# vghuy17ck1/svt-av1-psyex

Measured on AMD Instinct MI355X. Metric: ME+RD-cost Mpixels/s (2160p10 preset-6), higher is better.
Workload: dtype u8 SAD / i32 transforms; 1 GPU; 3840x2160 10-bit synthetic pan sequence, preset 6 (M6) search controls at qp 35; step = 16 pictures (4 current pictures x ref distance 1,2,4,8; R=2): open-loop ME of all 2040 b64 + full-pel pred + RD chain (64x64,32x32,16x16 DCT_DCT, 10-bit, b quantizer; qcoeff + recon + scalars written); 3 picture sets alternate from step to step

## Files before the change

### include/svt_hip_me.h

```cpp
#ifndef SVT_HIP_ME_H
#define SVT_HIP_ME_H

#include <stdint.h>
#include <stddef.h>

#ifdef __cplusplus
extern "C" {
#endif

#define SVT_HIP_OK 0
#define SVT_HIP_ERR_NO_DEVICE 1
#define SVT_HIP_ERR_BAD_PARAM 2
#define SVT_HIP_ERR_NO_MEMORY 3
#define SVT_HIP_ERR_LAUNCH 4

#define SVT_HIP_MAX_LISTS 2
#define SVT_HIP_MAX_REFS 4
#define SVT_HIP_SQUARE_PU_COUNT 85
#define SVT_HIP_MAX_SAD_VALUE (128 * 128 * 255)

typedef struct SvtHipSearchArea {
    uint16_t width, height;
} SvtHipSearchArea;

typedef struct SvtHipSearchAreaMinMax {
    SvtHipSearchArea sa_min, sa_max;
} SvtHipSearchAreaMinMax;

typedef struct SvtHipMeConfig {
    uint8_t hme_search_method, me_search_method;
    uint8_t enable_hme_flag, enable_hme_level0_flag, enable_hme_level1_flag, enable_hme_level2_flag;
    uint16_t num_hme_sa_w, num_hme_sa_h;
    SvtHipSearchAreaMinMax hme_l0_sa;
    SvtHipSearchArea       hme_l1_sa, hme_l2_sa;
    SvtHipSearchAreaMinMax me_sa;
    uint8_t                prehme_enable, prehme_skip_search_line, prehme_l1_early_exit;
    uint8_t                me_type;
    SvtHipSearchAreaMinMax prehme_sa_cfg[2];
    uint8_t  enable_me_hme_ref_pruning;
    uint16_t prune_ref_if_hme_sad_dev_bigger_than_th, prune_ref_if_me_sad_dev_bigger_than_th;
    uint32_t zz_sad_th;
    uint16_t zz_sad_pct;
    uint32_t phme_sad_th;
    uint16_t phme_sad_pct;
    uint8_t  enable_me_sr_adjustment;
    uint16_t reduce_me_sr_based_on_mv_length_th, stationary_hme_sad_abs_th, stationary_me_sr_divisor;
    uint16_t reduce_me_sr_based_on_hme_sad_abs_th, me_sr_divisor_for_low_hme_sad;
    uint8_t  distance_based_hme_resizing;
    uint8_t  me_8x8_var_enabled;
    uint32_t me_sr_div4_th, me_sr_div2_th, me_sr_mult2_th;
    uint8_t  mv_sa_adj_enabled, mv_sa_adj_nearest_ref_only;
    uint16_t mv_sa_adj_mv_size_th, mv_sa_adj_sa_multiplier;
    int32_t  prune_me_candidates_th;
    uint8_t  use_best_unipred_cand_only;
    uint8_t  reduce_hme_l0_sr_th_min, reduce_hme_l0_sr_th_max;
    uint32_t me_early_exit_th, me_safe_limit_zz_th, prev_me_stage_based_exit_th;
} SvtHipMeConfig;

typedef struct SvtHipMePresetDesc {
    int8_t   enc_mode;
    uint8_t  input_resolution;
    uint8_t  sc_class1;
    uint8_t  rtc_tune;
    uint8_t  temporal_layer_index;
    uint8_t  hierarchical_levels;
    uint32_t qp;
    uint32_t frame_rate_q16;
    uint8_t  safe_limit_nref;
    uint32_t safe_limit_zz_th;
} SvtHipMePresetDesc;

typedef struct SvtHipPlaneDesc {
    const uint8_t *buffer_y;
    uint32_t       stride_y;
    uint16_t       org_x, org_y;
    uint16_t       width, height;
} SvtHipPlaneDesc;

typedef struct SvtHipContext   SvtHipContext;
typedef struct SvtHipPaPicture SvtHipPaPicture;

typedef struct SvtHipMePictureDesc {
    uint64_t picture_number;
    uint16_t aligned_width, aligned_height;
    uint8_t  num_of_list_to_search;
    uint8_t  num_of_ref_pic_to_search[SVT_HIP_MAX_LISTS];
    uint8_t  temporal_layer_index, hierarchical_levels, is_ref, similar_brightness_refs;
    uint8_t  enable_me_8x8, enable_me_16x16;
    uint8_t  max_number_of_pus_per_sb;
    uint8_t  max_cand, max_refs, max_l0;
    uint8_t  input_resolution;
    uint8_t  only_l_bwd;
    uint8_t  gm_enabled, gm_use_distance_based_active_th;
    uint16_t b64_row_start, b64_row_count;
    uint32_t tf_me_exit_th;
    uint64_t ref_picture_number[SVT_HIP_MAX_LISTS][SVT_HIP_MAX_REFS];
} SvtHipMePictureDesc;

typedef struct SvtHipMeResults {
    uint8_t  *total_me_candidate_index;
    uint32_t *me_mv_array;
    uint8_t  *me_candidate_array;
    uint32_t *me_64x64_distortion, *me_32x32_distortion, *me_16x16_distortion, *me_8x8_distortion;
    uint32_t *rc_me_distortion, *me_8x8_cost_variance;
    uint8_t  *stationary_block_present_sb, *rc_me_allow_gm;
    uint32_t *sb_best_sad, *sb_best_mv;
    int16_t  *hme_sc;
    uint32_t *hme_sad;
    uint8_t  *do_ref;
} SvtHipMeResults;

static inline uint32_t svt_hip_me_n_pu(uint8_t enable_me_16x16, uint8_t enable_me_8x8) {
    return enable_me_16x16 ? (enable_me_8x8 ? 85u : 21u) : 5u;
}

int  svt_hip_context_create(SvtHipContext **ctx, int device);
void svt_hip_context_destroy(SvtHipContext *ctx);
const char *svt_hip_last_error(const SvtHipContext *ctx);
void *svt_hip_context_stream(SvtHipContext *ctx);
int   svt_hip_context_sync(SvtHipContext *ctx);
int   svt_hip_context_set_me_waves_per_cu(SvtHipContext *ctx, uint32_t waves);
int   svt_hip_context_set_me_dense(SvtHipContext *ctx, int on);
int   svt_hip_context_set_me_staged(SvtHipContext *ctx, int on);
#define SVT_HIP_ME_CHAIN_KERNELS 7
int   svt_hip_context_set_me_timing(SvtHipContext *ctx, int on);
int   svt_hip_me_launch_times(SvtHipContext *ctx, float ms[SVT_HIP_ME_CHAIN_KERNELS]);
const char *svt_hip_me_chain_kernel_name(int i);
int   svt_hip_context_set_me_counting(SvtHipContext *ctx, int on);
int   svt_hip_me_dense_counters(SvtHipContext *ctx, unsigned long long out[2]);

int     svt_hip_me_config_from_preset(const SvtHipMePresetDesc *p, SvtHipMeConfig *cfg);
uint8_t svt_hip_input_resolution(uint32_t width, uint32_t height);
uint8_t svt_hip_enable_me_8x8(int8_t enc_mode, uint8_t rtc_tune, uint8_t input_resolution);

int  svt_hip_pa_picture_create(SvtHipContext *ctx, const SvtHipPlaneDesc *full, const SvtHipPlaneDesc *quarter,
                               const SvtHipPlaneDesc *sixteenth, SvtHipPaPicture **pic);
int  svt_hip_pa_picture_create_dev(SvtHipContext *ctx, const SvtHipPlaneDesc *full_dev, SvtHipPaPicture **pic);
int  svt_hip_pa_picture_update(SvtHipContext *ctx, SvtHipPaPicture *pic, const SvtHipPlaneDesc *full, int full_on_device);
int  svt_hip_pa_picture_update_ahead(SvtHipContext *ctx, SvtHipPaPicture *pic, const SvtHipPlaneDesc *full, int full_on_device);
void *svt_hip_context_transfer_stream(SvtHipContext *ctx);
void svt_hip_pa_picture_destroy(SvtHipContext *ctx, SvtHipPaPicture *pic);
int  svt_hip_pa_picture_download(SvtHipContext *ctx, const SvtHipPaPicture *pic, int level, uint8_t *dst,
                                 uint32_t dst_stride);
int  svt_hip_pa_picture_geometry(const SvtHipPaPicture *pic, int level, SvtHipPlaneDesc *out);

int svt_hip_me_picture(SvtHipContext *ctx, const SvtHipMeConfig *cfg, const SvtHipMePictureDesc *desc,
                       const SvtHipPaPicture *cur, const SvtHipPaPicture *const refs[SVT_HIP_MAX_LISTS][SVT_HIP_MAX_REFS],
                       SvtHipMeResults *res);
int svt_hip_me_picture_async(SvtHipContext *ctx, const SvtHipMeConfig *cfg, const SvtHipMePictureDesc *desc,
                             const SvtHipPaPicture *cur,
                             const SvtHipPaPicture *const refs[SVT_HIP_MAX_LISTS][SVT_HIP_MAX_REFS],
                             const SvtHipMeResults *res_dev);

typedef struct SvtHipMeJob {
    const SvtHipMeConfig      *cfg;
    const SvtHipMePictureDesc *desc;
    const SvtHipPaPicture     *cur;
    const SvtHipPaPicture     *refs[SVT_HIP_MAX_LISTS][SVT_HIP_MAX_REFS];
    const SvtHipMeResults     *results;
} SvtHipMeJob;
int svt_hip_me_pictures_async(SvtHipContext *ctx, uint32_t n_pictures, const SvtHipMeJob *jobs);

typedef struct SvtHipDgMetrics {
    uint64_t tot_dist;
    uint32_t tot_cplx;
    uint32_t tot_active;
    int32_t  sum_in_vectors;
    uint32_t reserved;
} SvtHipDgMetrics;

int svt_hip_dg_detector_hme_level0(SvtHipContext *ctx, const SvtHipPaPicture *src, const SvtHipPaPicture *ref,
                                   uint16_t aligned_width, uint16_t aligned_height, uint8_t input_resolution,
                                   SvtHipDgMetrics *metrics, uint32_t *b64_sad, int16_t *b64_mv);
int svt_hip_dg_detector_hme_level0_async(SvtHipContext *ctx, const SvtHipPaPicture *src, const SvtHipPaPicture *ref,
                                         uint16_t aligned_width, uint16_t aligned_height, uint8_t input_resolution,
                                         SvtHipDgMetrics *metrics_dev, uint32_t *b64_sad_dev, int16_t *b64_mv_dev);

#ifdef __cplusplus
}
#endif
#endif
```

### svt-av1-psyex_amd/api.py

```python
import ctypes as C
import os

import numpy as np

from . import abi

_HERE = os.path.dirname(os.path.abspath(__file__))
LIB_PATH = os.environ.get("SVT_HIP_LIBRARY") or os.path.join(_HERE, "libsvthip.so")
_lib = None

ERRORS = {1: "no usable gfx950 device", 2: "bad parameter", 3: "out of device memory", 4: "launch/stream error"}


class SvtHipError(RuntimeError):
    pass


def lib():
    global _lib
    if _lib is None:
        if not os.path.exists(LIB_PATH):
            raise SvtHipError(f"{LIB_PATH} is missing: build it with `make -C svt-av1-psyex_amd/csrc` "
                              "(or __graft_entry__.build()); there is no CPU fallback")
        try:
            import torch
        except Exception:
            pass
        L = C.CDLL(LIB_PATH)
        L.svt_hip_last_error.restype = C.c_char_p
        L.svt_hip_last_error.argtypes = [C.c_void_p]
        L.svt_hip_context_stream.restype = C.c_void_p
        L.svt_hip_context_stream.argtypes = [C.c_void_p]
        L.svt_hip_sizeof.restype = C.c_size_t
        L.svt_hip_input_resolution.restype = C.c_uint8
        L.svt_hip_enable_me_8x8.restype = C.c_uint8
        for name in ("svt_hip_context_destroy", "svt_hip_context_sync"):
            getattr(L, name).argtypes = [C.c_void_p]
        L.svt_hip_pa_picture_destroy.argtypes = [C.c_void_p, C.c_void_p]
        L.svt_hip_block_stats_jobs_per_wave.restype = C.c_uint32
        L.svt_hip_block_stats_jobs_per_wave.argtypes = [C.c_void_p, C.c_void_p]
        _lib = L
    return _lib


def config_from_preset(enc_mode, width, height, qp=35, temporal_layer_index=1, hierarchical_levels=4, sc_class1=0,
                       rtc_tune=0, fps=30):
    L = lib()
    pd = abi.MePresetDesc(enc_mode=enc_mode, input_resolution=L.svt_hip_input_resolution(width, height), sc_class1=sc_class1,
                          rtc_tune=rtc_tune, temporal_layer_index=temporal_layer_index, hierarchical_levels=hierarchical_levels,
                          qp=qp, frame_rate_q16=fps << 16)
    cfg = abi.MeConfig()
    rc = L.svt_hip_me_config_from_preset(C.byref(pd), C.byref(cfg))
    if rc:
        raise SvtHipError(f"svt_hip_me_config_from_preset: {ERRORS.get(rc, rc)}")
    return cfg


def picture_desc(width, height, picture_number, refs, enc_mode=6, temporal_layer_index=1, hierarchical_levels=4, is_ref=1,
                 gm_enabled=0, rtc_tune=0):
    L = lib()
    res = L.svt_hip_input_resolution(width, height)
    r0 = sum(1 for (li, _) in refs if li == 0)
    r1 = sum(1 for (li, _) in refs if li == 1)
    d = abi.MePictureDesc(picture_number=picture_number, aligned_width=width, aligned_height=height,
                          num_of_list_to_search=2 if r1 else 1, temporal_layer_index=temporal_layer_index,
                          hierarchical_levels=hierarchical_levels, is_ref=is_ref, similar_brightness_refs=0,
                          enable_me_8x8=L.svt_hip_enable_me_8x8(enc_mode, rtc_tune, res), enable_me_16x16=1,
                          max_number_of_pus_per_sb=85, input_resolution=res, gm_enabled=gm_enabled)
    d.num_of_ref_pic_to_search[0] = r0
    d.num_of_ref_pic_to_search[1] = r1
    d.max_refs = r0 + r1
    d.max_cand = r0 + r1 + r0 * r1 + (r0 - 1) + (1 if r1 == 3 else 0)
    d.max_l0 = r0
    for (li, ri), num in refs.items():
        d.ref_picture_number[li][ri] = num
    return d


class Context:

    def __init__(self, device=-1):
        self._h = C.c_void_p()
        rc = lib().svt_hip_context_create(C.byref(self._h), device)
        if rc:
            raise SvtHipError(f"svt_hip_context_create failed: {ERRORS.get(rc, rc)} -- the HIP path cannot run here")

    def check(self, rc, what):
        if rc:
            raise SvtHipError(f"{what}: {ERRORS.get(rc, rc)}: {lib().svt_hip_last_error(self._h).decode()}")

    @property
    def stream(self):
        return lib().svt_hip_context_stream(self._h)

    def sync(self):
        self.check(lib().svt_hip_context_sync(self._h), "sync")

    def close(self):
        if self._h:
            lib().svt_hip_context_destroy(self._h)
            self._h = C.c_void_p()

    def set_me_dense(self, on):
        self.check(lib().svt_hip_context_set_me_dense(self._h, 1 if on else 0), "svt_hip_context_set_me_dense")

    def set_me_staged(self, on):
        self.check(lib().svt_hip_context_set_me_staged(self._h, int(on)), "svt_hip_context_set_me_staged")

    def set_me_timing(self, on):
        self.check(lib().svt_hip_context_set_me_timing(self._h, 1 if on else 0), "svt_hip_context_set_me_timing")

    def me_launch_times(self):
        L = lib()
        ms = (C.c_float * 7)()
        self.check(L.svt_hip_me_launch_times(self._h, ms), "svt_hip_me_launch_times")
        L.svt_hip_me_chain_kernel_name.restype = C.c_char_p
        return {L.svt_hip_me_chain_kernel_name(i).decode(): float(ms[i]) for i in range(7) if ms[i] > 0}

    def set_me_counting(self, on):
        self.check(lib().svt_hip_context_set_me_counting(self._h, 1 if on else 0), "svt_hip_context_set_me_counting")

    def me_dense_counters(self):
        v = (C.c_ulonglong * 2)()
        self.check(lib().svt_hip_me_dense_counters(self._h, v), "svt_hip_me_dense_counters")
        return int(v[0]), int(v[1])

    def upload(self, host_pyramid, device_pyramid=True):
        pic = C.c_void_p()
        full = host_pyramid.desc(2)
        if device_pyramid:
            rc = lib().svt_hip_pa_picture_create(self._h, C.byref(full), None, None, C.byref(pic))
        else:
            q, s = host_pyramid.desc(1), host_pyramid.desc(0)
            rc = lib().svt_hip_pa_picture_create(self._h, C.byref(full), C.byref(q), C.byref(s), C.byref(pic))
        self.check(rc, "svt_hip_pa_picture_create")
        return DevicePicture(self, pic, host_pyramid.picture_number)

    def upload_dev(self, dev_ptr, stride, width, height, pad, picture_number=0):
        pic = C.c_void_p()
        full = abi.PlaneDesc(dev_ptr, stride, pad, pad, width, height)
        self.check(lib().svt_hip_pa_picture_create_dev(self._h, C.byref(full), C.byref(pic)), "svt_hip_pa_picture_create_dev")
        return DevicePicture(self, pic, picture_number)

    def _ref_array(self, refs):
        arr = ((C.c_void_p * abi.MAX_REFS) * abi.MAX_LISTS)()
        for (li, ri), pic in refs.items():
            arr[li][ri] = pic._h
        return arr

    def me_picture(self, cfg, desc, cur, refs, search_level=True):
        n = abi.n_pu(desc.enable_me_16x16, desc.enable_me_8x8)
        nb = ((desc.aligned_width + 63) // 64) * ((desc.aligned_height + 63) // 64)
        res, arrs = abi.MeResults(), {}
        for name, dt, cnt in abi.RESULT_FIELDS:
            if not search_level and name in ("sb_best_sad", "sb_best_mv", "hme_sc", "hme_sad", "do_ref"):
                continue
            arrs[name] = np.zeros((nb, cnt(n, desc.max_refs, desc.max_cand)), dtype=dt)
            setattr(res, name, arrs[name].ctypes.data)
        rc = lib().svt_hip_me_picture(self._h, C.byref(cfg), C.byref(desc), cur._h, self._ref_array(refs), C.byref(res))
        self.check(rc, "svt_hip_me_picture")
        return arrs

    def me_picture_async(self, cfg, desc, cur, refs, res_dev):
        rc = lib().svt_hip_me_picture_async(self._h, C.byref(cfg), C.byref(desc), cur._h, self._ref_array(refs), C.byref(res_dev))
        self.check(rc, "svt_hip_me_picture_async")


    def me_pictures_async(self, jobs):
        arr = (abi.MeJob * len(jobs))()
        for j, (cfg, desc, cur, refs, res) in zip(arr, jobs):
            j.cfg, j.desc, j.results = C.addressof(cfg), C.addressof(desc), C.addressof(res)
            j.cur = cur._h if isinstance(cur._h, int) else cur._h.value
            for (li, ri), pic in refs.items():
                j.refs[li][ri] = pic._h if isinstance(pic._h, int) else pic._h.value
        self.check(lib().svt_hip_me_pictures_async(self._h, len(jobs), arr), "svt_hip_me_pictures_async")


    def dg_detector_hme_level0(self, src, ref, aligned_width, aligned_height, input_resolution, per_block=True):
        n = ((aligned_width + 63) // 64) * ((aligned_height + 63) // 64)
        m = abi.DgMetrics()
        sad = np.zeros(n, np.uint32) if per_block else None
        mv = np.zeros((n, 2), np.int16) if per_block else None
        rc = lib().svt_hip_dg_detector_hme_level0(self._h, src._h, ref._h, aligned_width, aligned_height, input_resolution, C.byref(m),
                                                  sad.ctypes.data_as(C.c_void_p) if per_block else None,
                                                  mv.ctypes.data_as(C.c_void_p) if per_block else None)
        self.check(rc, "svt_hip_dg_detector_hme_level0")
        out = m.as_dict()
        if per_block:
            out["b64_sad"], out["b64_mv"] = sad, mv
        return out


    def dg_detector_hme_level0_async(self, src, ref, aligned_width, aligned_height, input_resolution, metrics_ptr, sad_ptr=None, mv_ptr=None):
        rc = lib().svt_hip_dg_detector_hme_level0_async(self._h, src._h, ref._h, aligned_width, aligned_height, input_resolution,
                                                        C.c_void_p(metrics_ptr), C.c_void_p(sad_ptr), C.c_void_p(mv_ptr))
        self.check(rc, "svt_hip_dg_detector_hme_level0_async")


class DevicePicture:
    def __init__(self, ctx, handle, picture_number):
        self.ctx, self._h, self.picture_number = ctx, handle, picture_number

    def geometry(self, level):
        d = abi.PlaneDesc()
        self.ctx.check(lib().svt_hip_pa_picture_geometry(self._h, level, C.byref(d)), "geometry")
        return d

    def download(self, level):
        g = self.geometry(level)
        out = np.zeros((g.height + 2 * g.org_y, g.width + 2 * g.org_x), np.uint8)
        self.ctx.check(lib().svt_hip_pa_picture_download(self.ctx._h, self._h, level, out.ctypes.data_as(C.c_void_p), out.shape[1]), "download")
        return out

    def free(self):
        if self._h:
            lib().svt_hip_pa_picture_destroy(self.ctx._h, self._h)
            self._h = C.c_void_p()
```

### svt-av1-psyex_amd/csrc/me_kernel.hip

```cpp
#include <hip/hip_runtime.h>
#include <stdint.h>
#include <string.h>
#include "me_kernel.h"
#include "wave_ops.h"
#include "lds_dma.h"

#ifdef SVT_HIP_ME_PROFILE
struct Prof { uint32_t *acc; unsigned long long last; int step; };
#define SVT_HIP_ME_PROFILE_LDS (48 * 4)
#define PROF_DECL Prof prof_; prof_.acc = reinterpret_cast<uint32_t *>(g_lds + lay.total); if (threadIdx.x < 48) prof_.acc[threadIdx.x] = 0; prof_.last = __builtin_readcyclecounter(); prof_.step = 0; Prof *prof = &prof_
#define PROF_STEP(s) (prof->step = (s))
#define PROFS(i) PROF((i) + prof->step)
#define PROF(i) do { const unsigned long long t_ = __builtin_readcyclecounter(); if (threadIdx.x == 0) atomicAdd(&prof->acc[i], (uint32_t)(t_ - prof->last)); prof->last = t_; } while (0)
#define PROF_FLUSH(ptr) do { __builtin_amdgcn_fence(__ATOMIC_RELEASE, "wavefront"); if (threadIdx.x < 48) atomicAdd((unsigned long long *)(ptr) + threadIdx.x, (unsigned long long)prof->acc[threadIdx.x]); } while (0)
#define PROF_PARAM , Prof *prof
#define PROF_ARG , prof
#else
#define PROF_DECL do { } while (0)
#define PROF(i) do { } while (0)
#define PROFS(i) do { } while (0)
#define PROF_STEP(s) do { } while (0)
#define PROF_FLUSH(ptr) do { } while (0)
#define SVT_HIP_ME_PROFILE_LDS 0
#define PROF_PARAM
#define PROF_ARG
#endif

namespace {

constexpr int kThreads  = 64;
constexpr int kMaxReq   = 32;
constexpr int kWinBytes = SVT_HIP_ME_WIN_BYTES;
constexpr int kSrc64Pitch = 80, kSrc32Pitch = 48, kSrc16Pitch = 16;
constexpr int kNarrowMaxPos = 32;

__device__ const uint8_t c_z_to_raster[85] = {
    0,  1,  2,  3,  4,  5,  6,  9,  10, 7,  8,  11, 12, 13, 14, 17, 18, 15, 16, 19, 20, 21, 22, 29, 30, 23, 24, 31, 32,
    37, 38, 45, 46, 39, 40, 47, 48, 25, 26, 33, 34, 27, 28, 35, 36, 41, 42, 49, 50, 43, 44, 51, 52, 53, 54, 61, 62, 55,
    56, 63, 64, 69, 70, 77, 78, 71, 72, 79, 80, 57, 58, 65, 66, 59, 60, 67, 68, 73, 74, 81, 82, 75, 76, 83, 84};
__device__ const uint8_t c_8x8_to_16x16[64] = {5,  5,  6,  6,  7,  7,  8,  8,  5,  5,  6,  6,  7,  7,  8,  8,  9,  9,  10, 10, 11, 11,
                                               12, 12, 9,  9,  10, 10, 11, 11, 12, 12, 13, 13, 14, 14, 15, 15, 16, 16, 13, 13, 14, 14,
                                               15, 15, 16, 16, 17, 17, 18, 18, 19, 19, 20, 20, 17, 17, 18, 18, 19, 19, 20, 20};
__device__ const uint8_t c_16x16_to_32x32[16] = {1, 1, 2, 2, 1, 1, 2, 2, 3, 3, 4, 4, 3, 3, 4, 4};

typedef unsigned long long u64;

#define SVT_CONST_AS __attribute__((address_space(4)))
typedef const SVT_CONST_AS MeKernelParams CParams;
typedef const SVT_CONST_AS DevPlane       CPlane;

struct Req {
    const uint8_t *win;
    uint32_t       stride;
    int16_t        sa_w, sa_h;
    uint8_t        bw, bh, rs, level;
    uint8_t        skip_even, done;
    int16_t        pad1;
};

struct SearchGeo { int ox, oy, sa_w, sa_h; };

constexpr int kMaxTiles = 40;
struct __attribute__((aligned(16))) TileEnt {
    const uint8_t *g0;
    uint32_t stride;
    int16_t  x0, y0;
    int16_t  w, h;
    uint16_t pitch, nvec;
    uint8_t  req, flags;
    uint8_t  bw, bh;
    uint8_t  rs, kd, km, pad;
};
static_assert(sizeof(TileEnt) == 32, "TileEnt is read as two 16-byte words");

struct MeReq {
    const uint8_t *pix0;
    uint32_t       stride;
    int16_t        ox, oy, sa_w, sa_h;
    uint8_t        li, ri, probe, pad;
    int16_t        min_x, max_x, min_y, max_y;
};

struct PreHme {
    uint16_t sa_w, sa_h;
    int16_t  col, row;
    uint32_t sad;
    uint8_t  valid, pad[3];
};

struct St {
    uint32_t org_x, org_y, b64_w, b64_h, b64_index;
    uint32_t zz_sad[2][4];
    uint32_t sr_divisor[2][4];
    uint32_t hme_sad_final[2][4];
    u64      hme_sad64[2][4];
    int16_t  hme_sc_x[2][4], hme_sc_y[2][4];
    uint8_t  do_ref[2][4];
    PreHme   prehme[2][4][2];
    uint8_t  performed_phme[2][4][2];
    int16_t  hx[3][2][4][2][2], hy[3][2][4][2][2];
    uint32_t hs[3][2][4][2][2];
    SvtHipSearchAreaMinMax hme_l0_sa;
    int16_t  me_cx[2][4], me_cy[2][4];
    uint8_t  ph_req[2][4][2];
    uint8_t  l0_req[2][4];
    uint8_t  lvl_req[2][4][2][2];
    uint8_t  c00_req[2][4];
    int      nreq;
    union {
        Req      req[kMaxReq];
        struct { MeReq me[8], me_probe[8]; };
    };
    u64      req_key[kMaxReq];
    TileEnt  tile[kMaxTiles];
    uint32_t sadbuf[kNarrowMaxPos];
    int      nme, nprobe;
    uint32_t me_dist[85];
    uint8_t  cand0[88];
    uint32_t red[8];
    int      job, tf_exit;
};

struct LdsLayout { uint32_t src16, src32, src64, bsad, bmv, dense, win, total; };
constexpr int kMeFull = 0, kMeMid1 = 1, kMeS1 = 2, kMeMid2 = 4, kMeS2 = 5, kMeTail = 7;
#ifndef SVT_HIP_ME_LIST_WAVES_PER_CU
#define SVT_HIP_ME_LIST_WAVES_PER_CU 2
#endif
constexpr uint32_t kListWavesPerCu = SVT_HIP_ME_LIST_WAVES_PER_CU;
constexpr uint32_t kStagedMinJobs = 2048;
__host__ __device__ constexpr bool me_is_search(int m) { return m == kMeS1 || m == kMeS2; }
constexpr int kDirectWinBytes = 5120;
__host__ __device__ constexpr LdsLayout lds_layout(int n_slot, int cshift, int dense = 1, int mode = 0) {
    const bool v16 = mode == kMeFull, v32 = mode == kMeFull || mode == kMeS1, v64 = mode == kMeFull || mode == kMeS2 || mode == kMeTail;
    const bool best = mode == kMeFull || mode == kMeTail, slots = dense && (mode == kMeFull || mode == kMeMid1);
    const uint32_t arena = (mode == kMeMid1 || mode == kMeMid2) ? 0u : (mode == kMeS1 || mode == kMeS2) ? (uint32_t)kDirectWinBytes : (uint32_t)kWinBytes;
    LdsLayout l = {};
    l.src16 = (uint32_t)((sizeof(St) + 15) & ~(size_t)15);
    l.src32 = l.src16 + (v16 ? (uint32_t)((16 >> cshift) * kSrc16Pitch) : 0u);
    l.src64 = l.src32 + (v32 ? (uint32_t)((32 >> cshift) * kSrc32Pitch) : 0u);
    l.bsad  = l.src64 + (v64 ? (uint32_t)((64 >> cshift) * kSrc64Pitch) : 0u);
    l.bmv   = l.bsad + (best ? (uint32_t)n_slot * 85 * 4 : 0u);
    l.dense = (l.bmv + (best ? (uint32_t)n_slot * 85 * 4 : 0u) + 15) & ~15u;
    l.win   = l.dense + (slots ? (uint32_t)n_slot * SVT_HIP_ME_DENSE_KINDS * 16u : 0u);
    l.total = l.win + arena;
    return l;
}
extern __shared__ __attribute__((aligned(16))) uint8_t g_lds[];
struct Shared {
    St       &st;
    uint32_t  src64, src32, src16, win;
    int       cshift;
};
#define LDS(off) (g_lds + (off))

__host__ __device__ __forceinline__ int iabs(int v) { return v < 0 ? -v : v; }
__host__ __device__ __forceinline__ int imax(int a, int b) { return a > b ? a : b; }
__host__ __device__ __forceinline__ int imin(int a, int b) { return a < b ? a : b; }
__device__ __forceinline__ uint32_t umin32(uint32_t a, uint32_t b) { return a < b ? a : b; }
__device__ __forceinline__ uint32_t umin(uint32_t a, uint32_t b) { return a < b ? a : b; }

__host__ __device__ __forceinline__ uint32_t scaled_distance(uint32_t dist) { return (dist * 5) / 8 + ((dist % 8) ? 1 : 0); }

template <class P> __host__ __device__ __forceinline__ uint32_t ref_distance(P &p, int li, int ri) {
    long long d = (long long)p.desc.picture_number - (long long)p.desc.ref_picture_number[li][ri];
    return (uint16_t)(int16_t)(d < 0 ? -d : d);
}

__device__ __forceinline__ void clip_axis(int org, int &origin, int &size, int pad, int dim) {
    if (org + origin < -pad) origin = -pad - org;
    if (org + origin > dim - 1) origin -= (org + origin) - (dim - 1);
    if (org + origin + size > dim) size = imax(1, size - ((org + origin + size) - dim));
}

__device__ __forceinline__ const uint8_t *plane_at(CPlane &pl, int x, int y) {
    return pl.base + (long long)(pl.org_y + y) * pl.stride + (pl.org_x + x);
}


__device__ __forceinline__ float rcp_of(uint32_t d) { return __builtin_amdgcn_rcpf((float)d); }
__device__ __forceinline__ uint32_t div_by_rcp(uint32_t k, float r) { return (uint32_t)(((float)k + 0.5f) * r); }

__device__ __forceinline__ uint32_t row_pitch(int w, int bw) {
    uint32_t p = (uint32_t)(((w + 7) & ~7) + bw + 4 + 15) & ~15u;
    return (p & 16u) ? p : p + 16u;
}

__device__ __forceinline__ uint32_t tile_bytes(const Req &r, int w, int h) {
    return row_pitch(w, r.bw) * (uint32_t)(h - 1 + (r.bh - 1) * r.rs + 1);
}




__device__ __forceinline__ const uint8_t *src_view(const Shared &sh, int level) {
    return LDS(level == 2 ? sh.src64 : (level == 1 ? sh.src32 : sh.src16));
}

template <int NDW>
__device__ __forceinline__ void quad_sad_rows(const uint8_t *src, int src_pitch, int srs, const uint8_t *wrow0, int pitch, int rs, int r0, int r1,
                                              uint32_t out[4]) {
    uint32_t a0 = 0, a1 = 0, a2 = 0, a3 = 0;
    constexpr int kRowsPerFlush = 64 / NDW;
    for (int rb = r0; rb < r1; rb += kRowsPerFlush) {
        const int re = rb + kRowsPerFlush < r1 ? rb + kRowsPerFlush : r1;
        u64       acc = 0;
        for (int r = rb; r < re; r++) {
            const uint32_t *s = reinterpret_cast<const uint32_t *>(src + r * srs * src_pitch);
            const uint32_t *w = reinterpret_cast<const uint32_t *>(wrow0 + r * rs * pitch);
            uint32_t sv[NDW], wv[NDW + 1];
            if constexpr (NDW % 4 == 0) {
#pragma unroll
                for (int j = 0; j < NDW; j += 4) {
                    const uint4 q = *reinterpret_cast<const uint4 *>(s + j);
                    sv[j] = q.x; sv[j + 1] = q.y; sv[j + 2] = q.z; sv[j + 3] = q.w;
                }
            } else {
#pragma unroll
                for (int j = 0; j < NDW; j++) sv[j] = s[j];
            }
#pragma unroll
            for (int j = 0; j <= NDW; j++) wv[j] = w[j];
#pragma unroll
            for (int j = 0; j < NDW; j++) acc = __builtin_amdgcn_qsad_pk_u16_u8(((u64)wv[j + 1] << 32) | wv[j], sv[j], acc);
        }
        a0 += (uint32_t)(acc & 0xFFFF); a1 += (uint32_t)((acc >> 16) & 0xFFFF);
        a2 += (uint32_t)((acc >> 32) & 0xFFFF); a3 += (uint32_t)(acc >> 48);
    }
    out[0] = a0; out[1] = a1; out[2] = a2; out[3] = a3;
}

__device__ __attribute__((noinline)) uint4 quad_sad_generic(const uint8_t *src, int src_pitch, int srs, const uint8_t *wrow0, int pitch, int rs, int bw, int r0, int r1) {
    uint32_t a0 = 0, a1 = 0, a2 = 0, a3 = 0;
    if ((bw & 3) == 0) {
        const int nd = bw >> 2;
        for (int r = r0; r < r1; r++) {
            const uint32_t *s = reinterpret_cast<const uint32_t *>(src + r * srs * src_pitch);
            const uint32_t *w = reinterpret_cast<const uint32_t *>(wrow0 + r * rs * pitch);
            u64      acc = 0;
            uint32_t lo  = w[0];
            for (int j = 0; j < nd; j++) {
                const uint32_t hi = w[j + 1];
                acc = __builtin_amdgcn_qsad_pk_u16_u8(((u64)hi << 32) | lo, s[j], acc);
                lo  = hi;
            }
            a0 += (uint32_t)(acc & 0xFFFF); a1 += (uint32_t)((acc >> 16) & 0xFFFF);
            a2 += (uint32_t)((acc >> 32) & 0xFFFF); a3 += (uint32_t)(acc >> 48);
        }
    } else {
        for (int r = r0; r < r1; r++) {
            const uint8_t *s = src + r * srs * src_pitch;
            const uint8_t *w = wrow0 + r * rs * pitch;
            for (int c = 0; c < bw; c++) {
                const int sv = s[c];
                a0 += (uint32_t)iabs(sv - (int)w[c]);     a1 += (uint32_t)iabs(sv - (int)w[c + 1]);
                a2 += (uint32_t)iabs(sv - (int)w[c + 2]); a3 += (uint32_t)iabs(sv - (int)w[c + 3]);
            }
        }
    }
    return make_uint4(a0, a1, a2, a3);
}

__device__ __forceinline__ void quad_sad(const uint8_t *src, int src_pitch, int srs, const uint8_t *wrow0, int pitch, int rs, int bw, int r0,
                                         int r1, uint32_t out[4]) {
    switch (bw) {
    case 16: quad_sad_rows<4>(src, src_pitch, srs, wrow0, pitch, rs, r0, r1, out); return;
    case 32: quad_sad_rows<8>(src, src_pitch, srs, wrow0, pitch, rs, r0, r1, out); return;
    case 64: quad_sad_rows<16>(src, src_pitch, srs, wrow0, pitch, rs, r0, r1, out); return;
    case 8: quad_sad_rows<2>(src, src_pitch, srs, wrow0, pitch, rs, r0, r1, out); return;
    case 4: quad_sad_rows<1>(src, src_pitch, srs, wrow0, pitch, rs, r0, r1, out); return;
    default: break;
    }
    const uint4 v = quad_sad_generic(src, src_pitch, srs, wrow0, pitch, rs, bw, r0, r1);
    out[0] = v.x; out[1] = v.y; out[2] = v.z; out[3] = v.w;
}

template <int NDW>
__device__ __forceinline__ void oct_sad_rows(const uint8_t *src, int src_pitch, int srs, const uint8_t *wrow0, int pitch, int rs, int r0, int r1, uint32_t out[8]) {
    uint32_t a[8] = {0, 0, 0, 0, 0, 0, 0, 0};
    constexpr int kRowsPerFlush = 64 / NDW;
    constexpr int CH = NDW > 8 ? 8 : NDW;
    for (int rb = r0; rb < r1; rb += kRowsPerFlush) {
        const int re = rb + kRowsPerFlush < r1 ? rb + kRowsPerFlush : r1;
        u64       acc0 = 0, acc1 = 0;
        for (int r = rb; r < re; r++) {
            const uint32_t *s = reinterpret_cast<const uint32_t *>(src + r * srs * src_pitch);
            const uint32_t *w = reinterpret_cast<const uint32_t *>(wrow0 + r * rs * pitch);
#pragma unroll
            for (int c0 = 0; c0 < NDW; c0 += CH) {
                uint32_t sv[CH], wv[CH + 2];
                if constexpr (CH % 4 == 0) {
#pragma unroll
                    for (int j = 0; j < CH; j += 4) {
                        const uint4 q = *reinterpret_cast<const uint4 *>(s + c0 + j);
                        sv[j] = q.x; sv[j + 1] = q.y; sv[j + 2] = q.z; sv[j + 3] = q.w;
                    }
                } else {
#pragma unroll
                    for (int j = 0; j < CH; j++) sv[j] = s[c0 + j];
                }
                if constexpr (CH % 2 == 0) {
#pragma unroll
                    for (int j = 0; j < CH + 2; j += 2) {
                        const uint2 q = *reinterpret_cast<const uint2 *>(w + c0 + j);
                        wv[j] = q.x; wv[j + 1] = q.y;
                    }
                } else {
#pragma unroll
                    for (int j = 0; j < CH + 2; j++) wv[j] = w[c0 + j];
                }
#pragma unroll
                for (int j = 0; j < CH; j++) {
                    acc0 = __builtin_amdgcn_qsad_pk_u16_u8(((u64)wv[j + 1] << 32) | wv[j], sv[j], acc0);
                    acc1 = __builtin_amdgcn_qsad_pk_u16_u8(((u64)wv[j + 2] << 32) | wv[j + 1], sv[j], acc1);
                }
            }
        }
#pragma unroll
        for (int i = 0; i < 4; i++) { a[i] += (uint32_t)((acc0 >> (16 * i)) & 0xFFFF); a[4 + i] += (uint32_t)((acc1 >> (16 * i)) & 0xFFFF); }
    }
#pragma unroll
    for (int i = 0; i < 8; i++) out[i] = a[i];
}

__device__ __forceinline__ void oct_sad(const uint8_t *src, int src_pitch, int srs, const uint8_t *wrow0, int pitch, int rs, int bw, int r0, int r1, uint32_t out[8]) {
    switch (bw) {
    case 16: oct_sad_rows<4>(src, src_pitch, srs, wrow0, pitch, rs, r0, r1, out); return;
    case 32: oct_sad_rows<8>(src, src_pitch, srs, wrow0, pitch, rs, r0, r1, out); return;
    case 64: oct_sad_rows<16>(src, src_pitch, srs, wrow0, pitch, rs, r0, r1, out); return;
    case 8: oct_sad_rows<2>(src, src_pitch, srs, wrow0, pitch, rs, r0, r1, out); return;
    case 4: oct_sad_rows<1>(src, src_pitch, srs, wrow0, pitch, rs, r0, r1, out); return;
    default: break;
    }
    quad_sad(src, src_pitch, srs, wrow0, pitch, rs, bw, r0, r1, out);
    quad_sad(src, src_pitch, srs, wrow0 + 4, pitch, rs, bw, r0, r1, out + 4);
}

typedef uint32_t V4 __attribute__((ext_vector_type(4)));
typedef const __attribute__((address_space(1))) V4 GV4;
constexpr int kVecPerLane = (kWinBytes / 16 + 63) / 64;

__device__ __forceinline__ uint32_t uni(uint32_t v) { return (uint32_t)__builtin_amdgcn_readfirstlane((int)v); }
__device__ __forceinline__ const uint8_t *uni_ptr(const uint8_t *p) {
    const uintptr_t a = reinterpret_cast<uintptr_t>(p);
    return reinterpret_cast<const uint8_t *>(((uintptr_t)uni((uint32_t)(a >> 32)) << 32) | uni((uint32_t)a));
}

__device__ __forceinline__ u64 wave_min_key(uint32_t sad, uint32_t pos) {
    const uint32_t smin = wave_min_dpp(sad);
    const uint32_t pmin = wave_min_dpp(sad == smin ? pos : 0xFFFFFFFFu);
    return ((u64)smin << 32) | pmin;
}

struct TileGeo {
    const uint8_t *g0;
    uint32_t stride;
    int      req;
    int      x0, y0, w, h;
    int      pitch, nvec;
    int      last;
    int      bw, bh, rs, level, skip_even, narrow;
    int      kd, km;
};

__device__ __forceinline__ int scan32(int v) {
#define SVT_SCAN_DPP(ctrl, rmask, bc) v += __builtin_amdgcn_update_dpp(0, v, ctrl, rmask, 0xF, bc);
    SVT_SCAN_DPP(0x111, 0xF, true)
    SVT_SCAN_DPP(0x112, 0xF, true)
    SVT_SCAN_DPP(0x114, 0xF, true)
    SVT_SCAN_DPP(0x118, 0xF, true)
    SVT_SCAN_DPP(0x142, 0xA, false)
#undef SVT_SCAN_DPP
    return v;
}

__device__ __forceinline__ int plan_tiles(St &st, int nreq, int t0) {
    const int lane = threadIdx.x;
    int cnt = 0, tw = 8, th = 1, ntx = 1;
    Req r = {};
    if (lane < nreq) {
        r = st.req[lane];
        if (r.done) {
        } else if (r.sa_w > 0 && r.sa_h > 0) {
            tw = r.sa_w; th = r.sa_h;
            while (th > 1 && tile_bytes(r, tw, th) > (uint32_t)kWinBytes) th = (th + 1) >> 1;
            while (tw > 8 && tile_bytes(r, tw, th) > (uint32_t)kWinBytes) tw = ((tw >> 1) + 7) & ~7;
            ntx = (int)div_by_rcp((uint32_t)(r.sa_w + tw - 1), rcp_of((uint32_t)tw));
            cnt = ntx * (int)div_by_rcp((uint32_t)(r.sa_h + th - 1), rcp_of((uint32_t)th));
        } else if (t0 == 0)
            st.req_key[lane] = (0xffffffull << 32) | 0xffffffffull;
    }
    const int incl = scan32(cnt), base = incl - cnt - t0;
    const int total = __builtin_amdgcn_readlane(incl, 31);
    const float ntx_rcp = rcp_of((uint32_t)ntx);
    const int narrow = (r.sa_w * r.sa_h <= kNarrowMaxPos) ? 1 : 0;
    for (int k = imax(0, -base); k < cnt && base + k < kMaxTiles; k++) {
        const int ty = (int)div_by_rcp((uint32_t)k, ntx_rcp), tx = k - ty * ntx;
        const int x0 = tx * tw, y0 = ty * th, w = imin(tw, r.sa_w - x0), h = imin(th, r.sa_h - y0);
        const int pitch = (int)row_pitch(w, r.bw), vpr = pitch >> 4;
        const int kd = (int)div_by_rcp(64u, rcp_of((uint32_t)vpr));
        TileEnt e;
        e.g0 = r.win + x0 + (long long)y0 * r.stride; e.stride = r.stride;
        e.x0 = (int16_t)x0; e.y0 = (int16_t)y0; e.w = (int16_t)w; e.h = (int16_t)h;
        e.pitch = (uint16_t)pitch; e.nvec = (uint16_t)(vpr * (h - 1 + (r.bh - 1) * r.rs + 1));
        e.req = (uint8_t)lane; e.flags = (uint8_t)(r.level | (r.skip_even << 2) | (narrow << 3) | ((k == cnt - 1) << 4));
        e.bw = r.bw; e.bh = r.bh; e.rs = r.rs; e.kd = (uint8_t)kd; e.km = (uint8_t)(64 - kd * vpr); e.pad = 0;
        st.tile[base + k] = e;
    }
    return total;
}

__device__ __forceinline__ TileGeo read_tile(const St &st, int i) {
    const uint4 a = *reinterpret_cast<const uint4 *>(&st.tile[i]);
    const uint4 b = *(reinterpret_cast<const uint4 *>(&st.tile[i]) + 1);
    const uint32_t a0 = uni(a.x), a1 = uni(a.y), a2 = uni(a.z), a3 = uni(a.w), b0 = uni(b.x), b1 = uni(b.y), b2 = uni(b.z), b3 = uni(b.w);
    TileGeo t;
    t.g0 = reinterpret_cast<const uint8_t *>(((uintptr_t)a1 << 32) | a0); t.stride = a2;
    t.x0 = (int16_t)(a3 & 0xFFFF); t.y0 = (int16_t)(a3 >> 16); t.w = (int16_t)(b0 & 0xFFFF); t.h = (int16_t)(b0 >> 16);
    t.pitch = (int)(b1 & 0xFFFF); t.nvec = (int)(b1 >> 16);
    t.req = (int)(b2 & 0xFF);
    const int f = (int)((b2 >> 8) & 0xFF);
    t.level = f & 3; t.skip_even = (f >> 2) & 1; t.narrow = (f >> 3) & 1; t.last = (f >> 4) & 1;
    t.bw = (int)((b2 >> 16) & 0xFF); t.bh = (int)(b2 >> 24);
    t.rs = (int)(b3 & 0xFF); t.kd = (int)((b3 >> 8) & 0xFF); t.km = (int)((b3 >> 16) & 0xFF);
    return t;
}

typedef uint32_t V4U __attribute__((ext_vector_type(4), aligned(1)));
typedef const __attribute__((address_space(1))) V4U GV4U;
constexpr int kSmallVec = 128;
template <int S0, int NS>
__device__ __forceinline__ void tile_load(const TileGeo &t, V4 (&v)[kVecPerLane]) {
    const int      lane = threadIdx.x, vpr = t.pitch >> 4, nrows = (int)div_by_rcp((uint32_t)t.nvec, rcp_of((uint32_t)vpr));
    const int      row0 = (int)div_by_rcp((uint32_t)lane, rcp_of((uint32_t)vpr));
    int            c    = lane - row0 * vpr;
    uint32_t       off  = (uint32_t)__mul24(row0, (int)t.stride) + (uint32_t)c * 16u;
    const uint32_t last = (uint32_t)__mul24(nrows - 1, (int)t.stride) + (uint32_t)(vpr - 1) * 16u;
    const uint32_t step = (uint32_t)__mul24(t.kd, (int)t.stride) + (uint32_t)t.km * 16u, wrap = t.stride - (uint32_t)vpr * 16u;
    const uintptr_t base = reinterpret_cast<uintptr_t>(t.g0);
#pragma unroll
    for (int j = 0; j < NS; j++)
        if (j * 64 < t.nvec) {
            v[S0 + j] = __builtin_bit_cast(V4, *reinterpret_cast<GV4U *>(base + (uint64_t)umin(off, last)));
            off += step; c += t.km;
            if (c >= vpr) { c -= vpr; off += wrap; }
        }
}
template <int S0, int NS>
__device__ __forceinline__ void tile_store(const Shared &sh, int nvec, int lds_vec, const V4 (&v)[kVecPerLane]) {
    const int lane = threadIdx.x;
#pragma unroll
    for (int j = 0; j < NS; j++)
        if (j * 64 < nvec && lane + j * 64 < nvec) *reinterpret_cast<V4 *>(&LDS(sh.win)[(lds_vec + lane + j * 64) * 16]) = v[S0 + j];
}

__device__ __forceinline__ u64 tile_eval(const Shared &sh, const TileGeo &t, int lds_off PROF_PARAM) {
    St            &st   = sh.st;
    const int      lane = threadIdx.x;
    const uint8_t *src  = src_view(sh, t.level);
    const uint8_t *win  = LDS(sh.win) + lds_off;
    const int      sp   = (t.level == 2) ? kSrc64Pitch : (t.level == 1 ? kSrc32Pitch : kSrc16Pitch);
    const int      srs  = t.rs >> sh.cshift;
    uint32_t bsad_ = 0xFFFFFFFFu, bpos_ = 0xFFFFFFFFu;
    if (!t.narrow) {
        const int   ng = (t.w + 7) >> 3, nitems = ng * t.h;
        const float ng_rcp = rcp_of((uint32_t)ng);
        uint32_t best = 0xFFFFFFFFu;
        int      seq  = 0;
        for (int it = lane; it < nitems; it += kThreads, seq += 8) {
            const int y = (int)div_by_rcp((uint32_t)it, ng_rcp), g = it - y * ng;
            if (t.skip_even && !((t.y0 + y) & 1)) continue;
            uint32_t s8[8];
            oct_sad(src, sp, srs, win + y * t.pitch + 8 * g, t.pitch, t.rs, t.bw, 0, t.bh, s8);
            uint32_t k[8];
#pragma unroll
            for (int i = 0; i < 8; i++) k[i] = (s8[i] << 12) + (uint32_t)i;
            if (t.w & 7) {
#pragma unroll
// ... 143 lines not shown
    for (int dpt = 0; dpt < DEPTH; dpt++) {
#pragma unroll
        for (int k = 0; k < NV; k++) v[dpt][k] = V4U{0, 0, 0, 0};
        request(v[dpt], dpt);
    }
    u64 acc0 = 0, acc1 = 0;
    auto step = [&](V4U (&r)[NV], int t) {
#pragma unroll
        for (int k = 0; k < NV; k++) *reinterpret_cast<V4U *>(arena + 16 * (lane + 64 * k)) = r[k];
        wave_sync();
        request(r, t + DEPTH);
        if (t < rows) {
            const uint32_t *s = reinterpret_cast<const uint32_t *>(src + (e0 + t) * srs * sp);
            uint32_t sv[NDW], wv[4 * NV];
#pragma unroll
            for (int j = 0; j < NDW; j += 4) {
                const uint4 q = *reinterpret_cast<const uint4 *>(s + j);
                sv[j] = q.x; sv[j + 1] = q.y; sv[j + 2] = q.z; sv[j + 3] = q.w;
            }
#pragma unroll
            for (int k = 0; k < NV; k++) {
                const uint4 q = *reinterpret_cast<const uint4 *>(arena + 16 * (lane * NV + k));
                wv[4 * k] = q.x; wv[4 * k + 1] = q.y; wv[4 * k + 2] = q.z; wv[4 * k + 3] = q.w;
            }
#pragma unroll
            for (int j = 0; j < NDW; j++) {
                acc0 = __builtin_amdgcn_qsad_pk_u16_u8(((u64)wv[j + 1] << 32) | wv[j], sv[j], acc0);
                acc1 = __builtin_amdgcn_qsad_pk_u16_u8(((u64)wv[j + 2] << 32) | wv[j + 1], sv[j], acc1);
            }
        }
        if ((t + 1) % kRowsPerFlush == 0 || t + 1 == rows_max) {
#pragma unroll
            for (int i = 0; i < 4; i++) { a[i] += (uint32_t)((acc0 >> (16 * i)) & 0xFFFF); a[4 + i] += (uint32_t)((acc1 >> (16 * i)) & 0xFFFF); }
            acc0 = acc1 = 0;
        }
        wave_sync();
    };
    for (int t = 0; t < rows_max; t += DEPTH) {
        step(v[0], t);
        if (DEPTH >= 2 && t + 1 < rows_max) step(v[DEPTH >= 2 ? 1 : 0], t + 1);
        if (DEPTH >= 3 && t + 2 < rows_max) step(v[DEPTH >= 3 ? 2 : 0], t + 2);
    }
#pragma unroll
    for (int i = 0; i < 8; i++) out[i] = a[i];
}

__device__ __forceinline__ bool small_direct_ok(const St &st, int *q_total = nullptr) {
    const int lane = threadIdx.x, nreq = (int)uni((uint32_t)st.nreq);
    const Req &r0 = st.req[0];
    const int  bw = (int)uni(r0.bw), bh = (int)uni(r0.bh), rs = (int)uni(r0.rs), level = (int)uni(r0.level), stride = (int)uni((uint32_t)r0.stride);
    bool ok = true;
    int  per = 0;
    if (lane < nreq) {
        const Req &r = st.req[lane];
        const int  w = r.sa_w, h = r.sa_h;
        ok  = w > 0 && h > 0 && w * h <= kNarrowMaxPos && r.bw == bw && r.bh == bh && r.rs == rs && r.level == level && (int)r.stride == stride && !r.skip_even && !r.done;
        per = ((w + 7) >> 3) * h;
    }
    if (!__all(ok) || (bw != 32 && bw != 64) || nreq > kMaxReq || nreq <= 0) return false;
    const int q = (int)wave_sum_dpp((uint32_t)per);
    if (q_total) *q_total = q;
    return q <= kThreads;
}
template <int NDW, int DEPTH>
__device__ __forceinline__ void ring_rows(uint8_t *arena, const uint8_t *src, int sp, int srs, const St &st, int nreq, int lg, int S, int rows_per, int bh, int rs, int sa_h,
                                          long long stride, uint32_t (&a)[3][8]) {
    constexpr int NV = (NDW + 2 + 3) / 4, kRowsPerFlush = 64 / NDW;
    static_assert(NV & 1, "owners read their pieces back without bank conflicts");
    static_assert(DEPTH >= 1 && DEPTH <= 3, "steps in flight");
    const int lane = threadIdx.x, gmask = (1 << lg) - 1;
    const int steps_max = rs * (rows_per - 1) + sa_h;
    const uint8_t *pp[NV];
    int            pn[NV];
#pragma unroll
    for (int k = 0; k < NV; k++) {
        const int  n = lane + 64 * k, owner = n / NV, part = n - owner * NV, orq = owner >> lg, osl = owner & gmask;
        const bool act = orq < nreq && osl < S;
        const int  oe0 = osl * rows_per, orows = imin(oe0 + rows_per, bh) - oe0;
        pn[k] = act ? rs * (orows - 1) + sa_h : 0;
        pp[k] = st.req[act ? orq : 0].win + (long long)(oe0 * rs) * stride + 16 * part;
    }
    const int  req = lane >> lg, slice = lane & gmask, e0 = slice * rows_per;
    const int  rows = (req < nreq && slice < S) ? imin(e0 + rows_per, bh) - e0 : 0;
    V4U v[DEPTH][NV];
    auto request = [&](V4U (&r)[NV], int step) {
#pragma unroll
        for (int k = 0; k < NV; k++) {
            if (step < pn[k]) r[k] = *reinterpret_cast<GV4U *>(reinterpret_cast<uintptr_t>(pp[k]));
            pp[k] += stride;
        }
    };
#pragma unroll
    for (int dpt = 0; dpt < DEPTH; dpt++) {
#pragma unroll
        for (int k = 0; k < NV; k++) v[dpt][k] = V4U{0, 0, 0, 0};
        request(v[dpt], dpt);
    }
#pragma unroll
    for (int y = 0; y < 3; y++)
#pragma unroll
        for (int i = 0; i < 8; i++) a[y][i] = 0;
    u64 acc[3][2] = {{0, 0}, {0, 0}, {0, 0}};
    auto step = [&](V4U (&r)[NV], int j) {
#pragma unroll
        for (int k = 0; k < NV; k++) *reinterpret_cast<V4U *>(arena + 16 * (lane + 64 * k)) = r[k];
        wave_sync();
        request(r, j + DEPTH);
        uint32_t wv[4 * NV];
#pragma unroll
        for (int k = 0; k < NV; k++) {
            const uint4 q = *reinterpret_cast<const uint4 *>(arena + 16 * (lane * NV + k));
            wv[4 * k] = q.x; wv[4 * k + 1] = q.y; wv[4 * k + 2] = q.z; wv[4 * k + 3] = q.w;
        }
#pragma unroll
        for (int y = 0; y < 3; y++) {
            const int dd = j - y, t = rs == 2 ? dd >> 1 : dd;
            if (y < sa_h && dd >= 0 && (rs == 1 || !(dd & 1)) && t < rows_per) {
                if (t < rows) {
                    const uint32_t *s = reinterpret_cast<const uint32_t *>(src + (e0 + t) * srs * sp);
                    uint32_t sv[NDW];
#pragma unroll
                    for (int c = 0; c < NDW; c += 4) {
                        const uint4 q = *reinterpret_cast<const uint4 *>(s + c);
                        sv[c] = q.x; sv[c + 1] = q.y; sv[c + 2] = q.z; sv[c + 3] = q.w;
                    }
#pragma unroll
                    for (int c = 0; c < NDW; c++) {
                        acc[y][0] = __builtin_amdgcn_qsad_pk_u16_u8(((u64)wv[c + 1] << 32) | wv[c], sv[c], acc[y][0]);
                        acc[y][1] = __builtin_amdgcn_qsad_pk_u16_u8(((u64)wv[c + 2] << 32) | wv[c + 1], sv[c], acc[y][1]);
                    }
                }
                if ((t + 1) % kRowsPerFlush == 0 || t + 1 == rows_per) {
#pragma unroll
                    for (int i = 0; i < 4; i++) { a[y][i] += (uint32_t)((acc[y][0] >> (16 * i)) & 0xFFFF); a[y][4 + i] += (uint32_t)((acc[y][1] >> (16 * i)) & 0xFFFF); }
                    acc[y][0] = acc[y][1] = 0;
                }
            }
        }
        wave_sync();
    };
    for (int j = 0; j < steps_max; j += DEPTH) {
        step(v[0], j);
        if (DEPTH >= 2 && j + 1 < steps_max) step(v[DEPTH >= 2 ? 1 : 0], j + 1);
        if (DEPTH >= 3 && j + 2 < steps_max) step(v[DEPTH >= 3 ? 2 : 0], j + 2);
    }
}

template <int DEPTH> __device__ __forceinline__ void run_ring_searches(Shared &sh, int nreq, int bw, int bh, int rs, int level, int sa_h PROF_PARAM) {
    St       &st   = sh.st;
    const int lane = threadIdx.x;
    int lg = 0;
    while ((2 << lg) * nreq <= kThreads) lg++;
    const int S0 = imin(bh, 1 << lg), rows_per = (int)uni(div_by_rcp((uint32_t)(bh + S0 - 1), rcp_of((uint32_t)S0)));
    const int S  = (int)uni(div_by_rcp((uint32_t)(bh + rows_per - 1), rcp_of((uint32_t)rows_per)));
    const uint8_t *src = src_view(sh, level);
    const int      sp  = (level == 2) ? kSrc64Pitch : (level == 1 ? kSrc32Pitch : kSrc16Pitch), srs = rs >> sh.cshift;
    const long long stride = (long long)(int)uni((uint32_t)st.req[0].stride);
    uint32_t a[3][8];
    PROF(26);
    if (bw == 64) ring_rows<16, DEPTH>(LDS(sh.win), src, sp, srs, st, nreq, lg, S, rows_per, bh, rs, sa_h, stride, a);
    else ring_rows<8, DEPTH>(LDS(sh.win), src, sp, srs, st, nreq, lg, S, rows_per, bh, rs, sa_h, stride, a);
    PROF(27);
#define SVT_RING_SUM(cond, expr)                                                  \
    if (cond) {                                                                   \
        _Pragma("unroll") for (int y = 0; y < 3; y++)                             \
            _Pragma("unroll") for (int i = 0; i < 8; i++) { const uint32_t v = a[y][i]; a[y][i] = v + (uint32_t)(expr); } \
    }
    SVT_RING_SUM(lg >= 1, __builtin_amdgcn_mov_dpp((int)v, 0xB1 , 0xF, 0xF, true))
    SVT_RING_SUM(lg >= 2, __builtin_amdgcn_mov_dpp((int)v, 0x4E , 0xF, 0xF, true))
    SVT_RING_SUM(lg >= 3, __builtin_amdgcn_mov_dpp((int)v, 0x141 , 0xF, 0xF, true))
    SVT_RING_SUM(lg >= 4, __builtin_amdgcn_mov_dpp((int)v, 0x140 , 0xF, 0xF, true))
    SVT_RING_SUM(lg >= 5, __shfl_xor((int)v, 16, 64))
    SVT_RING_SUM(lg >= 6, __shfl_xor((int)v, 32, 64))
#undef SVT_RING_SUM
    PROF(23);
    const int req = lane >> lg;
    if (req < nreq && (lane & ((1 << lg) - 1)) == 0) {
        const int w = st.req[req].sa_w;
        uint32_t  best = 0xFFFFFFFFu;
#pragma unroll
        for (int y = 0; y < 3; y++)
#pragma unroll
            for (int i = 0; i < 8; i++)
                if (y < sa_h && i < w) best = umin(best, (a[y][i] << 6) | (uint32_t)(y * w + i));
        const int wl = (int)(best & 63u), wy = (int)div_by_rcp((uint32_t)wl, rcp_of((uint32_t)w)), wx = wl - wy * w;
        st.req_key[req] = ((u64)(best >> 6) << 32) | ((uint32_t)wy << 16) | (uint32_t)wx;
    }
    wave_sync();
}

#ifndef SVT_HIP_ME_DIRECT_RING
#define SVT_HIP_ME_DIRECT_RING 1
#endif
#ifndef SVT_HIP_ME_DIRECT_RING_FULL
#define SVT_HIP_ME_DIRECT_RING_FULL 0
#endif
#ifndef SVT_HIP_ME_DIRECT_TRUST
#define SVT_HIP_ME_DIRECT_TRUST 1
#endif
template <int DEPTH = 1, bool QUALIFIED = false, bool RING = true> __device__ __forceinline__ bool run_small_searches_direct(Shared &sh PROF_PARAM) {
    St       &st   = sh.st;
    const int lane = threadIdx.x, nreq = (int)uni((uint32_t)st.nreq);
    if constexpr (!(QUALIFIED && SVT_HIP_ME_DIRECT_TRUST)) {
        if (!small_direct_ok(st)) return false;
    }
    const Req &r0 = st.req[0];
    const int  bw = (int)uni(r0.bw), bh = (int)uni(r0.bh), rs = (int)uni(r0.rs), level = (int)uni(r0.level);
    int per = 0;
    if constexpr (RING && SVT_HIP_ME_DIRECT_RING) {
        const int h0 = (int)uni((uint32_t)r0.sa_h);
        bool alike = true;
        if (lane < nreq) {
            const int w = st.req[lane].sa_w, h = st.req[lane].sa_h;
            alike = w <= 8 && h == h0;
            per   = ((w + 7) >> 3) * h;
        }
        if (h0 <= 3 && rs <= 2 && __all(alike)) {
            run_ring_searches<DEPTH>(sh, nreq, bw, bh, rs, level, h0 PROF_ARG);
            return true;
        }
    } else if (lane < nreq)
        per = ((st.req[lane].sa_w + 7) >> 3) * st.req[lane].sa_h;
    const int Q = (int)wave_sum_dpp((uint32_t)per);
    {
        int incl = per;
#pragma unroll
        for (int o = 1; o < 32; o <<= 1) { const int t = __shfl_up(incl, o, 64); if ((lane & 31) >= o) incl += t; }
        if (lane < nreq) st.req_key[lane] = (u64)(uint32_t)(incl - per);
    }
    wave_sync();
    int       S        = imin(bh, (int)uni(div_by_rcp((uint32_t)kThreads, rcp_of((uint32_t)Q))));
    const int rows_per = (int)uni(div_by_rcp((uint32_t)(bh + S - 1), rcp_of((uint32_t)S)));
    S                  = (int)uni(div_by_rcp((uint32_t)(bh + rows_per - 1), rcp_of((uint32_t)rows_per)));
    uint32_t *sad = reinterpret_cast<uint32_t *>(LDS(sh.win));
    const uint8_t *src = src_view(sh, level);
    const int      sp  = (level == 2) ? kSrc64Pitch : (level == 1 ? kSrc32Pitch : kSrc16Pitch), srs = rs >> sh.cshift;
    const long long wstep = (long long)rs * (long long)(int)uni((uint32_t)r0.stride);
    const bool mine = lane < Q * S;
    int req = 0, y = 0, g = 0, e0 = 0, rows = 0, w = 1;
    const uint8_t *wp = nullptr;
    if (mine) {
        const int slice = (int)div_by_rcp((uint32_t)lane, rcp_of((uint32_t)Q)), q = lane - slice * Q;
        for (int r = 1; r < nreq; r++) req += q >= (int)(uint32_t)st.req_key[r] ? 1 : 0;
        const Req &r = st.req[req];
        w = r.sa_w;
        const int ng = (w + 7) >> 3, ql = q - (int)(uint32_t)st.req_key[req];
        y = (int)div_by_rcp((uint32_t)ql, rcp_of((uint32_t)ng)); g = ql - y * ng;
        e0   = slice * rows_per;
        rows = imin(e0 + rows_per, bh) - e0;
        wp   = r.win + (long long)y * r.stride + (long long)e0 * wstep + 8 * g;
    }
    uint32_t s8[8];
    PROF(26);
    if (bw == 64) direct_rows<16, DEPTH>(LDS(sh.win), src, sp, srs, wp, wstep, e0, rows, rows_per, s8);
    else direct_rows<8, DEPTH>(LDS(sh.win), src, sp, srs, wp, wstep, e0, rows, rows_per, s8);
    PROF(27);
    for (int p = lane; p < nreq * kNarrowMaxPos; p += kThreads) sad[p] = 0;
    wave_sync();
    if (mine) {
#pragma unroll
        for (int i = 0; i < 8; i++)
            if (8 * g + i < w) atomicAdd(&sad[req * kNarrowMaxPos + y * w + 8 * g + i], s8[i]);
    }
    wave_sync();
    PROF(23);
    for (int rq = 0; rq < nreq; rq++) {
        const int      wr = (int16_t)uni((uint32_t)st.req[rq].sa_w), hr = (int16_t)uni((uint32_t)st.req[rq].sa_h);
        const uint32_t k32 = wave_min_dpp(lane < wr * hr ? (sad[rq * kNarrowMaxPos + lane] << 6) | (uint32_t)lane : 0xFFFFFFFFu);
        const int      wl = (int)(k32 & 63u), wy = (int)uni(div_by_rcp((uint32_t)wl, rcp_of((uint32_t)wr))), wx = wl - wy * wr;
        if (lane == 0) st.req_key[rq] = ((u64)(k32 >> 6) << 32) | ((uint32_t)wy << 16) | (uint32_t)wx;
    }
    wave_sync();
    return true;
}

constexpr int kDenseKinds = SVT_HIP_ME_DENSE_KINDS;
__device__ __forceinline__ uint32_t dense_pack(int a, int b) { return (uint32_t)(uint16_t)a | ((uint32_t)(uint16_t)b << 16); }
__device__ __forceinline__ void dense_take(St &st, const MeDenseSlot *dl, int idx, int req, const SearchGeo &g, uint32_t &n_hit, uint32_t &n_miss) {
    if (!dl) return;
    const MeDenseSlot s = dl[idx];
    if (s.org == dense_pack(g.ox, g.oy) && s.size == dense_pack(g.sa_w, g.sa_h)) {
        st.req[req].done = 1;
        st.req_key[req]  = s.key == ~0ull ? ((0xffffffull << 32) | 0xffffffffull) : s.key;
        n_hit++;
    } else
        n_miss++;
}

__device__ __forceinline__ void push_req(St &st, const uint8_t *win, uint32_t stride, int sa_w, int sa_h, int bw, int bh, int rs,
                                         int level, int skip, int slot = -1) {
    Req &r      = st.req[slot >= 0 ? slot : st.nreq++];
    r.win       = win;
    r.stride    = stride;
    r.sa_w      = (int16_t)sa_w;
    r.sa_h      = (int16_t)sa_h;
    r.bw        = (uint8_t)bw;
    r.bh        = (uint8_t)bh;
    r.rs        = (uint8_t)rs;
    r.level     = (uint8_t)level;
    r.skip_even = (uint8_t)(skip && bw == 16 && bh <= 16);
    r.done      = 0;
}

__device__ __forceinline__ void push_hme_req(St &st, CParams &p, int level, CPlane &rp, int org_x, int org_y,
                                             int bw, int bh, int ox, int oy, int sa_w, int sa_h, int skip, int slot = -1) {
    const int full = (p.cfg.hme_search_method == 1);
    push_req(st, plane_at(rp, org_x + ox, org_y + oy), rp.stride, sa_w, sa_h, bw, full ? bh : (bh >> 1), full ? 1 : 2, level, skip, slot);
}


__device__ __forceinline__ void upd(u64 &best, uint32_t sad, uint32_t ord) {
    const u64 k = ((u64)sad << 32) | ord;
    best        = k < best ? k : best;
}

__device__ __attribute__((noinline)) void stage_clamped(uint8_t *win, const uint8_t *pix0, uint32_t stride, int min_x, int max_x, int min_y, int max_y, int wx0, int wy0,
                                                        int pitch, int rows) {
    for (int i = threadIdx.x; i < pitch * rows; i += kThreads) {
        const int row = i / pitch, cb = i - row * pitch;
        const int x = imin(imax(wx0 + cb, min_x), max_x), y = imin(imax(wy0 + row, min_y), max_y);
        win[row * pitch + cb] = pix0[x + (long long)y * stride];
    }
}

constexpr int kMeOrdBits = 12;
__device__ __forceinline__ void run_me_searches(Shared &sh, CParams &p, const MeReq *list, int count, uint32_t *bsad, uint32_t *bmv, int r0n PROF_PARAM) {
    const int lane = threadIdx.x;
    const int sub  = (p.cfg.me_search_method == 0);
    const int nrow = sub ? 4 : 8, rstep = sub ? 2 : 1;
    const int g = lane >> 4, pu = lane & 15;
    const int bx = (pu & 1) | ((pu >> 1) & 2), by = ((pu >> 1) & 1) | ((pu >> 2) & 2);
    const uint8_t *srow = &LDS(sh.src64)[bx * 16];
    for (int mi = 0; mi < count; mi++) {
        MeReq m;
        {
            const MeReq &mm = list[mi];
            m.pix0 = uni_ptr(mm.pix0); m.stride = uni(mm.stride);
            m.ox = (int16_t)uni((uint32_t)mm.ox); m.oy = (int16_t)uni((uint32_t)mm.oy); m.sa_w = (int16_t)uni((uint32_t)mm.sa_w); m.sa_h = (int16_t)uni((uint32_t)mm.sa_h);
            m.li = (uint8_t)uni(mm.li); m.ri = (uint8_t)uni(mm.ri); m.probe = 0; m.pad = 0;
            m.min_x = (int16_t)uni((uint32_t)mm.min_x); m.max_x = (int16_t)uni((uint32_t)mm.max_x); m.min_y = (int16_t)uni((uint32_t)mm.min_y); m.max_y = (int16_t)uni((uint32_t)mm.max_y);
        }
        u64 b8[4] = {~0ull, ~0ull, ~0ull, ~0ull}, b16 = ~0ull, b32 = ~0ull, b64 = ~0ull;
        const int W = m.sa_w, H = m.sa_h;
        int       tw = W, th = H;
        auto me_pitch = [](int shift, int ww) { return ((shift + ww - 1 + 64 + 15) & ~15) + 16; };
        auto wbytes = [&](int ww, int hh) { return (uint32_t)me_pitch(0, ww) * (uint32_t)(hh - 1 + 64); };
        while (th > 1 && (wbytes(tw, th) > (uint32_t)kWinBytes || tw * th > (1 << kMeOrdBits))) th = (th + 1) >> 1;
        while (tw > 8 && (wbytes(tw, th) > (uint32_t)kWinBytes || tw * th > (1 << kMeOrdBits))) tw = ((tw >> 1) + 7) & ~7;
        for (int y0 = 0; y0 < H; y0 += th)
            for (int x0 = 0; x0 < W; x0 += tw) {
                const int w = imin(tw, W - x0), h = imin(th, H - y0);
                const uint8_t *gwin  = m.pix0 + (m.ox + x0) + (long long)(m.oy + y0) * m.stride;
                const int pitch = me_pitch(0, w);
                const int rows        = h - 1 + 64;
                const int vec_per_row = pitch >> 4;
                lds_dma_after_stores();
                const int wx0 = m.ox + x0, wy0 = m.oy + y0;
                if (m.ox + x0 >= m.min_x && m.ox + x0 + w - 1 + 63 <= m.max_x && wy0 >= m.min_y && wy0 + rows - 1 <= m.max_y) {
                    lds_dma_window(gwin, m.stride, vec_per_row, rows, g_lds, sh.win);
                    lds_dma_wait();
                } else {
                    stage_clamped(LDS(sh.win), m.pix0, m.stride, m.min_x, m.max_x, m.min_y, m.max_y, wx0, wy0, pitch, rows);
                }
                wave_sync();
                PROF(46);
                const int ng = (w + 3) >> 2;
                uint32_t k8[4] = {~0u, ~0u, ~0u, ~0u}, k16 = ~0u, k32 = ~0u, k64 = ~0u;
                const int kshift = kMeOrdBits + sub;
                for (int y = 0; y < h; y += 4) {
                    const bool live = y + g < h;
                    const int  yy   = live ? y + g : h - 1;
                    const uint8_t *wrow = &LDS(sh.win)[(yy + by * 16) * pitch + bx * 16];
                    const uint32_t ord0 = (uint32_t)(yy * w);
                    for (int gq = 0; gq < ng; gq++) {
                        const uint8_t *wp = wrow + 4 * gq;
                        u64 acc[4] = {0, 0, 0, 0};
#pragma unroll
                        for (int half = 0; half < 2; half++)
#pragma unroll
                            for (int k = 0; k < 8; k++) {
                                if (k < nrow) {
                                    const int r = 8 * half + k * rstep;
                                    const uint32_t *wr = reinterpret_cast<const uint32_t *>(wp + r * pitch);
                                    const uint32_t d0 = wr[0], d1 = wr[1], d2 = wr[2], d3 = wr[3], d4 = wr[4];
                                    const uint4 sv = *reinterpret_cast<const uint4 *>(srow + ((by * 16 + r) >> sh.cshift) * kSrc64Pitch);
                                    acc[2 * half] = __builtin_amdgcn_qsad_pk_u16_u8(((u64)d1 << 32) | d0, sv.x, acc[2 * half]);
                                    acc[2 * half] = __builtin_amdgcn_qsad_pk_u16_u8(((u64)d2 << 32) | d1, sv.y, acc[2 * half]);
                                    acc[2 * half + 1] = __builtin_amdgcn_qsad_pk_u16_u8(((u64)d3 << 32) | d2, sv.z, acc[2 * half + 1]);
                                    acc[2 * half + 1] = __builtin_amdgcn_qsad_pk_u16_u8(((u64)d4 << 32) | d3, sv.w, acc[2 * half + 1]);
                                }
                            }
#pragma unroll
                        for (int i = 0; i < 4; i++) {
                            const int x = 4 * gq + i;
                            uint32_t v8[4];
#pragma unroll
                            for (int j = 0; j < 4; j++) v8[j] = (uint32_t)((acc[j] >> (16 * i)) & 0xFFFF);
                            const uint32_t v16 = (v8[0] + v8[1]) + (v8[2] + v8[3]);
                            const uint32_t v32 = quad_sum(v16);
                            const uint32_t v64 = row16_sum_of_quads(v32);
                            if (x < w && live) {
                                const uint32_t ord = ord0 + (uint32_t)x;
#pragma unroll
                                for (int j = 0; j < 4; j++) k8[j] = umin32(k8[j], (v8[j] << kshift) | ord);
                                k16 = umin32(k16, (v16 << kshift) | ord);
                                k32 = umin32(k32, (v32 << kshift) | ord);
                                k64 = umin32(k64, (v64 << kshift) | ord);
                            }
                        }
                    }
                }
                PROF(47);
                const float w_rcp = rcp_of((uint32_t)w);
                auto fold = [&](u64 &best, uint32_t k) {
                    k = umin32(k, (uint32_t)__shfl_xor((int)k, 16, 64));
                    k = umin32(k, (uint32_t)__shfl_xor((int)k, 32, 64));
                    if (k != ~0u) {
                        const uint32_t ordl = k & ((1u << kMeOrdBits) - 1u), ty = div_by_rcp(ordl, w_rcp), tx = ordl - ty * (uint32_t)w;
                        upd(best, k >> kMeOrdBits, (uint32_t)((y0 + (int)ty) * W + (x0 + (int)tx)));
                    }
                };
#pragma unroll
                for (int j = 0; j < 4; j++) fold(b8[j], k8[j]);
                fold(b16, k16); fold(b32, k32); fold(b64, k64);
            }
        uint32_t *rs_ = bsad + ((m.li ? r0n : 0) + m.ri) * 85, *rm_ = bmv + ((m.li ? r0n : 0) + m.ri) * 85;
        auto merge = [&](int n, u64 k) {
            const uint32_t sad = (uint32_t)(k >> 32);
            if (k != ~0ull && sad < rs_[n]) {
                const uint32_t ord = (uint32_t)k;
                const int      yy = (int)(ord / (uint32_t)W), xx = (int)(ord - (uint32_t)yy * (uint32_t)W);
                rs_[n] = sad;
                rm_[n] = ((uint32_t)(m.oy + yy) << 16) | (uint16_t)(m.ox + xx);
            }
        };
        if (g == 0) {
#pragma unroll
            for (int j = 0; j < 4; j++) merge(21 + 4 * pu + j, b8[j]);
            merge(5 + pu, b16);
            if ((pu & 3) == 0) merge(1 + (pu >> 2), b32);
            if (pu == 0) merge(0, b64);
        }
        wave_sync();
    }
}


constexpr int kC00Round = 8;
__device__ __forceinline__ void c00_sads(Shared &sh) {
    St &st = sh.st;
    const int lane = threadIdx.x;
    const int nreq = (int)uni((uint32_t)st.nreq), bw = (int)uni(st.b64_w), bh = (int)uni(st.b64_h);
    for (int q0 = 0; q0 < nreq; q0 += kC00Round) {
        V4 w[kC00Round][2];
#pragma unroll
        for (int j = 0; j < kC00Round; j++)
            if (q0 + j < nreq) {
                const uint8_t *win = uni_ptr(st.req[q0 + j].win);
                const uint32_t stride = uni(st.req[q0 + j].stride);
#pragma unroll
                for (int h = 0; h < 2; h++) {
                    const int i = lane + 64 * h, y = (i >> 2) * 2, x = (i & 3) * 16;
                    w[j][h] = V4{0, 0, 0, 0};
                    if (y < bh && x < bw) w[j][h] = __builtin_bit_cast(V4, *reinterpret_cast<GV4U *>(reinterpret_cast<uintptr_t>(win + (long long)y * stride + x)));
                }
            }
#pragma unroll
        for (int j = 0; j < kC00Round; j++)
            if (q0 + j < nreq) {
                uint32_t a = 0;
#pragma unroll
                for (int h = 0; h < 2; h++) {
                    const int i = lane + 64 * h, y = (i >> 2) * 2, x = (i & 3) * 16;
                    if (y < bh && x < bw) {
                        const V4 v = *reinterpret_cast<const V4 *>(&LDS(sh.src64)[(y >> sh.cshift) * kSrc64Pitch + x]);
                        a = __builtin_amdgcn_sad_u8(v.x, w[j][h].x, a);
                        a = __builtin_amdgcn_sad_u8(v.y, w[j][h].y, a);
                        if (x + 8 < bw) { a = __builtin_amdgcn_sad_u8(v.z, w[j][h].z, a); a = __builtin_amdgcn_sad_u8(v.w, w[j][h].w, a); }
                    }
                }
                const uint32_t t = wave_sum_dpp(a);
                if (lane == 0) st.req_key[q0 + j] = (u64)t << 32;
            }
    }
    wave_sync();
}

typedef uint32_t V2 __attribute__((ext_vector_type(2)));
typedef uint32_t V2U __attribute__((ext_vector_type(2), aligned(1)));
typedef const __attribute__((address_space(1))) V2U GV2U;

constexpr int kProbeRound = 4;
__device__ __forceinline__ void probe_sads(Shared &sh, CParams &p, uint32_t *bsad, uint32_t *bmv, int r0n PROF_PARAM) {
    St &st = sh.st;
    const int lane = threadIdx.x;
    const int sub  = (p.cfg.me_search_method == 0);
    const int nrow = sub ? 4 : 8, rstep = sub ? 2 : 1;
    const int px = 8 * ((lane & 1) | ((lane >> 1) & 2) | ((lane >> 2) & 4)), py = 8 * (((lane >> 1) & 1) | ((lane >> 2) & 2) | ((lane >> 3) & 4));
    const int count = (int)uni((uint32_t)st.nprobe);
    for (int m0 = 0; m0 < count; m0 += kProbeRound) {
        V2 w[kProbeRound][8];
#pragma unroll
        for (int j = 0; j < kProbeRound; j++)
            if (m0 + j < count) {
                const MeReq &mm = st.me_probe[m0 + j];
                const uint8_t *pix0 = uni_ptr(mm.pix0);
                const uint32_t stride = uni(mm.stride);
                const int ox = (int16_t)uni((uint32_t)mm.ox), oy = (int16_t)uni((uint32_t)mm.oy);
                const int min_x = (int16_t)uni((uint32_t)mm.min_x), max_x = (int16_t)uni((uint32_t)mm.max_x);
                const int min_y = (int16_t)uni((uint32_t)mm.min_y), max_y = (int16_t)uni((uint32_t)mm.max_y);
                if (ox >= min_x && ox + 63 <= max_x && oy >= min_y && oy + 63 <= max_y) {
                    const uint8_t *g = pix0 + (ox + px) + (long long)(oy + py) * stride;
#pragma unroll
                    for (int k = 0; k < 8; k++)
                        if (k < nrow) w[j][k] = __builtin_bit_cast(V2, *reinterpret_cast<GV2U *>(reinterpret_cast<uintptr_t>(g + (long long)(k * rstep) * stride)));
                }
            }
        PROF(17);
#pragma unroll
        for (int j = 0; j < kProbeRound; j++)
            if (m0 + j < count) {
                const MeReq &mm = st.me_probe[m0 + j];
                const int ox = (int16_t)uni((uint32_t)mm.ox), oy = (int16_t)uni((uint32_t)mm.oy);
                const int row = (uni(mm.li) ? r0n : 0) + (int)uni(mm.ri);
                const int min_x = (int16_t)uni((uint32_t)mm.min_x), max_x = (int16_t)uni((uint32_t)mm.max_x);
                const int min_y = (int16_t)uni((uint32_t)mm.min_y), max_y = (int16_t)uni((uint32_t)mm.max_y);
                uint32_t a = 0;
                if (ox >= min_x && ox + 63 <= max_x && oy >= min_y && oy + 63 <= max_y) {
#pragma unroll
                    for (int k = 0; k < 8; k++)
                        if (k < nrow) {
                            const V2 s = *reinterpret_cast<const V2 *>(&LDS(sh.src64)[((py + k * rstep) >> sh.cshift) * kSrc64Pitch + px]);
                            a = __builtin_amdgcn_sad_u8(s.x, w[j][k].x, a);
                            a = __builtin_amdgcn_sad_u8(s.y, w[j][k].y, a);
                        }
                } else {
                    const uint8_t *pix0 = uni_ptr(mm.pix0);
                    const uint32_t stride = uni(mm.stride);
#pragma nounroll
                    for (int i = 0; i < nrow * 8; i++) {
                        const int k = i >> 3, b = i & 7;
                        const int x = imin(imax(ox + px + b, min_x), max_x), y = imin(imax(oy + py + k * rstep, min_y), max_y);
                        a += (uint32_t)iabs((int)LDS(sh.src64)[((py + k * rstep) >> sh.cshift) * kSrc64Pitch + px + b] - (int)*reinterpret_cast<const __attribute__((address_space(1))) uint8_t *>(reinterpret_cast<uintptr_t>(pix0 + x + (long long)y * stride)));
                    }
                }
                const uint32_t v8 = a << sub, v16 = quad_sum(v8), v32 = row16_sum_of_quads(v16), v64 = wave_sum_dpp(v8);
                uint32_t *rs_ = bsad + row * 85, *rm_ = bmv + row * 85;
                const uint32_t mv = ((uint32_t)oy << 16) | (uint16_t)ox;
                auto merge = [&](int n, uint32_t sad) {
                    if (sad < rs_[n]) { rs_[n] = sad; rm_[n] = mv; }
                };
                merge(21 + lane, v8);
                if ((lane & 3) == 0) merge(5 + (lane >> 2), v16);
                if ((lane & 15) == 0) merge(1 + (lane >> 4), v32);
                if (lane == 0) merge(0, v64);
            }
    }
    wave_sync();
}


__device__ __forceinline__ bool searched(CParams &p, int li) { return p.desc.temporal_layer_index > 0 || li == 0; }

__device__ void set_hme_all(St &st, CParams &p, int lvl, int li, int ri, int x, int y, uint32_t sad) {
    for (int h = 0; h < p.cfg.num_hme_sa_h; h++)
        for (int w = 0; w < p.cfg.num_hme_sa_w; w++) {
            st.hx[lvl][li][ri][w][h] = (int16_t)x;
            st.hy[lvl][li][ri][w][h] = (int16_t)y;
            st.hs[lvl][li][ri][w][h] = sad;
        }
}

template <class P> __host__ __device__ __forceinline__ void hme_l0_area(P &p, int li, int ri, uint32_t dist, int mvx, int mvy, int &sa_w, int &sa_h) {
    auto &c = p.cfg;
    struct { SvtHipSearchAreaMinMax hme_l0_sa; } st;
    st.hme_l0_sa.sa_min.width = (uint16_t)c.hme_l0_sa.sa_min.width; st.hme_l0_sa.sa_min.height = (uint16_t)c.hme_l0_sa.sa_min.height;
    st.hme_l0_sa.sa_max.width = (uint16_t)c.hme_l0_sa.sa_max.width; st.hme_l0_sa.sa_max.height = (uint16_t)c.hme_l0_sa.sa_max.height;
    if (c.enable_me_sr_adjustment && c.distance_based_hme_resizing) {
        int is_hor = 1, is_ver = 1, is_still = 0;
        if (c.reduce_hme_l0_sr_th_min && c.reduce_hme_l0_sr_th_max && (li || ri)) {
            is_ver   = iabs(mvx) < c.reduce_hme_l0_sr_th_min && iabs(mvy) > c.reduce_hme_l0_sr_th_max;
            is_hor   = iabs(mvx) > c.reduce_hme_l0_sr_th_max && iabs(mvy) < c.reduce_hme_l0_sr_th_min;
            is_still = iabs(mvx) < c.reduce_hme_l0_sr_th_min * 3 && iabs(mvy) < c.reduce_hme_l0_sr_th_min * 3;
        }
        int xo = is_hor ? 1 : 2, yo = is_ver ? 1 : 2;
        if (c.enable_me_sr_adjustment == 2 && is_still) xo = yo = 4;
        st.hme_l0_sa.sa_min.width  = (uint16_t)(st.hme_l0_sa.sa_min.width / (xo + ri));
        st.hme_l0_sa.sa_min.height = (uint16_t)(st.hme_l0_sa.sa_min.height / (yo + ri));
        st.hme_l0_sa.sa_max.width  = (uint16_t)(st.hme_l0_sa.sa_max.width / (xo + ri));
        st.hme_l0_sa.sa_max.height = (uint16_t)(st.hme_l0_sa.sa_max.height / (yo + ri));
    }
    const int f = (int)scaled_distance(dist);
    int       w = (int16_t)(st.hme_l0_sa.sa_min.width / c.num_hme_sa_w);
    w           = (int16_t)imin(((w * f) + 15) & ~15, ((st.hme_l0_sa.sa_max.width / c.num_hme_sa_w) + 15) & ~15);
    int h       = (int16_t)(st.hme_l0_sa.sa_min.height / c.num_hme_sa_h);
    h           = (int16_t)imin(h * f, st.hme_l0_sa.sa_max.height / c.num_hme_sa_h);
    sa_w        = w;
    sa_h        = h;
}
__device__ void hme_l0_search_area(const St &cst, CParams &p, int li, int ri, uint32_t dist, int &sa_w, int &sa_h) {
    hme_l0_area(p, li, ri, dist, cst.hx[0][0][0][0][0], cst.hy[0][0][0][0][0], sa_w, sa_h);
}

template <class P> __host__ __device__ __forceinline__ void prehme_size(P &p, int li, int ri, int sri, int &sa_w, int &sa_h) {
    auto &c = p.cfg;
    const uint32_t f = scaled_distance(ref_distance(p, li, ri));
    sa_w = (int16_t)(uint16_t)imin((int)(c.prehme_sa_cfg[sri].sa_min.width * f), c.prehme_sa_cfg[sri].sa_max.width);
    sa_h = (int16_t)(uint16_t)imin((int)(c.prehme_sa_cfg[sri].sa_min.height * f), c.prehme_sa_cfg[sri].sa_max.height);
}
__device__ __forceinline__ SearchGeo prehme_geometry(CParams &p, int li, int ri, int sri, uint32_t org_x, uint32_t org_y) {
    int sa_w, sa_h;
    prehme_size(p, li, ri, sri, sa_w, sa_h);
    CPlane &rp = p.ref[li][ri].lvl[0];
    const int ox16 = (int16_t)org_x >> 2, oy16 = (int16_t)org_y >> 2;
    int ox = -(int16_t)(sa_w >> 1), oy = -(int16_t)(sa_h >> 1);
    clip_axis(ox16, ox, sa_w, rp.org_x - 1, rp.width);
    clip_axis(oy16, oy, sa_h, rp.org_y - 1, rp.height);
    SearchGeo g = {ox, oy, sa_w, sa_h};
    return g;
}

__device__ __forceinline__ SearchGeo hme_level_geometry(CParams &p, int level, CPlane &rp, int org_x, int org_y, int sa_w, int sa_h, int cx, int cy, int sr_w, int sr_h) {
    sa_w = (int16_t)((sa_w + 7) & ~7);
    int pad_w, pad_h, ox, oy;
    if (level == 2) { pad_w = pad_h = 63; } else { pad_w = rp.org_x - 1; pad_h = rp.org_y - 1; }
    if (level == 0) {
        ox = -(int16_t)((sa_w * p.cfg.num_hme_sa_w) >> 1) + (int16_t)(sa_w * sr_w);
        oy = -(int16_t)((sa_h * p.cfg.num_hme_sa_h) >> 1) + (int16_t)(sa_h * sr_h);
    } else {
        ox = -(sa_w >> 1) + cx;
        oy = -(sa_h >> 1) + cy;
    }
    clip_axis(org_x, ox, sa_w, pad_w, rp.width);
    sa_w = (sa_w < 8) ? sa_w : (sa_w & ~7);
    clip_axis(org_y, oy, sa_h, pad_h, rp.height);
    SearchGeo g = {ox, oy, sa_w, sa_h};
    return g;
}

struct HmeGeom { int16_t ox, oy; };

__device__ HmeGeom push_hme_level(St &st, CParams &p, int level, CPlane &rp, int org_x, int org_y, int bw, int bh,
                                  int sa_w, int sa_h, int cx, int cy, int sr_w, int sr_h, int slot = -1) {
    const SearchGeo sg = hme_level_geometry(p, level, rp, org_x, org_y, sa_w, sa_h, cx, cy, sr_w, sr_h);
    push_hme_req(st, p, level, rp, org_x, org_y, bw, bh, sg.ox, sg.oy, sg.sa_w, sg.sa_h, 0, slot);
    HmeGeom g = {(int16_t)sg.ox, (int16_t)sg.oy};
    return g;
}

__device__ __forceinline__ void key_to_result(u64 key, int full, uint32_t &sad, int &x, int &y) {
    sad = (uint32_t)(key >> 32);
    if ((uint32_t)key == 0xffffffffu) { x = 0; y = 0; }
    else { y = (int)((key >> 16) & 0xFFFF); x = (int)(key & 0xFFFF); }
    if (!full) sad *= 2;
}

__device__ __forceinline__ void push_zz_req(St &st, CPlane &rp, int dx, int dy, int slot = -1) {
    push_req(st, plane_at(rp, (int)st.org_x + dx, (int)st.org_y + dy), rp.stride, 1, 1, (int)st.b64_w, (int)st.b64_h >> 1, 2, 2, 0, slot);
}

}


#ifndef SVT_ME_CTRL_PRIO
#define SVT_ME_CTRL_PRIO 2
#endif
#define CTRL_PRIO(x) __builtin_amdgcn_s_setprio(x)

constexpr size_t kPersistBytes = (offsetof(St, req) + 15) & ~(size_t)15;
template <int MODE>
__device__ __forceinline__ void me_b64_body(const MeBatchHeader *__restrict__ ghdr, const MeKernelParams *__restrict__ gparams, const uint32_t launch_flags) {
    St     &st = *reinterpret_cast<St *>(g_lds);
    constexpr bool kImports = MODE == kMeMid2 || MODE == kMeTail;
    typedef const SVT_CONST_AS MeBatchHeader CHeader;
    CHeader  &hdr = *(CHeader *)ghdr;
    const int tid = threadIdx.x;
    const int       cshift = (int)hdr.cshift;
    const bool      has_dense = hdr.dense != nullptr;
    const LdsLayout lay    = lds_layout((int)hdr.n_slot, cshift, has_dense ? 1 : 0, MODE);
    uint32_t *const bsad = reinterpret_cast<uint32_t *>(g_lds + lay.bsad);
    uint32_t *const bmv  = reinterpret_cast<uint32_t *>(g_lds + lay.bmv);
    const MeDenseSlot *const dense_lds = has_dense ? reinterpret_cast<const MeDenseSlot *>(g_lds + lay.dense) : nullptr;
    uint32_t n_hit = 0, n_miss = 0;
    Shared sh = {st, lay.src64, lay.src32, lay.src16, lay.win, cshift};

    uint32_t xcc = 0;
    asm volatile("s_getreg_b32 %0, hwreg(HW_REG_XCC_ID)" : "=s"(xcc));
    xcc &= 7;
    int queue_probe = 0;
    constexpr int kList = 0;
    const bool list_mode = (launch_flags & 1u) != 0;
    const uint32_t n_total = hdr.job_base[hdr.n_pictures];
    uint32_t share_next = 0, share_end = 0, share_step = 1;
    if (MODE != kMeFull && !list_mode) {
        if (gridDim.x >= SVT_HIP_ME_QUEUES) {
            const uint32_t q = blockIdx.x % SVT_HIP_ME_QUEUES;
            share_step = (gridDim.x - q + SVT_HIP_ME_QUEUES - 1) / SVT_HIP_ME_QUEUES;
            share_next = hdr.queue_begin[q] + blockIdx.x / SVT_HIP_ME_QUEUES;
            share_end  = hdr.queue_begin[q + 1];
        } else {
            share_step = gridDim.x; share_next = blockIdx.x; share_end = n_total;
        }
    }
    auto fetch_job = [&]() {
        int job = -1;
        if (list_mode) {
            const uint32_t n = __hip_atomic_load(&hdr.queue_head[SVT_HIP_ME_LIST_COUNT(kList)], __ATOMIC_RELAXED, __HIP_MEMORY_SCOPE_AGENT);
            if (__hip_atomic_load(&hdr.queue_head[SVT_HIP_ME_LIST_CURSOR(kList)], __ATOMIC_RELAXED, __HIP_MEMORY_SCOPE_AGENT) >= n) return job;
            const uint32_t k = atomicAdd(&hdr.queue_head[SVT_HIP_ME_LIST_CURSOR(kList)], 1u);
            if (k < n) job = (int)hdr.lists[kList][k];
            return job;
        }
        if (MODE != kMeFull) {
            if (share_next < share_end) { job = (int)share_next; share_next += share_step; }
            return job;
        }
        while (queue_probe < SVT_HIP_ME_QUEUES) {
            const int      q  = (int)((xcc + queue_probe) & 7);
            const uint32_t lo = hdr.queue_begin[q], hi = hdr.queue_begin[q + 1];
            if (lo < hi) {
                const uint32_t k = atomicAdd(&hdr.queue_head[q], 1u);
                if (lo + k < hi) { job = (int)(lo + k); break; }
            }
            queue_probe++;
        }
        return job;
    };
    auto stage_base = [&](int gjob) { return hdr.stage + (size_t)gjob * SVT_HIP_ME_STAGE_BYTES; };
    auto export_state = [&](int gjob) {
        uint4 *dst = reinterpret_cast<uint4 *>(stage_base(gjob));
        const uint4 *src = reinterpret_cast<const uint4 *>(g_lds);
        for (int i = tid; i < (int)(kPersistBytes / 16); i += kThreads) dst[i] = src[i];
    };
    static_assert(kPersistBytes + kMaxReq * (sizeof(Req) + sizeof(u64)) <= SVT_HIP_ME_STAGE_BYTES, "a block's record holds its state, its requests and their results");
    auto export_reqs = [&](int gjob) {
        uint4 *dst = reinterpret_cast<uint4 *>(stage_base(gjob) + kPersistBytes);
        const uint4 *src = reinterpret_cast<const uint4 *>(st.req);
        static_assert(sizeof(Req) == 24 && (kMaxReq * sizeof(Req)) % 16 == 0, "requests are copied as 16-byte words");
        for (int i = tid; i < (int)(kMaxReq * sizeof(Req) / 16); i += kThreads) dst[i] = src[i];
    };
    auto keys_of = [&](int gjob) { return reinterpret_cast<u64 *>(stage_base(gjob) + kPersistBytes + kMaxReq * sizeof(Req)); };
    PROF_DECL;

    for (;;) {
        int gjob = 0;
        if (tid == 0) gjob = fetch_job();
        gjob = __builtin_amdgcn_readfirstlane(gjob);
        if (gjob < 0) break;
        PROF(0);
        int pic = 0;
        while (pic + 1 < (int)hdr.n_pictures && (uint32_t)gjob >= hdr.job_base[pic + 1]) pic++;
        pic = __builtin_amdgcn_readfirstlane(pic);
        CParams &p = ((CParams *)gparams)[pic];
        auto &c = p.cfg;
        auto &d = p.desc;
        const int full_hme = (c.hme_search_method == 1);
        const int nl       = d.num_of_list_to_search;
        const bool mctf    = c.me_type == 1;
        const int job      = gjob - (int)hdr.job_base[pic];
        const uint32_t bxi = (uint32_t)job % p.w64, byi = p.row0 + (uint32_t)job / p.w64;
        const uint32_t b   = bxi + byi * p.w64;
        const int r0n      = d.num_of_ref_pic_to_search[0];
#define BEST_SAD(li, ri) (bsad + (((li) ? r0n : 0) + (ri)) * 85)
#define BEST_MV(li, ri) (bmv + (((li) ? r0n : 0) + (ri)) * 85)
        const int n_rows   = r0n + (nl > 1 ? d.num_of_ref_pic_to_search[1] : 0);
        uint32_t *const jflag = hdr.job_flags ? hdr.job_flags + gjob : nullptr;
        if constexpr (me_is_search(MODE)) {
            constexpr int lvl = MODE == kMeS1 ? 1 : 2, parts = lvl == 1 ? 3 : 5;
            static_assert(offsetof(St, req) == kPersistBytes && offsetof(St, nreq) >= kPersistBytes - 16, "nreq sits in the last 16-byte word of the record's head, the requests behind it");
            static_assert(kSrc32Pitch == 3 * 16 && kSrc64Pitch == 5 * 16, "a view row is its pieces and one piece of padding");
            lds_dma_after_stores();
            lds_dma_copy(stage_base(gjob) + kPersistBytes - 16, g_lds, (uint32_t)(kPersistBytes - 16), 1 + (int)(kMaxReq * sizeof(Req) / 16));
            const int ox = (int)(bxi * 64) >> (2 - lvl), oy = (int)(byi * 64) >> (2 - lvl), rstep = 1 << cshift, npiece = ((lvl == 1 ? 32 : 64) >> cshift) * parts;
            for (int b0 = 0; b0 < npiece; b0 += kThreads) {
                const int n = b0 + tid, row = n / parts, cc = n - row * parts;
                if (n < npiece && cc < parts - 1) lds_dma_load16(plane_at(p.cur.lvl[lvl], ox + cc * 16, oy + row * rstep), g_lds, (lvl == 1 ? lay.src32 : lay.src64) + (uint32_t)b0 * 16);
            }
            const uint32_t f = __hip_atomic_load(jflag, __ATOMIC_RELAXED, __HIP_MEMORY_SCOPE_AGENT);
            lds_dma_wait();
            if (f & SVT_HIP_ME_JOB_DEFERRED) continue;
        } else if constexpr (kImports) {
            static_assert(offsetof(St, req_key) % 16 == 0 && kPersistBytes <= offsetof(St, req) + 8 && offsetof(St, req) + 8 <= offsetof(St, req_key), "the record's parts land on 16-byte words of their own");
            static_assert(kSrc64Pitch == 5 * 16, "a view row is four pieces and one piece of padding");
            lds_dma_after_stores();
            lds_dma_copy(stage_base(gjob), g_lds, 0, (int)(kPersistBytes / 16));
            lds_dma_copy(reinterpret_cast<const uint8_t *>(keys_of(gjob)), g_lds, (uint32_t)offsetof(St, req_key), (int)(kMaxReq * sizeof(u64) / 16));
            if constexpr (MODE == kMeTail) {
                const int ox = (int)(bxi * 64), oy = (int)(byi * 64), rstep = 1 << cshift, npiece = (64 >> cshift) * 5;
                for (int b0 = 0; b0 < npiece; b0 += kThreads) {
                    const int n = b0 + tid, row = n / 5, cc = n - row * 5;
                    if (n < npiece && cc < 4) lds_dma_load16(plane_at(p.cur.lvl[2], ox + cc * 16, oy + row * rstep), g_lds, lay.src64 + (uint32_t)b0 * 16);
                }
            }
            const uint32_t f = __hip_atomic_load(jflag, __ATOMIC_RELAXED, __HIP_MEMORY_SCOPE_AGENT);
            if constexpr (MODE == kMeTail)
                for (int i = tid; i < n_rows * 85; i += kThreads) { bmv[i] = 0; bsad[i] = SVT_HIP_MAX_SAD_VALUE; }
            if (tid == 0) { st.nme = 0; st.nprobe = 0; }
            lds_dma_wait();
            if (f & SVT_HIP_ME_JOB_DEFERRED) continue;
        }
        if constexpr (me_is_search(MODE)) {
            PROF(24);
            wave_sync();
            PROF(25);
            if (st.nreq) {
                (void)run_small_searches_direct<SVT_HIP_ME_SEARCH_DEPTH, MODE == kMeS1>(sh PROF_ARG);
            }
            wave_sync();
            u64 *keys = keys_of(gjob);
            if (tid < kMaxReq) keys[tid] = st.req_key[tid];
            wave_sync();
            continue;
        }

        if constexpr (!kImports) {
        if (tid == 0) {
            st.b64_index = b;
            st.org_x = bxi * 64; st.org_y = byi * 64;
            st.b64_w = (uint32_t)(d.aligned_width - st.org_x) < 64 ? d.aligned_width - st.org_x : 64;
            st.b64_h = (uint32_t)(d.aligned_height - st.org_y) < 64 ? d.aligned_height - st.org_y : 64;
            st.hme_l0_sa.sa_min.width = (uint16_t)c.hme_l0_sa.sa_min.width; st.hme_l0_sa.sa_min.height = (uint16_t)c.hme_l0_sa.sa_min.height;
            st.hme_l0_sa.sa_max.width = (uint16_t)c.hme_l0_sa.sa_max.width; st.hme_l0_sa.sa_max.height = (uint16_t)c.hme_l0_sa.sa_max.height;
            st.nreq = 0; st.nme = 0; st.nprobe = 0;
        }
        for (int i = tid; i < 3 * 2 * 4 * 2 * 2; i += kThreads) { (&st.hx[0][0][0][0][0])[i] = 0; (&st.hy[0][0][0][0][0])[i] = 0; (&st.hs[0][0][0][0][0])[i] = 0; }
        if constexpr (MODE == kMeFull)
            for (int i = tid; i < n_rows * 85; i += kThreads) { bmv[i] = 0; bsad[i] = SVT_HIP_MAX_SAD_VALUE; }
        if (tid < 8) {
            const int li = tid >> 2, ri = tid & 3;
            st.do_ref[li][ri] = 1; st.hme_sad64[li][ri] = 0xFFFFFFFFull; st.sr_divisor[li][ri] = 1; st.zz_sad[li][ri] = ~0u;
            st.hme_sc_x[li][ri] = st.hme_sc_y[li][ri] = 0;
            for (int sri = 0; sri < 2; sri++) {
                PreHme &ph = st.prehme[li][ri][sri];
                ph.valid = 0; ph.col = ph.row = 0; ph.sad = 0; ph.sa_w = ph.sa_h = 0;
                st.performed_phme[li][ri][sri] = 0;
            }
        }
        }
        if ((MODE == kMeFull || MODE == kMeMid1) && has_dense && tid < n_rows * kDenseKinds)
            reinterpret_cast<uint4 *>(g_lds + lay.dense)[tid] = reinterpret_cast<const uint4 *>(hdr.dense)[((size_t)gjob * hdr.n_slot) * kDenseKinds + tid];
        const bool zz_on = (MODE == kMeFull || MODE == kMeMid1) && (c.me_early_exit_th || c.me_safe_limit_zz_th);
        const int  nzz   = zz_on ? r0n + ((nl > 1 && d.temporal_layer_index > 0) ? d.num_of_ref_pic_to_search[1] : 0) : 0;
        uint32_t   zz_sum[8] = {0, 0, 0, 0, 0, 0, 0, 0};
        {
            const int ox = (int)(bxi * 64), oy = (int)(byi * 64), rstep = 1 << cshift;
            const int bw64 = imin(64, (int)d.aligned_width - ox), bh64 = imin(64, (int)d.aligned_height - oy);
            if constexpr (!kImports)
            for (int i = tid; i < (64 >> cshift) * 4; i += kThreads) {
                const int row = i >> 2, cc = i & 3;
                uint4 v; memcpy(&v, plane_at(p.cur.lvl[2], ox + cc * 16, oy + row * rstep), 16);
                if constexpr (MODE != kMeMid1) *reinterpret_cast<uint4 *>(&LDS(sh.src64)[row * kSrc64Pitch + cc * 16]) = v;
                const int y = row * rstep, x = cc * 16;
                if (nzz && !(y & 1) && y < bh64 && x < bw64) {
                    const bool whole = x + 8 < bw64;
#pragma unroll
                    for (int k = 0; k < 8; k++)
                        if (k < nzz) {
                            const int li = k < r0n ? 0 : 1, ri = k < r0n ? k : k - r0n;
                            uint4 w; memcpy(&w, plane_at(p.ref[li][ri].lvl[2], ox + x, oy + y), 16);
                            uint32_t a = __builtin_amdgcn_sad_u8(v.x, w.x, zz_sum[k]);
                            a = __builtin_amdgcn_sad_u8(v.y, w.y, a);
                            if (whole) { a = __builtin_amdgcn_sad_u8(v.z, w.z, a); a = __builtin_amdgcn_sad_u8(v.w, w.w, a); }
                            zz_sum[k] = a;
                        }
                }
            }
            if constexpr (MODE == kMeFull) {
                for (int i = tid; i < (32 >> cshift) * 2; i += kThreads) {
                    const int row = i >> 1, cc = i & 1;
                    uint4 v; memcpy(&v, plane_at(p.cur.lvl[1], (ox >> 1) + cc * 16, (oy >> 1) + row * rstep), 16);
                    *reinterpret_cast<uint4 *>(&LDS(sh.src32)[row * kSrc32Pitch + cc * 16]) = v;
                }
                for (int i = tid; i < (16 >> cshift); i += kThreads) {
                    uint4 v; memcpy(&v, plane_at(p.cur.lvl[0], ox >> 2, (oy >> 2) + i * rstep), 16);
                    *reinterpret_cast<uint4 *>(&LDS(sh.src16)[i * kSrc16Pitch]) = v;
                }
            }
        }
#pragma unroll
        for (int k = 0; k < 8; k++)
            if (k < nzz) {
                const uint32_t t = wave_sum_dpp(zz_sum[k]);
                if (tid == 0) st.req_key[k] = (u64)t << 32;
            }
        wave_sync();

        PROF(1);
        auto zz_pre = [&]() {
            if (tid == 0) st.nreq = 0;
        };
        auto zz_post = [&]() {
            const int  li = (tid >> 2) & 1, ri = tid & 3;
            const bool valid = tid < 8 && li < nl && ri < d.num_of_ref_pic_to_search[li];
            const bool srch  = valid && searched(p, li);
            const u64  smask = __ballot(srch);
            uint32_t   z = 0xFFFFFFFFu;
            if (srch) {
                const int k = __popcll(smask & ((1ull << tid) - 1ull));
                z = (uint32_t)(st.req_key[k] >> 32) << 1;
                z = (z * 64 * 64) / (st.b64_w * st.b64_h);
                st.zz_sad[li][ri] = z;
            }
            const uint32_t best = wave_min_dpp(z);
            if (d.temporal_layer_index > 0 && best < c.zz_sad_th && valid && ri >= 1)
                if ((uint32_t)((z - best) * 100) > (uint32_t)(c.zz_sad_pct * best)) st.do_ref[li][ri] = 0;
            if (c.me_safe_limit_zz_th) {
                wave_sync();
                const bool limit = d.hierarchical_levels > 0 && nl == 2 && d.temporal_layer_index >= d.hierarchical_levels &&
                    d.similar_brightness_refs && st.zz_sad[0][0] < c.me_safe_limit_zz_th && st.zz_sad[1][0] < c.me_safe_limit_zz_th;
                if (limit && valid && ri >= 1) st.do_ref[li][ri] = 0;
            }
        };
        auto prehme_pre = [&](int bi) {
            const int  l_lo = c.prehme_l1_early_exit ? bi : 0, l_hi = c.prehme_l1_early_exit ? bi + 1 : nl;
            const int  li = (tid >> 3) & 1, ri = (tid >> 1) & 3, sri = tid & 1;
            const bool mine = tid < 16 && li >= l_lo && li < l_hi && ri < d.num_of_ref_pic_to_search[li];
            bool       push = false;
            if (mine) {
                st.ph_req[li][ri][sri] = 0;
                if (searched(p, li)) {
                    PreHme &ph = st.prehme[li][ri][sri];
                    bool    handled = false;
                    if (c.me_early_exit_th && st.zz_sad[li][ri] < c.me_early_exit_th) { ph.col = ph.row = 0; ph.sad = 0; ph.valid = 1; handled = true; }
                    if (!handled && c.prehme_l1_early_exit) {
                        const PreHme &q = st.prehme[0][ri][sri];
                        if (li == 1 && q.valid && (q.sad < 32 * 32 || (iabs(q.col) < 16 && iabs(q.row) < 16))) {
                            ph.col = (int16_t)-q.col; ph.row = (int16_t)-q.row; ph.sad = q.sad; ph.valid = 1; handled = true;
                        }
                    }
                    if (!handled && !st.do_ref[li][ri]) { ph.col = ph.row = 0; ph.sad = 0xFFFFFFFFu; handled = true; }
                    push = !handled;
                }
            }
            const u64 mask = __ballot(push);
            const int slot = __popcll(mask & ((1ull << tid) - 1ull));
            if (push) {
                PreHme &ph = st.prehme[li][ri][sri];
                CPlane &rp = p.ref[li][ri].lvl[0];
                const int ox16 = (int16_t)st.org_x >> 2, oy16 = (int16_t)st.org_y >> 2;
                const SearchGeo sg = prehme_geometry(p, li, ri, sri, st.org_x, st.org_y);
                push_hme_req(st, p, 0, rp, ox16, oy16, (int)st.b64_w >> 2, (int)st.b64_h >> 2, sg.ox, sg.oy, sg.sa_w, sg.sa_h, c.prehme_skip_search_line, slot);
                st.ph_req[li][ri][sri] = (uint8_t)(slot + 1);
                dense_take(st, dense_lds, (((li ? r0n : 0) + ri) * kDenseKinds + sri), slot, sg, n_hit, n_miss);
                ph.col = (int16_t)sg.ox; ph.row = (int16_t)sg.oy;
                st.performed_phme[li][ri][sri] = 1;
            }
            if (tid == 0) st.nreq = __popcll(mask);
        };
        auto prehme_post = [&](int bi) {
            const int  l_lo = c.prehme_l1_early_exit ? bi : 0, l_hi = c.prehme_l1_early_exit ? bi + 1 : nl;
            const int  li = (tid >> 3) & 1, ri = (tid >> 1) & 3, sri = tid & 1;
            const bool mine = tid < 16 && li >= l_lo && li < l_hi && ri < d.num_of_ref_pic_to_search[li];
            const int  k = mine ? st.ph_req[li][ri][sri] : 0;
            if (k) {
                PreHme &ph = st.prehme[li][ri][sri];
                uint32_t sad; int x, y;
                key_to_result(st.req_key[k - 1], full_hme, sad, x, y);
                ph.sad = sad;
                ph.col = (int16_t)((int16_t)(x + ph.col) * 4);
                ph.row = (int16_t)((int16_t)(y + ph.row) * 4);
                ph.valid = 1;
            }
        };
        auto prehme_final = [&]() {
            wave_sync();
            const int  li = (tid >> 2) & 1, ri = tid & 3;
            const bool valid = tid < 8 && li < nl && ri < d.num_of_ref_pic_to_search[li];
            uint32_t   m = 0xFFFFFFFFu;
            if (valid) {
                if (searched(p, li)) {
                    m = st.prehme[li][ri][0].sad < st.prehme[li][ri][1].sad ? st.prehme[li][ri][0].sad : st.prehme[li][ri][1].sad;
                } else {
                    for (int sri = 0; sri < 2; sri++) {
                        st.prehme[1][ri][sri].col = (int16_t)-st.prehme[0][ri][sri].col;
                        st.prehme[1][ri][sri].row = (int16_t)-st.prehme[0][ri][sri].row;
                        st.prehme[1][ri][sri].sad = st.prehme[0][ri][sri].sad;
                    }
                }
            }
            const uint32_t best_sad = wave_min_dpp(m);
            if (d.temporal_layer_index > 0 && best_sad < c.phme_sad_th && valid && ri >= 1 && st.do_ref[li][ri])
                if ((uint32_t)((m - best_sad) * 100) > (uint32_t)(c.phme_sad_pct * best_sad)) st.do_ref[li][ri] = 0;
        };
        const bool l0_dep = c.enable_me_sr_adjustment && c.distance_based_hme_resizing && c.reduce_hme_l0_sr_th_min && c.reduce_hme_l0_sr_th_max;
        auto region_of = [&](int lane, int &li, int &ri, int &h, int &w) { li = lane >> 4; ri = (lane >> 2) & 3; h = (lane >> 1) & 1; w = lane & 1; };
        auto set_region = [&](int lvl, int li, int ri, int w, int h, int x, int y, uint32_t sad) {
            st.hx[lvl][li][ri][w][h] = (int16_t)x; st.hy[lvl][li][ri][w][h] = (int16_t)y; st.hs[lvl][li][ri][w][h] = sad;
        };
        auto l0_pre = [&](int bi) {
            const bool dep = l0_dep;
            if (tid < 64) {
                int li, ri, h, w;
                region_of(tid, li, ri, h, w);
                bool push = false;
                int  sa_w = 0, sa_h = 0;
                const bool mine = tid < 32 && li < nl && ri < d.num_of_ref_pic_to_search[li] && !(dep && ((li == 0 && ri == 0) != (bi == 0)));
                if (mine) {
                    if (h == 0 && w == 0) st.l0_req[li][ri] = 0;
                    bool handled = false;
                    if (c.me_early_exit_th && st.zz_sad[li][ri] < (c.me_early_exit_th >> 2)) { set_region(0, li, ri, w, h, 0, 0, 0); handled = true; }
                    if (!handled && c.prev_me_stage_based_exit_th) {
                        const int sri = st.prehme[li][ri][0].sad <= st.prehme[li][ri][1].sad ? 0 : 1;
                        if (st.performed_phme[li][ri][sri] && st.prehme[li][ri][sri].sad < (c.prev_me_stage_based_exit_th >> 4)) {
                            set_region(0, li, ri, w, h, st.prehme[li][ri][sri].col, st.prehme[li][ri][sri].row, st.prehme[li][ri][sri].sad);
                            handled = true;
                        }
                    }
                    if (!handled && !st.do_ref[li][ri]) { set_region(0, li, ri, w, h, 0, 0, 0xFFFFFFFFu); handled = true; }
                    if (!handled && searched(p, li)) {
                        hme_l0_search_area(st, p, li, ri, ref_distance(p, li, ri), sa_w, sa_h);
                        push = true;
                    }
                }
                const u64 mask = __ballot(push);
                const int slot = __popcll(mask & ((1ull << tid) - 1ull));
                if (push) {
                    const HmeGeom g = push_hme_level(st, p, 0, p.ref[li][ri].lvl[0], (int16_t)st.org_x >> 2, (int16_t)st.org_y >> 2, (int)st.b64_w >> 2,
                                                     (int)st.b64_h >> 2, sa_w, sa_h, 0, 0, w, h, slot);
                    st.hx[0][li][ri][w][h] = g.ox; st.hy[0][li][ri][w][h] = g.oy;
                    if (h == 0 && w == 0) st.l0_req[li][ri] = (uint8_t)(slot + 1);
                    const SearchGeo sg = {g.ox, g.oy, st.req[slot].sa_w, st.req[slot].sa_h};
                    dense_take(st, dense_lds, (((li ? r0n : 0) + ri) * kDenseKinds + 2 + h * 2 + w), slot, sg, n_hit, n_miss);
                }
                if (tid == 0) st.nreq = __popcll(mask);
            }
        };
        auto l0_post = [&](int bi) {
            const bool dep = l0_dep;
            if (tid < 64) {
                int li, ri, h, w;
                region_of(tid, li, ri, h, w);
                const bool mine = tid < 32 && li < nl && ri < d.num_of_ref_pic_to_search[li] && !(dep && ((li == 0 && ri == 0) != (bi == 0)));
                const int  k0   = mine ? st.l0_req[li][ri] : 0;
                if (k0) {
                    uint32_t sad; int x, y;
                    key_to_result(st.req_key[k0 - 1 + h * 2 + w], full_hme, sad, x, y);
                    st.hs[0][li][ri][w][h] = sad;
                    st.hx[0][li][ri][w][h] = (int16_t)((int16_t)(x + st.hx[0][li][ri][w][h]) * 4);
                    st.hy[0][li][ri][w][h] = (int16_t)((int16_t)(y + st.hy[0][li][ri][w][h]) * 4);
                }
                wave_sync();
                if (k0 && h == 0 && w == 0 && c.prehme_enable) {
                    int ww = 0, wh = 0; uint32_t mx = 0;
                    if (st.hs[0][li][ri][0][0] > mx) { mx = st.hs[0][li][ri][0][0]; ww = 0; wh = 0; }
                    if (st.hs[0][li][ri][1][0] > mx) { mx = st.hs[0][li][ri][1][0]; ww = 1; wh = 0; }
                    if (st.hs[0][li][ri][0][1] > mx) { mx = st.hs[0][li][ri][0][1]; ww = 0; wh = 1; }
                    if (st.hs[0][li][ri][1][1] > mx) { ww = 1; wh = 1; }
                    const int sri = st.prehme[li][ri][0].sad <= st.prehme[li][ri][1].sad ? 0 : 1;
                    if (st.prehme[li][ri][sri].sad < st.hs[0][li][ri][ww][wh]) {
                        st.hs[0][li][ri][ww][wh] = st.prehme[li][ri][sri].sad;
                        st.hx[0][li][ri][ww][wh] = st.prehme[li][ri][sri].col;
                        st.hy[0][li][ri][ww][wh] = st.prehme[li][ri][sri].row;
                    }
                }
            }
        };
        auto lvl_pre = [&](int lvl) {
            if (tid < 64) {
                int li, ri, h, w;
                region_of(tid, li, ri, h, w);
                bool push = false;
                if (tid < 32) st.lvl_req[li][ri][w][h] = 0;
                if (tid < 32 && li < nl && ri < d.num_of_ref_pic_to_search[li] && searched(p, li)) {
                    bool live = true;
                    if (lvl == 1) {
                        if (c.me_early_exit_th && st.zz_sad[li][ri] < (c.me_early_exit_th >> 2)) { set_region(1, li, ri, w, h, 0, 0, 0); live = false; }
                        else if (!st.do_ref[li][ri]) { set_region(1, li, ri, w, h, 0, 0, 0xFFFFFFFFu); live = false; }
                    }
                    if (live) {
                        const uint32_t exit_th = c.prev_me_stage_based_exit_th >> (lvl == 1 ? 5 : 2);
                        if (c.prev_me_stage_based_exit_th && st.hs[lvl - 1][li][ri][w][h] < exit_th)
                            set_region(lvl, li, ri, w, h, st.hx[lvl - 1][li][ri][w][h], st.hy[lvl - 1][li][ri][w][h], st.hs[lvl - 1][li][ri][w][h]);
                        else push = true;
                    }
                }
                const u64 mask = __ballot(push);
                const int slot = __popcll(mask & ((1ull << tid) - 1ull));
                if (push) {
                    HmeGeom g;
                    if (lvl == 1)
                        g = push_hme_level(st, p, 1, p.ref[li][ri].lvl[1], (int16_t)st.org_x >> 1, (int16_t)st.org_y >> 1, (int)st.b64_w >> 1,
                                           (int)st.b64_h >> 1, (int16_t)c.hme_l1_sa.width, (int16_t)c.hme_l1_sa.height,
                                           st.hx[0][li][ri][w][h] >> 1, st.hy[0][li][ri][w][h] >> 1, 0, 0, slot);
                    else
                        g = push_hme_level(st, p, 2, p.ref[li][ri].lvl[2], (int16_t)st.org_x, (int16_t)st.org_y, (int)st.b64_w, (int)st.b64_h,
                                           (int16_t)c.hme_l2_sa.width, (int16_t)c.hme_l2_sa.height, st.hx[1][li][ri][w][h],
                                           st.hy[1][li][ri][w][h], 0, 0, slot);
                    st.lvl_req[li][ri][w][h] = (uint8_t)(slot + 1);
                    st.hx[lvl][li][ri][w][h] = g.ox; st.hy[lvl][li][ri][w][h] = g.oy;
                }
                if (tid == 0) st.nreq = __popcll(mask);
            }
        };
        auto lvl_post = [&](int lvl) {
            if (tid < 32) {
                int li, ri, h, w;
                region_of(tid, li, ri, h, w);
                const int scale = (lvl == 1) ? 2 : 1;
                const int k = (li < nl && ri < d.num_of_ref_pic_to_search[li]) ? st.lvl_req[li][ri][w][h] : 0;
                if (k) {
                    uint32_t sad; int x, y;
                    key_to_result(st.req_key[k - 1], full_hme, sad, x, y);
                    st.hs[lvl][li][ri][w][h] = sad;
                    st.hx[lvl][li][ri][w][h] = (int16_t)((int16_t)(x + st.hx[lvl][li][ri][w][h]) * scale);
                    st.hy[lvl][li][ri][w][h] = (int16_t)((int16_t)(y + st.hy[lvl][li][ri][w][h]) * scale);
                }
            }
        };
        auto centre = [&]() {
            {
                const int  li = (tid >> 2) & 1, ri = tid & 3;
                const bool valid = tid < 8 && li < nl && ri < d.num_of_ref_pic_to_search[li];
                const bool srch  = valid && searched(p, li);
                int16_t sx = 0, sy = 0;
                u64     hme_sad = 0;
                if (srch && c.enable_hme_flag) {
                    int16_t cx = 0, cy = 0;
                    int lvl = -1;
                    if (c.enable_hme_level0_flag && !c.enable_hme_level1_flag && !c.enable_hme_level2_flag) lvl = 0;
                    if (c.enable_hme_level1_flag && !c.enable_hme_level2_flag) lvl = 1;
                    if (c.enable_hme_level2_flag) lvl = 2;
                    if (lvl >= 0) {
                        cx = st.hx[lvl][li][ri][0][0]; cy = st.hy[lvl][li][ri][0][0]; hme_sad = st.hs[lvl][li][ri][0][0];
                        int w = 1;
                        for (int h = 0; h < c.num_hme_sa_h; h++) {
                            for (; w < c.num_hme_sa_w; w++)
                                if (st.hs[lvl][li][ri][w][h] < hme_sad) {
                                    cx = st.hx[lvl][li][ri][w][h]; cy = st.hy[lvl][li][ri][w][h]; hme_sad = st.hs[lvl][li][ri][w][h];
                                }
                            w = 0;
                        }
                    }
                    sx = cx; sy = cy;
                }
                const int last0 = d.num_of_ref_pic_to_search[0] - 1;
                const u64 carry = ((u64)(uint32_t)__shfl((int)(uint32_t)(hme_sad >> 32), last0, 64) << 32) | (uint32_t)__shfl((int)(uint32_t)hme_sad, last0, 64);
                if (valid && !srch) hme_sad = carry;
                if (valid) { st.hme_sc_x[li][ri] = sx; st.hme_sc_y[li][ri] = sy; st.hme_sad64[li][ri] = hme_sad; }
                if (tid == 0) st.tf_exit = mctf && hme_sad < (u64)d.tf_me_exit_th;
            }
            if (c.enable_hme_flag && !mctf) {
                wave_sync();
                const int  li = (tid >> 2) & 1, ri = tid & 3;
                const bool slot = tid < 8;
                const u64  hs = slot ? st.hme_sad64[li][ri] : ~0ull;
                const uint16_t th = c.prune_ref_if_hme_sad_dev_bigger_than_th;
                if (c.enable_me_hme_ref_pruning && th != 0xFFFF) {
                    const u64 best = (u64)wave_min_dpp((uint32_t)(hs < 0xFFFFFFFFull ? hs : 0xFFFFFFFFull));
                    if (slot && ri >= 1 && (hs - best) * 100 > (u64)th * best) st.do_ref[li][ri] = 0;
                }
                if (c.enable_me_sr_adjustment && slot) {
                    if (iabs(st.hme_sc_x[li][ri]) <= c.reduce_me_sr_based_on_mv_length_th && iabs(st.hme_sc_y[li][ri]) <= c.reduce_me_sr_based_on_mv_length_th &&
                        hs < c.stationary_hme_sad_abs_th)
                        st.sr_divisor[li][ri] = c.stationary_me_sr_divisor;
                    else if (hs < c.reduce_me_sr_based_on_hme_sad_abs_th)
                        st.sr_divisor[li][ri] = c.me_sr_divisor_for_low_hme_sad;
                }
                wave_sync();
            }
        };
        const bool me_dep = (!c.me_early_exit_th) && c.enable_me_sr_adjustment == 2;
        auto c00_pre = [&](int gi) {
            const bool dep = me_dep;
            const int  li = (tid >> 2) & 1, ri = tid & 3;
            const bool mine = tid < 8 && li < nl && ri < d.num_of_ref_pic_to_search[li] && !(dep && ((li == 0 && ri == 0) != (gi == 0)));
            bool    push = false;
            int16_t cx = 0, cy = 0;
            if (mine) {
                st.c00_req[li][ri] = 0;
                cx = st.hme_sc_x[li][ri]; cy = st.hme_sc_y[li][ri];
                st.me_cx[li][ri] = cx; st.me_cy[li][ri] = cy;
                push = !(c.me_early_exit_th || !st.do_ref[li][ri]) && (cx != 0 || cy != 0) && d.is_ref;
            }
            const u64 mask = __ballot(push);
            const int slot = 2 * __popcll(mask & ((1ull << tid) - 1ull));
            if (push) {
                CPlane &rp = p.ref[li][ri].lvl[2];
                const int ox = (int16_t)st.org_x, oy = (int16_t)st.org_y;
                if (ox + cx < -63) cx = (int16_t)(-63 - ox);
                if (ox + cx > rp.width - 1) cx = (int16_t)(cx - ((ox + cx) - (rp.width - 1)));
                if (oy + cy < -63) cy = (int16_t)(-63 - oy);
                if (oy + cy > rp.height - 1) cy = (int16_t)(cy - ((oy + cy) - (rp.height - 1)));
                st.me_cx[li][ri] = cx; st.me_cy[li][ri] = cy;
                push_zz_req(st, rp, 0, 0, slot);
                push_zz_req(st, rp, cx, cy, slot + 1);
                st.c00_req[li][ri] = (uint8_t)(slot + 2);
            }
            if (tid == 0) st.nreq = 2 * __popcll(mask);
        };
        auto probe_pre = [&](int gi) {
            const bool dep = me_dep;
            const int  li = (tid >> 2) & 1, ri = tid & 3;
            const bool mine = tid < 8 && li < nl && ri < d.num_of_ref_pic_to_search[li] && !(dep && ((li == 0 && ri == 0) != (gi == 0))) && st.do_ref[li][ri];
            MeReq m = {};
            if (mine) {
                CPlane &rp = p.ref[li][ri].lvl[2];
                int16_t  cx = st.me_cx[li][ri], cy = st.me_cy[li][ri];
                const uint32_t dist = mctf ? (uint16_t)ref_distance(p, li, ri) : (uint16_t)scaled_distance(ref_distance(p, li, ri));
                int16_t sa_w = (int16_t)imin((int)(c.me_sa.sa_min.width * dist), c.me_sa.sa_max.width);
                int16_t sa_h = (int16_t)imin((int)(c.me_sa.sa_min.height * dist), c.me_sa.sa_max.height);
                if (c.mv_sa_adj_enabled && (!c.mv_sa_adj_nearest_ref_only || ri == 0)) {
                    if (iabs(st.hme_sc_x[li][ri]) > c.mv_sa_adj_mv_size_th) sa_w = (int16_t)(sa_w * c.mv_sa_adj_sa_multiplier);
                    if (iabs(st.hme_sc_y[li][ri]) > c.mv_sa_adj_mv_size_th) sa_h = (int16_t)(sa_h * c.mv_sa_adj_sa_multiplier);
                }
                { const uint32_t q = (uint32_t)(int)sa_w / st.sr_divisor[li][ri]; sa_w = (int16_t)(((q > 1u ? q : 1u) + 7) & ~7u); }
                { const uint32_t q = (uint32_t)(int)sa_h / st.sr_divisor[li][ri]; sa_h = (int16_t)(q > 3u ? q : 3u); }
                const int16_t h0 = sa_h, w0 = sa_w;
                u64 best_hme_sad = ~0ull;
                if (c.me_early_exit_th) {
                    if (st.zz_sad[li][ri] < c.me_early_exit_th / 6) sa_w = sa_h = 1;
                } else {
                    int accurate = 1;
                    const int k2 = st.c00_req[li][ri];
                    if (k2) {
                        const uint32_t zero = (uint32_t)(st.req_key[k2 - 2] >> 32) << 1;
                        const uint32_t hme  = (uint32_t)(st.req_key[k2 - 1] >> 32) << 1;
                        if (zero <= hme) cx = cy = 0;
                        best_hme_sad = hme;
                        if (cx == 0 && cy == 0) accurate = 0;
                    }
                    if (c.enable_me_sr_adjustment == 2) {
                        if ((accurate && best_hme_sad < 24 * 24) || (d.is_ref && st.hme_sad64[li][ri] < 24 * 24)) sa_h = (int16_t)(sa_h / 2);
                        if ((li || ri) && BEST_SAD(0, 0)[0] < 5000 && sa_h == h0 && sa_w == w0) { sa_h = (int16_t)(sa_h >> 1); sa_w = (int16_t)(sa_w >> 1); }
                    }
                }
                m.pix0 = plane_at(rp, (int)st.org_x, (int)st.org_y); m.stride = rp.stride;
                m.min_x = (int16_t)(-rp.org_x - (int)st.org_x); m.max_x = (int16_t)(rp.width + rp.org_x - 1 - (int)st.org_x);
                m.min_y = (int16_t)(-rp.org_y - (int)st.org_y); m.max_y = (int16_t)(rp.height + rp.org_y - 1 - (int)st.org_y);
                m.li = (uint8_t)li; m.ri = (uint8_t)ri; m.pad = 0;
                m.sa_w = sa_w; m.sa_h = sa_h;
                m.ox = cx; m.oy = cy;
                m.probe = (c.me_8x8_var_enabled && sa_w * sa_h > 24) ? 1 : 0;
            }
            const bool probe = mine && m.probe;
            const u64  mask = __ballot(mine), pmask = __ballot(probe), below = (1ull << tid) - 1ull;
            if (mine) st.me[__popcll(mask & below)] = m;
            if (probe) { MeReq pr = m; pr.sa_w = pr.sa_h = 1; st.me_probe[__popcll(pmask & below)] = pr; }
            if (tid == 0) { st.nme = __popcll(mask); st.nprobe = __popcll(pmask); }
        };
        auto main_pre = [&]() {
            if (tid < 64) {
                const int pic_w = (int16_t)d.aligned_width, pic_h = (int16_t)d.aligned_height;
                for (int i = 0; i < st.nme; i++) {
                    const MeReq m = st.me[i];
                    int16_t sa_w = m.sa_w, sa_h = m.sa_h;
                    const int cx = m.ox, cy = m.oy;
                    if (m.probe) {
                        const uint32_t mean = BEST_SAD(m.li, m.ri)[0] / 64;
                        const int32_t  dd   = (int32_t)BEST_SAD(m.li, m.ri)[21 + tid] - (int32_t)mean;
                        const uint32_t var  = wave_sum((uint32_t)(dd * dd)) / 64;
                        if (var > c.me_sr_mult2_th) { sa_w = (int16_t)((imax(1, sa_w * 3 / 2) + 7) & ~7); sa_h = (int16_t)imax(1, sa_h * 3 / 2); }
                        if (var < c.me_sr_div4_th) { sa_w = (int16_t)((imax(1, sa_w >> 2) + 7) & ~7); sa_h = (int16_t)imax(3, imax(1, sa_h >> 2)); }
                        else if (var < c.me_sr_div2_th) { sa_w = (int16_t)((imin(sa_w, sa_w >> 1) + 7) & ~7); sa_h = (int16_t)imax(3, imin(sa_h, sa_h >> 1)); }
                    }
                    int ox = (int16_t)(cx - (sa_w >> 1)), oy = (int16_t)(cy - (sa_h >> 1)), w = sa_w, h = sa_h;
                    clip_axis((int16_t)st.org_x, ox, w, 63, pic_w);
                    w = (w < 8) ? w : (w & ~7);
                    clip_axis((int16_t)st.org_y, oy, h, 63, pic_h);
                    if (tid == 0) { MeReq &o = st.me[i]; o.ox = (int16_t)ox; o.oy = (int16_t)oy; o.sa_w = (int16_t)w; o.sa_h = (int16_t)h; }
                }
            }
        };

        enum { kZz, kPrehme, kL0, kL1, kL2, kC00, kProbe, kMain, kEnd };
#ifdef SVT_ME_ABLATE
        if (SVT_ME_ABLATE == 1) continue;
#endif
        const int n_prehme = c.prehme_l1_early_exit ? nl : 1, n_l0 = l0_dep ? 2 : 1, n_group = me_dep ? 2 : 1;
        if constexpr (MODE == kMeMid1 || MODE == kMeMid2) {
            const bool hme_on = c.enable_hme_flag;
            bool defer = false;
            uint32_t flags = 0;
            if constexpr (MODE == kMeMid1) {
                auto pending = [&]() { return __any(tid < st.nreq && !st.req[tid].done); };
                if (c.me_early_exit_th || c.me_safe_limit_zz_th) { zz_pre(); wave_sync(); zz_post(); wave_sync(); }
                if (c.prehme_enable) {
                    for (int b2 = 0; b2 < n_prehme; b2++) {
                        prehme_pre(b2); wave_sync();
                        if (pending()) { defer = true; break; }
                        prehme_post(b2);
                        if (b2 + 1 < n_prehme) wave_sync();
                    }
                    if (!defer) { prehme_final(); wave_sync(); }
                }
                if (!defer && hme_on && c.enable_hme_level0_flag)
                    for (int b2 = 0; b2 < n_l0; b2++) {
                        l0_pre(b2); wave_sync();
                        if (pending()) { defer = true; break; }
                        l0_post(b2); wave_sync();
                    }
                if (!defer) {
                    if (hme_on && c.enable_hme_level1_flag) lvl_pre(1);
                    else if (tid == 0) st.nreq = 0;
                    wave_sync();
                }
            } else {
                flags = __hip_atomic_load(jflag, __ATOMIC_RELAXED, __HIP_MEMORY_SCOPE_AGENT);
                if (hme_on && c.enable_hme_level1_flag) { lvl_post(1); wave_sync(); }
                if (hme_on && c.enable_hme_level2_flag) lvl_pre(2);
                else if (tid == 0) st.nreq = 0;
                wave_sync();
            }
            if (!defer && st.nreq && !small_direct_ok(st)) defer = true;
            if (defer) {
                if (tid == 0) {
                    *jflag = SVT_HIP_ME_JOB_DEFERRED;
                    hdr.lists[0][atomicAdd(&hdr.queue_head[SVT_HIP_ME_LIST_COUNT(0)], 1u)] = (uint32_t)gjob;
                }
            } else {
                export_state(gjob);
                export_reqs(gjob);
                if (tid == 0) *jflag = flags;
            }
            wave_sync();
            continue;
        }
        if constexpr (MODE == kMeTail) {
            if (c.enable_hme_flag && c.enable_hme_level2_flag) { lvl_post(2); wave_sync(); }
        }
        int step = MODE == kMeTail ? kC00 : kZz, bi = 0;
        PROF(2);
        while (step != kEnd) {
            bool run = true;
            CTRL_PRIO(SVT_ME_CTRL_PRIO);
            switch (step) {
            case kZz: run = c.me_early_exit_th || c.me_safe_limit_zz_th; if (run) zz_pre(); break;
            case kPrehme: run = c.prehme_enable; if (run) prehme_pre(bi); break;
            case kL0: run = c.enable_hme_flag && c.enable_hme_level0_flag; if (run) l0_pre(bi); break;
            case kL1: run = c.enable_hme_flag && c.enable_hme_level1_flag; if (run) lvl_pre(1); break;
            case kL2: run = c.enable_hme_flag && c.enable_hme_level2_flag; if (run) lvl_pre(2); break;
            case kC00: if (bi == 0) centre(); c00_pre(bi); break;
            case kProbe: probe_pre(bi); break;
            default: main_pre(); break;
            }
#ifdef SVT_ME_ABLATE
            if (SVT_ME_ABLATE == 2 && step == kC00) break;
            if (SVT_ME_ABLATE >= 10 && step == SVT_ME_ABLATE - 10) break;
            if (SVT_ME_ABLATE == 4 && run && step < kProbe) { step = step == kPrehme ? kL0 : step + 1; bi = 0; continue; }
            if (SVT_ME_ABLATE == 5 && run && step < kProbe) st.nreq = 0;
#endif
            if (run) {
                CTRL_PRIO(0);
                wave_sync();
                PROF(step == kMain ? 20 : 6 + step);
                if (step == kC00 && bi == 0 && st.tf_exit) { step = kEnd; continue; }
                if constexpr (MODE == kMeTail) {
                    if (step == kC00) {
                        c00_sads(sh);
                        PROF(18);
                    } else if (step == kProbe) {
                        probe_sads(sh, p, bsad, bmv, r0n PROF_ARG);
                    } else {
                        run_me_searches(sh, p, st.me, st.nme, bsad, bmv, r0n PROF_ARG);
                    }
                } else if (step < kProbe) {
                    PROF_STEP(step);
                    if (st.nreq) {
                        if (!run_small_searches_direct<1, false, SVT_HIP_ME_DIRECT_RING_FULL != 0>(sh PROF_ARG)) run_searches(sh PROF_ARG);
                    }
                } else {
                    const bool   probe = step == kProbe;
                    const MeReq *list  = probe ? st.me_probe : st.me;
                    const int    count = probe ? st.nprobe : st.nme;
                    run_me_searches(sh, p, list, count, bsad, bmv, r0n PROF_ARG);
                }
                PROF(step == kProbe ? 3 : step == kMain ? 4 : 19);
            }
            CTRL_PRIO(SVT_ME_CTRL_PRIO);
            switch (step) {
            case kZz: if (run) zz_post(); step = kPrehme; break;
            case kPrehme:
                if (run) prehme_post(bi);
                if (run && bi + 1 < n_prehme) { bi++; break; }
                if (run) prehme_final();
                step = kL0; bi = 0;
                break;
            case kL0:
                if (run) l0_post(bi);
                if (run && bi + 1 < n_l0) { bi++; break; }
                step = kL1; bi = 0;
                break;
            case kL1: if (run) lvl_post(1); step = kL2; break;
            case kL2: if (run) lvl_post(2); step = kC00; break;
            case kC00: step = kProbe; break;
            case kProbe: step = kMain; break;
            default:
                if (bi + 1 < n_group) { bi++; step = kC00; } else step = kEnd;
                break;
            }
            CTRL_PRIO(0);
            wave_sync();
            PROF(5);
        }


#ifdef SVT_ME_ABLATE
        if (SVT_ME_ABLATE == 2 || SVT_ME_ABLATE == 3 || SVT_ME_ABLATE >= 10) continue;
#endif
        if (c.enable_hme_flag && c.enable_me_hme_ref_pruning && !mctf) {
            for (int r = 0; r < 8; r++) {
                const int li = r >> 2, ri = r & 3;
                if (li >= nl || ri >= d.num_of_ref_pic_to_search[li]) continue;
                const u64 t = st.do_ref[li][ri] ? (u64)wave_sum(BEST_SAD(li, ri)[21 + (tid & 63)]) : (u64)SVT_HIP_MAX_SAD_VALUE * 64;
                if ((tid & 63) == 0) st.hme_sad64[li][ri] = t;
            }
            wave_sync();
            {
                const uint16_t th = c.prune_ref_if_me_sad_dev_bigger_than_th;
                if (th != 0xFFFF) {
                    const int  li = (tid >> 2) & 1, ri = tid & 3;
                    const bool slot = tid < 8;
                    const u64  hs = slot ? st.hme_sad64[li][ri] : ~0ull;
                    const u64  best = (u64)wave_min_dpp((uint32_t)(hs < 0xFFFFFFFFull ? hs : 0xFFFFFFFFull));
                    if (slot && ri >= 1 && (hs - best) * 100 > (u64)th * best) st.do_ref[li][ri] = 0;
                }
            }
            wave_sync();
        }

        PROF(13);
        {
          if (!mctf) {
            const uint32_t n_pu = p.n_pu;
            uint8_t  *o_total = p.res.total_me_candidate_index + (size_t)b * n_pu;
            uint32_t *o_mv    = p.res.me_mv_array + (size_t)b * n_pu * d.max_refs;
            uint8_t  *o_cand  = p.res.me_candidate_array + (size_t)b * n_pu * d.max_cand;
            const int r0 = d.num_of_ref_pic_to_search[0], r1 = d.num_of_ref_pic_to_search[1];
            auto use_pu = [&](int nn) { return d.enable_me_16x16 ? (d.enable_me_8x8 || nn < 21) : nn < 5; };
            auto pack   = [](unsigned dir, unsigned i0, unsigned i1, unsigned l0, unsigned l1) {
                return (uint8_t)((dir & 3) | ((i0 & 3) << 2) | ((i1 & 3) << 4) | ((l0 & 1) << 6) | ((l1 & 1) << 7));
            };
            uint32_t *l_mv    = reinterpret_cast<uint32_t *>(LDS(sh.win));
            uint8_t  *l_cand  = LDS(sh.win) + 4 * n_pu * d.max_refs;
            uint8_t  *l_total = l_cand + n_pu * d.max_cand;
            const int stage_dwords = (int)(4 * n_pu * d.max_refs + n_pu * d.max_cand + n_pu + 3) >> 2;
            static_assert(kWinBytes >= 85 * (4 * SVT_HIP_MAX_LISTS * SVT_HIP_MAX_REFS + 32 + 1), "the result rows of one block fit the arena");
            for (int i = tid; i < stage_dwords; i += kThreads) reinterpret_cast<uint32_t *>(LDS(sh.win))[i] = 0;
            wave_sync();
            for (int n = tid; n < d.max_number_of_pus_per_sb; n += kThreads) {
                const int use = use_pu(n);
                const int row = (n > 4) ? c_z_to_raster[n] : n;
                uint8_t first = 0;
                auto put_cand = [&](int idx, uint8_t v) { l_cand[row * d.max_cand + idx] = v; if (idx == 0) first = v; };
                uint32_t  nls = nl;
                if (r0 == 1 && r1 == 0) {
                    const int pu   = c_z_to_raster[n];
                    st.me_dist[pu] = BEST_SAD(0, 0)[n];
                    if (use) l_total[pu] = 1;
                    if (st.do_ref[0][0] && use) { put_cand(0, pack(0, 0, 0, 0, 0)); l_mv[pu * d.max_refs] = BEST_MV(0, 0)[n]; }
                } else if (r0 == 1 && r1 == 1) {
                    const int     pu = c_z_to_raster[n];
                    const uint8_t d0 = st.do_ref[0][0], d1 = (nls == 1) ? 0 : st.do_ref[1][0];
                    if (nls < 2 || !st.do_ref[1][0]) nls = 1;
                    const uint32_t prune_th = (d0 && d1) ? (uint32_t)c.prune_me_candidates_th : 0;
                    uint8_t  blk[2] = {d0, d1};
                    uint8_t  off = 0;
                    const uint32_t s0 = BEST_SAD(0, 0)[n], s1 = BEST_SAD(1, 0)[n];
                    const uint32_t best = (d0 && d1) ? (s0 < s1 ? s0 : s1) : (d0 ? s0 : s1);
                    st.me_dist[pu] = best;
                    if (use) l_total[pu] = 1;
                    int min_list = -1;
                    if (c.use_best_unipred_cand_only && blk[0] && blk[1]) min_list = s0 < s1 ? 0 : 1;
                    for (uint32_t li = 0; li < nls && (use || off == 0); li++) {
                        if (!blk[li]) continue;
                        if (prune_th > 0) {
                            const uint32_t dev = (BEST_SAD(li, 0)[n] - best) * 100;
                            if (dev > best * prune_th) { blk[li] = 0; continue; }
                        }
                        if (min_list != -1 && min_list != (int)li) {
                            if (use) l_mv[pu * d.max_refs + (li ? d.max_l0 : 0)] = BEST_MV(li, 0)[n];
                            continue;
                        }
                        if (use) {
                            put_cand(off, pack(li, 0, 0, li == 0 ? li : 24, li == 1 ? li : 24));
                            l_mv[pu * d.max_refs + (li ? d.max_l0 : 0)] = BEST_MV(li, 0)[n];
                        }
                        off++;
                    }
                    if (blk[0] && blk[1] && use) { put_cand(off, pack(2, 0, 0, 0, 1)); l_total[pu] = (uint8_t)(off + 1); }
                } else {
                    const int pu = (n > 4) ? c_z_to_raster[n] : n;
                    uint8_t   off = 0;
                    uint8_t   blk[2][4] = {{0, 0, 0, 0}, {0, 0, 0, 0}};
                    const uint32_t prune_th = (uint32_t)c.prune_me_candidates_th;
                    uint32_t       best     = ~0u;
                    for (uint32_t li = 0; li < nls; li++)
                        for (int ri = 0; ri < d.num_of_ref_pic_to_search[li]; ri++) {
                            blk[li][ri] = st.do_ref[li][ri];
                            if (blk[li][ri]) best = BEST_SAD(li, ri)[n] < best ? BEST_SAD(li, ri)[n] : best;
                        }
                    st.me_dist[pu] = best;
                    for (uint32_t li = 0; li < nls && (use || off == 0); li++)
                        for (int ri = 0; ri < d.num_of_ref_pic_to_search[li] && (use || off == 0); ri++) {
                            if (!blk[li][ri]) continue;
                            if (prune_th > 0) {
                                const uint32_t dev = (BEST_SAD(li, ri)[n] - best) * 100;
                                if (dev > best * prune_th) { blk[li][ri] = 0; continue; }
                            }
                            if (use) {
                                put_cand(off, pack(li, ri, ri, li == 0 ? li : 24, li == 1 ? li : 24));
                                l_mv[pu * d.max_refs + (li ? d.max_l0 : 0) + ri] = BEST_MV(li, ri)[n];
                            }
                            off++;
                        }
                    if (nls == 2 && use) {
                        for (int a = 0; a < r0; a++)
                            for (int bb = 0; bb < r1; bb++) {
                                if (d.only_l_bwd && (a > 0 || bb > 0)) continue;
                                if (blk[0][a] && blk[1][bb]) put_cand(off++, pack(2, a, bb, 0, 1));
                            }
                        if (!d.only_l_bwd) {
                            for (int a = 1; a < r0; a++)
                                if (blk[0][0] && blk[0][a]) put_cand(off++, pack(2, 0, a, 0, 0));
                            if (r1 == 3 && blk[1][0] && blk[1][2]) put_cand(off++, pack(2, 0, 2, 1, 1));
                        }
                    }
                    if (use) l_total[pu] = off;
                }
                if (row < 88) st.cand0[row] = first;
            }
            wave_sync();
            for (int i = tid; i < (int)(n_pu * d.max_refs); i += kThreads) o_mv[i] = l_mv[i];
            for (int i = tid; i < (int)(n_pu * d.max_cand); i += kThreads) o_cand[i] = l_cand[i];
            for (int i = tid; i < (int)n_pu; i += kThreads) o_total[i] = l_total[i];

            PROF(14);
            if (tid < 64) {
                const uint32_t v8  = st.me_dist[21 + tid];
                const uint32_t d8  = wave_sum(v8);
                const uint32_t d16 = wave_sum(tid < 16 ? st.me_dist[5 + tid] : 0u);
                const uint32_t d32 = wave_sum(tid < 4 ? st.me_dist[1 + tid] : 0u);
                const u64       mean = d8 / 64;
                const long long dd   = (long long)v8 - (long long)mean;
                const u64       ssq  = wave_sum((u64)(dd * dd));
                uint8_t stationary = 0, allow_gm = 0;
                if (d.gm_enabled) {
                    const int low = d.input_resolution <= 2;
                    const int nn  = low ? 64 : 16;
                    int  refk = 0;
                    bool neg_x = false, pos_x = false, neg_y = false, pos_y = false, still_l = false;
                    if (tid < nn) {
                        int idx = (low ? 21 : 5) + tid;
                        if (low && !d.enable_me_8x8) {
                            if (idx >= 21) idx = c_8x8_to_16x16[idx - 21];
                            if (!d.enable_me_16x16 && idx >= 5) idx = c_16x16_to_32x32[idx - 5];
                        } else if (!low && !d.enable_me_16x16 && idx >= 5) idx = c_16x16_to_32x32[idx - 5];
                        const uint8_t  cb  = st.cand0[idx];
                        const unsigned dir = cb & 3;
                        const unsigned li  = (dir == 0 || dir == 2) ? ((cb >> 6) & 1) : ((cb >> 7) & 1);
                        const unsigned ri  = (dir == 0 || dir == 2) ? ((cb >> 2) & 3) : ((cb >> 4) & 3);
                        const u64 a = d.picture_number, bb = d.ref_picture_number[li][ri];
                        int th;
                        if (low) { const int dist = (uint16_t)iabs((int)(int16_t)((a > bb ? a : bb) - (a < bb ? a : bb))); th = d.gm_use_distance_based_active_th ? imax(dist >> 1, 4) : 4; }
                        else     { const int dist = (uint16_t)iabs((int)(int16_t)(a - bb)); th = d.gm_use_distance_based_active_th ? imax(dist * 16, 32) : 32; }
                        const uint32_t mv = BEST_MV(li, ri)[idx];
                        const int mx = (int)(int16_t)(mv & 0xFFFF) << 2, my = (int)(int16_t)(mv >> 16) << 2;
                        refk  = (int)(li * 4 + ri);
                        neg_x = mx < -th; pos_x = !neg_x && mx > th;
                        neg_y = my < -th; pos_y = !neg_y && my > th;
                        const int sth = low ? 0 : 4;
                        still_l = iabs(mx) <= sth && iabs(my) <= sth;
                    }
                    const uint32_t tot = (uint32_t)nn;
                    if ((uint32_t)__popcll(__ballot(still_l)) > (tot * 5) / 100) stationary = 1;
                    const u64 bnx = __ballot(neg_x), bpx = __ballot(pos_x), bny = __ballot(neg_y), bpy = __ballot(pos_y);
                    for (int k = 0; k < 8; k++) {
                        const u64 m = __ballot(tid < nn && refk == k);
                        if ((uint32_t)__popcll(m & bnx) > tot / 2 || (uint32_t)__popcll(m & bpx) > tot / 2 || (uint32_t)__popcll(m & bny) > tot / 2 ||
                            (uint32_t)__popcll(m & bpy) > tot / 2)
                            allow_gm = 1;
                    }
                }
              if (tid == 0) {
                const uint32_t pix = st.b64_w * st.b64_h;
                p.res.me_8x8_cost_variance[b] = (uint32_t)(ssq / 64);
                p.res.rc_me_distortion[b]     = d.input_resolution <= 2 ? d8 : d16;
                p.res.me_64x64_distortion[b]  = (st.me_dist[0] * 4096u) / pix;
                p.res.me_32x32_distortion[b]  = (d32 * 4096u) / pix;
                p.res.me_16x16_distortion[b]  = (d16 * 4096u) / pix;
                p.res.me_8x8_distortion[b]    = (d8 * 4096u) / pix;
                p.res.stationary_block_present_sb[b] = stationary;
                p.res.rc_me_allow_gm[b]              = allow_gm;
              }
            }
          }
            PROF(15);
            if (p.res.sb_best_sad || p.res.sb_best_mv)
                for (int i = tid; i < n_rows * 85; i += kThreads) {
                    const int row = i / 85, nn = i - row * 85, li = row < r0n ? 0 : 1, ri = row < r0n ? row : row - r0n;
                    const bool   ok = st.do_ref[li][ri] != 0;
                    const size_t o  = (size_t)b * 680 + (size_t)(li * 4 + ri) * 85 + nn;
                    if (p.res.sb_best_sad) p.res.sb_best_sad[o] = ok ? bsad[i] : SVT_HIP_MAX_SAD_VALUE;
                    if (p.res.sb_best_mv) p.res.sb_best_mv[o] = ok ? bmv[i] : 0;
                }
            if (tid < 8) {
                const int li = tid >> 2, ri = tid & 3;
                const bool live = li < nl && ri < d.num_of_ref_pic_to_search[li];
                if (p.res.do_ref) p.res.do_ref[(size_t)b * 8 + tid] = live ? st.do_ref[li][ri] : 0;
                if (p.res.hme_sad) p.res.hme_sad[(size_t)b * 8 + tid] = live ? (uint32_t)st.hme_sad64[li][ri] : 0;
                if (p.res.hme_sc) {
                    p.res.hme_sc[((size_t)b * 8 + tid) * 2]     = live ? st.hme_sc_x[li][ri] : 0;
                    p.res.hme_sc[((size_t)b * 8 + tid) * 2 + 1] = live ? st.hme_sc_y[li][ri] : 0;
                }
            }
        }
        wave_sync();
        PROF(16);
    }
#ifdef SVT_HIP_ME_PROFILE
#ifndef SVT_HIP_ME_PROFILE_MODE
#define SVT_HIP_ME_PROFILE_MODE 0
#endif
    if (MODE == SVT_HIP_ME_PROFILE_MODE) PROF_FLUSH(hdr.queue_head + 16);
#endif
    if ((MODE == kMeFull || MODE == kMeMid1) && has_dense && hdr.count_dense) {
        const uint32_t h = wave_sum_dpp(n_hit), m = wave_sum_dpp(n_miss);
        if (tid == 0) {
            atomicAdd(reinterpret_cast<unsigned long long *>(hdr.queue_head + SVT_HIP_ME_COUNTER_WORD), (unsigned long long)h);
            atomicAdd(reinterpret_cast<unsigned long long *>(hdr.queue_head + SVT_HIP_ME_COUNTER_WORD) + 1, (unsigned long long)m);
        }
    }
}

#undef BEST_SAD
#undef BEST_MV

#define SVT_ME_KERNEL(NAME, MODE, WAVES)                                                                                                              \
    extern "C" __global__ void __launch_bounds__(64, WAVES) NAME(const MeBatchHeader *__restrict__ ghdr, const MeKernelParams *__restrict__ gparams,   \
                                                                 const uint32_t launch_flags) {                                                       \
        me_b64_body<MODE>(ghdr, gparams, launch_flags);                                                                                               \
    }
SVT_ME_KERNEL(svt_hip_me_b64_kernel, kMeFull, SVT_HIP_ME_WAVES_PER_SIMD)
SVT_ME_KERNEL(svt_hip_me_mid1_kernel, kMeMid1, SVT_HIP_ME_MID_WAVES_PER_SIMD)
SVT_ME_KERNEL(svt_hip_me_s1_kernel, kMeS1, SVT_HIP_ME_SEARCH_WAVES_PER_SIMD)
SVT_ME_KERNEL(svt_hip_me_mid2_kernel, kMeMid2, SVT_HIP_ME_MID_WAVES_PER_SIMD)
SVT_ME_KERNEL(svt_hip_me_s2_kernel, kMeS2, SVT_HIP_ME_SEARCH_WAVES_PER_SIMD)
SVT_ME_KERNEL(svt_hip_me_tail_kernel, kMeTail, SVT_HIP_ME_TAIL_WAVES_PER_SIMD)
#undef SVT_ME_KERNEL

#include "me_dense.inl"

size_t svt_hip_me_kernel_lds_bytes(void) { return lds_layout(SVT_HIP_MAX_LISTS * SVT_HIP_MAX_REFS, 0, 1).total + SVT_HIP_ME_PROFILE_LDS; }

#include "svt_hip_internal.h"

int svt_hip_me_launch(SvtHipContext *ctx, SvtHipLane *lane, const MeKernelParams *params, const uint32_t *n_jobs, uint32_t n_pictures) {
    if (n_pictures == 0 || n_pictures > SVT_HIP_ME_MAX_PICTURES) return svt_hip_fail(ctx, SVT_HIP_ERR_BAD_PARAM, "%u pictures in one ME launch (1..%d)", n_pictures, SVT_HIP_ME_MAX_PICTURES);
    MeBatchHeader hdr;
    memset(&hdr, 0, sizeof(hdr));
    hdr.n_pictures = n_pictures;
    int all_sub = 1;
    for (uint32_t i = 0; i < n_pictures; i++) {
        hdr.job_base[i + 1] = hdr.job_base[i] + n_jobs[i];
        const uint32_t rows = (uint32_t)params[i].desc.num_of_ref_pic_to_search[0] + (params[i].desc.num_of_list_to_search > 1 ? (uint32_t)params[i].desc.num_of_ref_pic_to_search[1] : 0u);
        hdr.n_slot = rows > hdr.n_slot ? rows : hdr.n_slot;
        if (params[i].cfg.hme_search_method != 0 || params[i].cfg.me_search_method != 0) all_sub = 0;
    }
    hdr.cshift = (uint32_t)all_sub;
    for (uint32_t i = n_pictures; i < SVT_HIP_ME_MAX_PICTURES; i++) hdr.job_base[i + 1] = hdr.job_base[n_pictures];
    const uint32_t total = hdr.job_base[n_pictures];
    if (total == 0) return SVT_HIP_OK;
    for (int q = 0; q <= SVT_HIP_ME_QUEUES; q++) hdr.queue_begin[q] = (uint32_t)(((uint64_t)total * q) / SVT_HIP_ME_QUEUES);
    hdr.queue_head = lane->queue_head;
    SVT_HIP_CHECK(ctx, hipMemsetAsync(lane->queue_head, 0, SVT_HIP_ME_QUEUES * sizeof(uint32_t), lane->stream));
    static thread_local MeDenseEntry entries[SVT_HIP_ME_DENSE_MAX_ENTRIES];
    uint32_t n_entries = 0, n_units = 0;
    if (ctx->me_dense) n_entries = dense_plan(params, n_jobs, n_pictures, entries, &n_units, (uint32_t)ctx->num_cus * 4u * SVT_HIP_ME_DENSE_WAVES);
    auto grow = [&](void **buf, size_t *have, size_t need) -> int {
        if (need <= *have) return SVT_HIP_OK;
        if (*buf) {
            SVT_HIP_CHECK(ctx, hipStreamSynchronize(lane->stream));
            (void)hipFree(*buf);
            *buf = nullptr; *have = 0;
        }
        if (hipMalloc(buf, need) != hipSuccess) return svt_hip_fail(ctx, SVT_HIP_ERR_NO_MEMORY, "hipMalloc(%zu) failed (ME launch buffers)", need);
        *have = need;
        return SVT_HIP_OK;
    };
    if (n_units) {
        const size_t need = (size_t)total * hdr.n_slot * SVT_HIP_ME_DENSE_KINDS * sizeof(MeDenseSlot);
        if (int rc = grow(&lane->dense, &lane->dense_bytes, need)) return rc;
        SVT_HIP_CHECK(ctx, hipMemsetAsync(lane->dense, 0xFF, need, lane->stream));
        hdr.dense = static_cast<MeDenseSlot *>(lane->dense);
        hdr.n_dense_entries = n_entries; hdr.n_dense_units = n_units;
        hdr.count_dense = ctx->me_counting ? 1u : 0u;
    }
    const bool staged = n_units && (ctx->me_staged == 2 || (ctx->me_staged == 1 && total >= kStagedMinJobs));
    if (staged) {
        const size_t stage_bytes = (size_t)total * SVT_HIP_ME_STAGE_BYTES, words = (size_t)total * sizeof(uint32_t);
        if (int rc = grow(&lane->stage, &lane->stage_bytes, stage_bytes + 2 * words)) return rc;
        uint8_t *base = static_cast<uint8_t *>(lane->stage);
        hdr.stage     = base;
        hdr.job_flags = reinterpret_cast<uint32_t *>(base + stage_bytes);
        hdr.lists[0] = reinterpret_cast<uint32_t *>(base + stage_bytes + words);
        SVT_HIP_CHECK(ctx, hipMemsetAsync(lane->queue_head + 128, 0, SVT_HIP_ME_QUEUE_BLOCK_BYTES - 128 * sizeof(uint32_t), lane->stream));
    }
    if (!ctx->me_attr_set) {
        const void *kernels[] = {reinterpret_cast<const void *>(svt_hip_me_b64_kernel),  reinterpret_cast<const void *>(svt_hip_me_mid1_kernel), reinterpret_cast<const void *>(svt_hip_me_s1_kernel),
                                 reinterpret_cast<const void *>(svt_hip_me_mid2_kernel), reinterpret_cast<const void *>(svt_hip_me_s2_kernel),   reinterpret_cast<const void *>(svt_hip_me_tail_kernel)};
        for (const void *k : kernels) SVT_HIP_CHECK(ctx, hipFuncSetAttribute(k, hipFuncAttributeMaxDynamicSharedMemorySize, (int)svt_hip_me_kernel_lds_bytes()));
        ctx->me_attr_set = true;
    }
    const int slot = lane->ring_next;
    lane->ring_next = (slot + 1) % SVT_HIP_PARAM_RING;
    SVT_HIP_CHECK(ctx, hipEventSynchronize(lane->params_copied[slot]));
    uint8_t *host = lane->params_host[slot], *dev = lane->params_dev;
    memcpy(host, &hdr, sizeof(hdr));
    memcpy(host + SVT_HIP_ME_HEADER_BYTES, params, sizeof(MeKernelParams) * n_pictures);
    size_t block_bytes = SVT_HIP_ME_HEADER_BYTES + sizeof(MeKernelParams) * n_pictures;
    if (n_units) {
        memcpy(host + SVT_HIP_ME_ENTRIES_OFFSET, entries, sizeof(MeDenseEntry) * n_entries);
        block_bytes = SVT_HIP_ME_ENTRIES_OFFSET + sizeof(MeDenseEntry) * n_entries;
    }
    SVT_HIP_CHECK(ctx, hipMemcpyAsync(dev, host, block_bytes, hipMemcpyHostToDevice, lane->stream));
    SVT_HIP_CHECK(ctx, hipEventRecord(lane->params_copied[slot], lane->stream));
    const MeBatchHeader  *d_hdr = reinterpret_cast<const MeBatchHeader *>(dev);
    const MeKernelParams *d_par = reinterpret_cast<const MeKernelParams *>(dev + SVT_HIP_ME_HEADER_BYTES);
    const bool timing = ctx->me_timing;
    lane->me_marked = 0;
    auto mark = [&](int kernel) {
        if (!timing) return;
        const int i = kernel < 0 ? SVT_HIP_ME_CHAIN_KERNELS : kernel;
        if (!lane->me_mark[i]) hipEventCreate(&lane->me_mark[i]);
        hipEventRecord(lane->me_mark[i], lane->stream);
        if (kernel >= 0) lane->me_marked |= 1u << kernel;
    };
    if (n_units) {
        mark(0);
        hipLaunchKernelGGL(svt_hip_me_dense_kernel, dim3(n_units), dim3(64), 0, lane->stream, d_hdr, d_par, reinterpret_cast<const MeDenseEntry *>(dev + SVT_HIP_ME_ENTRIES_OFFSET));
        SVT_HIP_CHECK(ctx, hipGetLastError());
    }
    auto launch = [&](void (*kernel)(const MeBatchHeader *, const MeKernelParams *, uint32_t), int mode, uint32_t waves_per_simd, uint32_t flags) {
        const size_t lds = ((size_t)lds_layout((int)hdr.n_slot, (int)hdr.cshift, hdr.dense ? 1 : 0, mode).total + SVT_HIP_ME_PROFILE_LDS + 127) & ~(size_t)127;
        uint32_t per_cu = (uint32_t)((160u * 1024u) / lds);
        if (per_cu > 4u * waves_per_simd) per_cu = 4u * waves_per_simd;
        if (ctx->me_waves_per_cu && per_cu > ctx->me_waves_per_cu) per_cu = ctx->me_waves_per_cu;
        uint32_t grid = (uint32_t)ctx->num_cus * per_cu;
        if ((flags & 1u) && grid > (uint32_t)ctx->num_cus * kListWavesPerCu) grid = (uint32_t)ctx->num_cus * kListWavesPerCu;
        if (grid > total) grid = total;
        hipLaunchKernelGGL(kernel, dim3(grid), dim3(64), lds, lane->stream, d_hdr, d_par, flags);
    };
    if (staged) {
        mark(1); launch(svt_hip_me_mid1_kernel, kMeMid1, SVT_HIP_ME_MID_WAVES_PER_SIMD, 0u);
        mark(2); launch(svt_hip_me_s1_kernel, kMeS1, SVT_HIP_ME_SEARCH_WAVES_PER_SIMD, 0u);
        mark(3); launch(svt_hip_me_mid2_kernel, kMeMid2, SVT_HIP_ME_MID_WAVES_PER_SIMD, 0u);
        mark(4); launch(svt_hip_me_s2_kernel, kMeS2, SVT_HIP_ME_SEARCH_WAVES_PER_SIMD, 0u);
        mark(5); launch(svt_hip_me_tail_kernel, kMeTail, SVT_HIP_ME_TAIL_WAVES_PER_SIMD, 0u);
        mark(6); launch(svt_hip_me_b64_kernel, kMeFull, SVT_HIP_ME_WAVES_PER_SIMD, 1u);
    } else {
        mark(6); launch(svt_hip_me_b64_kernel, kMeFull, SVT_HIP_ME_WAVES_PER_SIMD, 0u);
    }
    mark(-1);
    SVT_HIP_CHECK(ctx, hipGetLastError());
    return SVT_HIP_OK;
}

static const char *const kChainKernelNames[SVT_HIP_ME_CHAIN_KERNELS] = {"svt_hip_me_dense_kernel", "svt_hip_me_mid1_kernel", "svt_hip_me_s1_kernel",  "svt_hip_me_mid2_kernel",
                                                                        "svt_hip_me_s2_kernel",    "svt_hip_me_tail_kernel", "svt_hip_me_b64_kernel"};
extern "C" const char *svt_hip_me_chain_kernel_name(int i) { return i >= 0 && i < SVT_HIP_ME_CHAIN_KERNELS ? kChainKernelNames[i] : nullptr; }

extern "C" int svt_hip_context_set_me_counting(SvtHipContext *ctx, int on) {
    if (!ctx) return SVT_HIP_ERR_BAD_PARAM;
    ctx->me_counting = on != 0;
    return SVT_HIP_OK;
}

extern "C" int svt_hip_context_set_me_timing(SvtHipContext *ctx, int on) {
    if (!ctx) return SVT_HIP_ERR_BAD_PARAM;
    ctx->me_timing = on != 0;
    return SVT_HIP_OK;
}

extern "C" int svt_hip_me_launch_times(SvtHipContext *ctx, float ms[SVT_HIP_ME_CHAIN_KERNELS]) {
    if (!ctx || !ms) return SVT_HIP_ERR_BAD_PARAM;
    SvtHipLane &l = ctx->lane[0];
    hipSetDevice(ctx->device);
    SVT_HIP_CHECK(ctx, hipStreamSynchronize(l.stream));
    for (int i = 0; i < SVT_HIP_ME_CHAIN_KERNELS; i++) {
        ms[i] = 0.f;
        if (!(l.me_marked >> i & 1u)) continue;
        int j = i + 1;
        while (j < SVT_HIP_ME_CHAIN_KERNELS && !(l.me_marked >> j & 1u)) j++;
        SVT_HIP_CHECK(ctx, hipEventElapsedTime(&ms[i], l.me_mark[i], l.me_mark[j]));
    }
    return SVT_HIP_OK;
}

extern "C" int svt_hip_context_set_me_staged(SvtHipContext *ctx, int on) {
    if (!ctx) return SVT_HIP_ERR_BAD_PARAM;
    if (on < 0 || on > 2) return svt_hip_fail(ctx, SVT_HIP_ERR_BAD_PARAM, "svt_hip_context_set_me_staged: %d is not 0 (off), 1 (large launches) or 2 (every launch)", on);
    ctx->me_staged = on;
    return SVT_HIP_OK;
}

extern "C" int svt_hip_context_set_me_dense(SvtHipContext *ctx, int on) {
    if (!ctx) return SVT_HIP_ERR_BAD_PARAM;
    ctx->me_dense = on != 0;
    return SVT_HIP_OK;
}

extern "C" int svt_hip_me_dense_counters(SvtHipContext *ctx, unsigned long long out[2]) {
    if (!ctx || !out) return SVT_HIP_ERR_BAD_PARAM;
    out[0] = out[1] = 0;
    hipSetDevice(ctx->device);
    for (int i = 0; i < SVT_HIP_LANES; i++) {
        SvtHipLane &l = ctx->lane[i];
        if (!l.ready) continue;
        unsigned long long v[2];
        SVT_HIP_CHECK(ctx, hipStreamSynchronize(l.stream));
        SVT_HIP_CHECK(ctx, hipMemcpy(v, l.queue_head + SVT_HIP_ME_COUNTER_WORD, sizeof(v), hipMemcpyDeviceToHost));
        SVT_HIP_CHECK(ctx, hipMemset(l.queue_head + SVT_HIP_ME_COUNTER_WORD, 0, sizeof(v)));
        out[0] += v[0]; out[1] += v[1];
    }
    return SVT_HIP_OK;
}

extern "C" int svt_hip_context_set_me_waves_per_cu(SvtHipContext *ctx, uint32_t waves) {
    if (!ctx) return SVT_HIP_ERR_BAD_PARAM;
    ctx->me_waves_per_cu = waves;
    return SVT_HIP_OK;
}
```

### svt-av1-psyex_amd/csrc/svt_hip_internal.h

```cpp
#ifndef SVT_HIP_INTERNAL_H
#define SVT_HIP_INTERNAL_H
#include <hip/hip_runtime_api.h>
#include <stdarg.h>
#include <stdio.h>
#include <condition_variable>
#include <mutex>
#include "me_kernel.h"

#define SVT_HIP_LANES 9
#define SVT_HIP_PARAM_RING 4

struct SvtHipLane {
    hipStream_t stream;
    uint32_t   *queue_head;
    uint8_t    *params_dev;
    uint8_t    *params_host[SVT_HIP_PARAM_RING];
    hipEvent_t  params_copied[SVT_HIP_PARAM_RING];
    int         ring_next;
    void       *scratch;
    size_t      scratch_bytes;
    void       *dense;
    size_t      dense_bytes;
    void       *stage;
    size_t      stage_bytes;
    hipEvent_t  me_mark[SVT_HIP_ME_CHAIN_KERNELS + 1];
    uint32_t    me_marked;
    bool        ready;
};

struct SvtHipContext {
    int         device;
    int         num_cus;
    hipStream_t stream;
    SvtHipLane  lane[SVT_HIP_LANES];
    std::mutex  async_mu;
    std::mutex  pool_mu;
    std::condition_variable pool_cv;
    uint32_t    lane_busy;
    int16_t    *iscan_dev;
    bool        me_attr_set;
    int         me_staged;
    bool        me_counting;
    bool        me_timing;
    bool        me_dense;
    uint32_t    me_waves_per_cu;
    hipStream_t io_stream;
    hipEvent_t  io_fence;
    void       *tpl_scratch;
    size_t      tpl_scratch_bytes;
    void       *tpl_group_dev;
    void       *tpl_group_host;
    hipEvent_t  tpl_group_done[4];
    int         tpl_group_next;
};

struct SvtHipPaPicture {
    DevPyramid  pyr;
    void       *mem[3];
    size_t      bytes[3];
    hipEvent_t  ready;
    hipStream_t ready_stream;
};

char *svt_hip_err_buf(void);
#define SVT_HIP_ERR_BYTES 512

static inline int svt_hip_fail(SvtHipContext *, int code, const char *fmt, ...) {
    va_list ap;
    va_start(ap, fmt);
    vsnprintf(svt_hip_err_buf(), SVT_HIP_ERR_BYTES, fmt, ap);
    va_end(ap);
    return code;
}

#define SVT_HIP_CHECK(ctx, call)                                                                                  \
    do {                                                                                                          \
        hipError_t e_ = (call);                                                                                   \
        if (e_ != hipSuccess)                                                                                     \
            return svt_hip_fail(ctx, SVT_HIP_ERR_LAUNCH, "%s failed: %s (%s:%d)", #call, hipGetErrorString(e_), \
                                __FILE__, __LINE__);                                                              \
    } while (0)

class SvtHipLaneGuard {
public:
    explicit SvtHipLaneGuard(SvtHipContext *ctx);
    ~SvtHipLaneGuard();
    SvtHipLane *lane() const { return lane_; }
private:
    SvtHipContext *ctx_;
    SvtHipLane    *lane_;
    int            index_;
};
int svt_hip_lane_setup(SvtHipContext *ctx, SvtHipLane *l, bool make_stream);
int svt_hip_wait_picture(SvtHipContext *ctx, hipStream_t stream, const SvtHipPaPicture *pic);

size_t svt_hip_me_kernel_lds_bytes(void);
int    svt_hip_me_launch(SvtHipContext *ctx, SvtHipLane *lane, const MeKernelParams *params, const uint32_t *n_jobs, uint32_t n_pictures);
int    svt_hip_me_pictures_on_lane(SvtHipContext *ctx, SvtHipLane *lane, uint32_t n_pictures, const SvtHipMeJob *jobs);
int    svt_hip_scratch(SvtHipContext *ctx, SvtHipLane *lane, size_t bytes, void **out);
__attribute__((visibility("hidden"))) hipError_t svt_hip_hadamard_launch(SvtHipContext *ctx, const int16_t *src, int stride, int n, int32_t *coeff);
int    svt_hip_rd_tables_init(SvtHipContext *ctx);
void   svt_hip_rd_tables_free(SvtHipContext *ctx);
int    svt_hip_tpl_tables_init(SvtHipContext *ctx);
void   svt_hip_tpl_free(SvtHipContext *ctx);
struct SvtHipTplDesc;
int    svt_hip_tpl_dispense_locked(SvtHipContext *ctx, const SvtHipTplDesc *d);
#define SVT_HIP_TPL_GROUP_RING 4
void   svt_hip_tpl_group_free(SvtHipContext *ctx);
#endif
```

Baseline: 45290 Mpixels/s.

## Cache per-picture reference descriptors in LDS and trim the ME epilogue

Each persistent ME wave now builds an LDS table of per-reference plane descriptors, distances, liveness, search flags and pre-HME sizes once per picture. Later stages read this table instead of recomputing them from constant-space parameters. The PU index maps are computed arithmetically instead of read from device tables, and the epilogue uses DPP wave sums, a shift-based divide for full 64x64 blocks, and later output copies. A max-waves launch cap knob is also exposed. The table uses extra LDS in full mode (or reuses tile entries in staged modes), which may affect occupancy.

```diff
diff --git a/include/svt_hip_me.h b/include/svt_hip_me.h
--- a/include/svt_hip_me.h
+++ b/include/svt_hip_me.h
@@ -120,6 +120,7 @@
 void *svt_hip_context_stream(SvtHipContext *ctx);
 int   svt_hip_context_sync(SvtHipContext *ctx);
 int   svt_hip_context_set_me_waves_per_cu(SvtHipContext *ctx, uint32_t waves);
+int   svt_hip_context_set_me_max_waves(SvtHipContext *ctx, uint32_t waves);
 int   svt_hip_context_set_me_dense(SvtHipContext *ctx, int on);
 int   svt_hip_context_set_me_staged(SvtHipContext *ctx, int on);
 #define SVT_HIP_ME_CHAIN_KERNELS 7
diff --git a/svt-av1-psyex_amd/api.py b/svt-av1-psyex_amd/api.py
--- a/svt-av1-psyex_amd/api.py
+++ b/svt-av1-psyex_amd/api.py
@@ -107,6 +107,12 @@
     def set_me_staged(self, on):
         self.check(lib().svt_hip_context_set_me_staged(self._h, int(on)), "svt_hip_context_set_me_staged")
 
+    def set_me_waves_per_cu(self, waves):
+        self.check(lib().svt_hip_context_set_me_waves_per_cu(self._h, int(waves)), "svt_hip_context_set_me_waves_per_cu")
+
+    def set_me_max_waves(self, waves):
+        self.check(lib().svt_hip_context_set_me_max_waves(self._h, int(waves)), "svt_hip_context_set_me_max_waves")
+
     def set_me_timing(self, on):
         self.check(lib().svt_hip_context_set_me_timing(self._h, 1 if on else 0), "svt_hip_context_set_me_timing")
 
diff --git a/svt-av1-psyex_amd/csrc/me_kernel.hip b/svt-av1-psyex_amd/csrc/me_kernel.hip
--- a/svt-av1-psyex_amd/csrc/me_kernel.hip
+++ b/svt-av1-psyex_amd/csrc/me_kernel.hip
@@ -34,6 +34,19 @@
 constexpr int kSrc64Pitch = 80, kSrc32Pitch = 48, kSrc16Pitch = 16;
 constexpr int kNarrowMaxPos = 32;
 
+#ifndef SVT_HIP_ME_REFTAB
+#define SVT_HIP_ME_REFTAB 1
+#endif
+#ifndef SVT_HIP_ME_REFTAB_FULL
+#define SVT_HIP_ME_REFTAB_FULL 1
+#endif
+#ifndef SVT_HIP_ME_CALC_MAPS
+#define SVT_HIP_ME_CALC_MAPS 1
+#endif
+#ifndef SVT_HIP_ME_LEAN_EPILOGUE
+#define SVT_HIP_ME_LEAN_EPILOGUE 1
+#endif
+
 __device__ const uint8_t c_z_to_raster[85] = {
     0,  1,  2,  3,  4,  5,  6,  9,  10, 7,  8,  11, 12, 13, 14, 17, 18, 15, 16, 19, 20, 21, 22, 29, 30, 23, 24, 31, 32,
     37, 38, 45, 46, 39, 40, 47, 48, 25, 26, 33, 34, 27, 28, 35, 36, 41, 42, 49, 50, 43, 44, 51, 52, 53, 54, 61, 62, 55,
@@ -42,6 +55,33 @@
                                                12, 12, 9,  9,  10, 10, 11, 11, 12, 12, 13, 13, 14, 14, 15, 15, 16, 16, 13, 13, 14, 14,
                                                15, 15, 16, 16, 17, 17, 18, 18, 19, 19, 20, 20, 17, 17, 18, 18, 19, 19, 20, 20};
 __device__ const uint8_t c_16x16_to_32x32[16] = {1, 1, 2, 2, 1, 1, 2, 2, 3, 3, 4, 4, 3, 3, 4, 4};
+
+__host__ __device__ constexpr int pu_z_to_raster(int n) {
+    if (n < 5) return n;
+    const int base = n < 21 ? 5 : 21, i = n - base, dim_log = n < 21 ? 2 : 3;
+    const int x = (i & 1) | ((i >> 1) & 2) | ((i >> 2) & 4), y = ((i >> 1) & 1) | ((i >> 2) & 2) | ((i >> 3) & 4);
+    return base + (y << dim_log) + x;
+}
+__host__ __device__ constexpr int pu_8x8_to_16x16(int i) { return 5 + ((i >> 4) << 2) + ((i & 7) >> 1); }
+__host__ __device__ constexpr int pu_16x16_to_32x32(int i) { return 1 + ((i >> 3) << 1) + ((i & 3) >> 1); }
+namespace map_proof {
+constexpr uint8_t z[85] = {0,  1,  2,  3,  4,  5,  6,  9,  10, 7,  8,  11, 12, 13, 14, 17, 18, 15, 16, 19, 20, 21, 22, 29, 30, 23, 24, 31, 32,
+                           37, 38, 45, 46, 39, 40, 47, 48, 25, 26, 33, 34, 27, 28, 35, 36, 41, 42, 49, 50, 43, 44, 51, 52, 53, 54, 61, 62, 55,
+                           56, 63, 64, 69, 70, 77, 78, 71, 72, 79, 80, 57, 58, 65, 66, 59, 60, 67, 68, 73, 74, 81, 82, 75, 76, 83, 84};
+constexpr uint8_t p16[64] = {5,  5,  6,  6,  7,  7,  8,  8,  5,  5,  6,  6,  7,  7,  8,  8,  9,  9,  10, 10, 11, 11, 12, 12, 9,  9,  10, 10, 11, 11, 12, 12,
+                             13, 13, 14, 14, 15, 15, 16, 16, 13, 13, 14, 14, 15, 15, 16, 16, 17, 17, 18, 18, 19, 19, 20, 20, 17, 17, 18, 18, 19, 19, 20, 20};
+constexpr uint8_t p32[16] = {1, 1, 2, 2, 1, 1, 2, 2, 3, 3, 4, 4, 3, 3, 4, 4};
+constexpr bool equal() {
+    for (int n = 0; n < 85; n++) if (pu_z_to_raster(n) != z[n]) return false;
+    for (int i = 0; i < 64; i++) if (pu_8x8_to_16x16(i) != p16[i]) return false;
+    for (int i = 0; i < 16; i++) if (pu_16x16_to_32x32(i) != p32[i]) return false;
+    return true;
+}
+static_assert(equal(), "the computed PU maps are the reference's tables (motion_estimation.c:2520-2531, definitions.h:2613-2632)");
+}
+__device__ __forceinline__ int z_to_raster(int n) { return SVT_HIP_ME_CALC_MAPS ? pu_z_to_raster(n) : (int)c_z_to_raster[n]; }
+__device__ __forceinline__ int parent_16x16(int i) { return SVT_HIP_ME_CALC_MAPS ? pu_8x8_to_16x16(i) : (int)c_8x8_to_16x16[i]; }
+__device__ __forceinline__ int parent_32x32(int i) { return SVT_HIP_ME_CALC_MAPS ? pu_16x16_to_32x32(i) : (int)c_16x16_to_32x32[i]; }
 
 typedef unsigned long long u64;
 
@@ -121,6 +161,19 @@
     int      job, tf_exit;
 };
 
+struct RefEnt {
+    DevPlane lvl[3];
+    uint32_t dist, sdist;
+    uint16_t gm_dist;
+    uint8_t  live, srch;
+    int16_t  ph_w[2], ph_h[2];
+    uint32_t pad;
+};
+struct RefTab { RefEnt ent[SVT_HIP_MAX_LISTS * SVT_HIP_MAX_REFS]; };
+static_assert(SVT_HIP_MAX_LISTS == 2 && SVT_HIP_MAX_REFS == 4, "slot = li * 4 + ri, eight of them");
+static_assert(sizeof(RefTab) % 16 == 0 && sizeof(RefTab) <= 1024, "the table's budget: 1 KB of a wave's slice");
+__host__ __device__ constexpr bool me_has_reftab(int mode);
+
 struct LdsLayout { uint32_t src16, src32, src64, bsad, bmv, dense, win, total; };
 constexpr int kMeFull = 0, kMeMid1 = 1, kMeS1 = 2, kMeMid2 = 4, kMeS2 = 5, kMeTail = 7;
 #ifndef SVT_HIP_ME_LIST_WAVES_PER_CU
@@ -129,13 +182,25 @@
 constexpr uint32_t kListWavesPerCu = SVT_HIP_ME_LIST_WAVES_PER_CU;
 constexpr uint32_t kStagedMinJobs = 2048;
 __host__ __device__ constexpr bool me_is_search(int m) { return m == kMeS1 || m == kMeS2; }
+#ifndef SVT_HIP_ME_REFTAB_MID2
+#define SVT_HIP_ME_REFTAB_MID2 0
+#endif
+__host__ __device__ constexpr bool me_has_reftab(int m) {
+    return SVT_HIP_ME_REFTAB && (m == kMeFull ? SVT_HIP_ME_REFTAB_FULL != 0 : m == kMeMid2 ? SVT_HIP_ME_REFTAB_MID2 != 0 : !me_is_search(m));
+}
+constexpr uint32_t kStEnd = (uint32_t)((sizeof(St) + 15) & ~(size_t)15);
+__host__ __device__ constexpr bool me_reftab_in_tiles(int m) { return m != kMeFull; }
+__host__ __device__ constexpr uint32_t me_reftab_off(int m) { return me_reftab_in_tiles(m) ? (uint32_t)offsetof(St, tile) : kStEnd; }
+static_assert(offsetof(St, tile) % 16 == 0 && sizeof(RefTab) <= sizeof(TileEnt) * kMaxTiles, "the table fits the idle tile entries");
+static_assert(offsetof(St, tile) >= ((offsetof(St, req) + 15) & ~(size_t)15) + kMaxReq * sizeof(Req) && offsetof(St, tile) >= offsetof(St, req_key) + kMaxReq * sizeof(u64),
+              "no batch destination of the staged kernels (record head, requests, keys) reaches the tile entries");
 constexpr int kDirectWinBytes = 5120;
 __host__ __device__ constexpr LdsLayout lds_layout(int n_slot, int cshift, int dense = 1, int mode = 0) {
     const bool v16 = mode == kMeFull, v32 = mode == kMeFull || mode == kMeS1, v64 = mode == kMeFull || mode == kMeS2 || mode == kMeTail;
     const bool best = mode == kMeFull || mode == kMeTail, slots = dense && (mode == kMeFull || mode == kMeMid1);
     const uint32_t arena = (mode == kMeMid1 || mode == kMeMid2) ? 0u : (mode == kMeS1 || mode == kMeS2) ? (uint32_t)kDirectWinBytes : (uint32_t)kWinBytes;
     LdsLayout l = {};
-    l.src16 = (uint32_t)((sizeof(St) + 15) & ~(size_t)15);
+    l.src16 = kStEnd + (me_has_reftab(mode) && !me_reftab_in_tiles(mode) ? (uint32_t)sizeof(RefTab) : 0u);
     l.src32 = l.src16 + (v16 ? (uint32_t)((16 >> cshift) * kSrc16Pitch) : 0u);
     l.src64 = l.src32 + (v32 ? (uint32_t)((32 >> cshift) * kSrc32Pitch) : 0u);
     l.bsad  = l.src64 + (v64 ? (uint32_t)((64 >> cshift) * kSrc64Pitch) : 0u);
@@ -172,7 +237,7 @@
     if (org + origin + size > dim) size = imax(1, size - ((org + origin + size) - dim));
 }
 
-__device__ __forceinline__ const uint8_t *plane_at(CPlane &pl, int x, int y) {
+template <class PL> __device__ __forceinline__ const uint8_t *plane_at(PL &pl, int x, int y) {
     return pl.base + (long long)(pl.org_y + y) * pl.stride + (pl.org_x + x);
 }
 
@@ -922,7 +987,7 @@
     r.done      = 0;
 }
 
-__device__ __forceinline__ void push_hme_req(St &st, CParams &p, int level, CPlane &rp, int org_x, int org_y,
+template <class PL> __device__ __forceinline__ void push_hme_req(St &st, CParams &p, int level, PL &rp, int org_x, int org_y,
                                              int bw, int bh, int ox, int oy, int sa_w, int sa_h, int skip, int slot = -1) {
     const int full = (p.cfg.hme_search_method == 1);
     push_req(st, plane_at(rp, org_x + ox, org_y + oy), rp.stride, sa_w, sa_h, bw, full ? bh : (bh >> 1), full ? 1 : 2, level, skip, slot);
@@ -1228,10 +1293,7 @@
     sa_w = (int16_t)(uint16_t)imin((int)(c.prehme_sa_cfg[sri].sa_min.width * f), c.prehme_sa_cfg[sri].sa_max.width);
     sa_h = (int16_t)(uint16_t)imin((int)(c.prehme_sa_cfg[sri].sa_min.height * f), c.prehme_sa_cfg[sri].sa_max.height);
 }
-__device__ __forceinline__ SearchGeo prehme_geometry(CParams &p, int li, int ri, int sri, uint32_t org_x, uint32_t org_y) {
-    int sa_w, sa_h;
-    prehme_size(p, li, ri, sri, sa_w, sa_h);
-    CPlane &rp = p.ref[li][ri].lvl[0];
+template <class PL> __device__ __forceinline__ SearchGeo prehme_geometry_sized(PL &rp, int sa_w, int sa_h, uint32_t org_x, uint32_t org_y) {
     const int ox16 = (int16_t)org_x >> 2, oy16 = (int16_t)org_y >> 2;
     int ox = -(int16_t)(sa_w >> 1), oy = -(int16_t)(sa_h >> 1);
     clip_axis(ox16, ox, sa_w, rp.org_x - 1, rp.width);
@@ -1239,8 +1301,13 @@
     SearchGeo g = {ox, oy, sa_w, sa_h};
     return g;
 }
-
-__device__ __forceinline__ SearchGeo hme_level_geometry(CParams &p, int level, CPlane &rp, int org_x, int org_y, int sa_w, int sa_h, int cx, int cy, int sr_w, int sr_h) {
+__device__ __forceinline__ SearchGeo prehme_geometry(CParams &p, int li, int ri, int sri, uint32_t org_x, uint32_t org_y) {
+    int sa_w, sa_h;
+    prehme_size(p, li, ri, sri, sa_w, sa_h);
+    return prehme_geometry_sized(p.ref[li][ri].lvl[0], sa_w, sa_h, org_x, org_y);
+}
+
+template <class PL> __device__ __forceinline__ SearchGeo hme_level_geometry(CParams &p, int level, PL &rp, int org_x, int org_y, int sa_w, int sa_h, int cx, int cy, int sr_w, int sr_h) {
     sa_w = (int16_t)((sa_w + 7) & ~7);
     int pad_w, pad_h, ox, oy;
     if (level == 2) { pad_w = pad_h = 63; } else { pad_w = rp.org_x - 1; pad_h = rp.org_y - 1; }
@@ -1260,7 +1327,24 @@
 
 struct HmeGeom { int16_t ox, oy; };
 
-__device__ HmeGeom push_hme_level(St &st, CParams &p, int level, CPlane &rp, int org_x, int org_y, int bw, int bh,
+__device__ __forceinline__ uint32_t ctrl_sum32(uint32_t v) { return SVT_HIP_ME_LEAN_EPILOGUE ? wave_sum_dpp(v) : wave_sum(v); }
+__device__ __forceinline__ u64 ctrl_sum64(u64 v) {
+    if (!SVT_HIP_ME_LEAN_EPILOGUE) return wave_sum(v);
+    const u64 lo = wave_sum_dpp((uint32_t)v & 0xFFFFFFu), mid = wave_sum_dpp((uint32_t)(v >> 24) & 0xFFFFFFu), hi = wave_sum_dpp((uint32_t)(v >> 48));
+    return (hi << 48) + (mid << 24) + lo;
+}
+
+template <bool MASK> struct RefFlags {
+    uint32_t m = 0;
+    uint8_t  a[2][4] = {{0, 0, 0, 0}, {0, 0, 0, 0}};
+    __device__ __forceinline__ bool get(int li, int ri) const { if constexpr (MASK) return (m >> (li * 4 + ri)) & 1u; else return a[li][ri] != 0; }
+    __device__ __forceinline__ void set(int li, int ri, bool v) {
+        if constexpr (MASK) m = (m & ~(1u << (li * 4 + ri))) | ((uint32_t)v << (li * 4 + ri));
+        else a[li][ri] = (uint8_t)v;
+    }
+};
+
+template <class PL> __device__ __forceinline__ HmeGeom push_hme_level(St &st, CParams &p, int level, PL &rp, int org_x, int org_y, int bw, int bh,
                                   int sa_w, int sa_h, int cx, int cy, int sr_w, int sr_h, int slot = -1) {
     const SearchGeo sg = hme_level_geometry(p, level, rp, org_x, org_y, sa_w, sa_h, cx, cy, sr_w, sr_h);
     push_hme_req(st, p, level, rp, org_x, org_y, bw, bh, sg.ox, sg.oy, sg.sa_w, sg.sa_h, 0, slot);
@@ -1275,7 +1359,7 @@
     if (!full) sad *= 2;
 }
 
-__device__ __forceinline__ void push_zz_req(St &st, CPlane &rp, int dx, int dy, int slot = -1) {
+template <class PL> __device__ __forceinline__ void push_zz_req(St &st, PL &rp, int dx, int dy, int slot = -1) {
     push_req(st, plane_at(rp, (int)st.org_x + dx, (int)st.org_y + dy), rp.stride, 1, 1, (int)st.b64_w, (int)st.b64_h >> 1, 2, 2, 0, slot);
 }
 
@@ -1292,6 +1376,9 @@
 __device__ __forceinline__ void me_b64_body(const MeBatchHeader *__restrict__ ghdr, const MeKernelParams *__restrict__ gparams, const uint32_t launch_flags) {
     St     &st = *reinterpret_cast<St *>(g_lds);
     constexpr bool kImports = MODE == kMeMid2 || MODE == kMeTail;
+    constexpr bool kTab = me_has_reftab(MODE);
+    RefTab &tab = *reinterpret_cast<RefTab *>(g_lds + me_reftab_off(MODE));
+    int tab_pic = -1;
     typedef const SVT_CONST_AS MeBatchHeader CHeader;
     CHeader  &hdr = *(CHeader *)ghdr;
     const int tid = threadIdx.x;
@@ -1385,6 +1472,41 @@
 #define BEST_MV(li, ri) (bmv + (((li) ? r0n : 0) + (ri)) * 85)
         const int n_rows   = r0n + (nl > 1 ? d.num_of_ref_pic_to_search[1] : 0);
         uint32_t *const jflag = hdr.job_flags ? hdr.job_flags + gjob : nullptr;
+        if constexpr (kTab) {
+            if (pic != tab_pic) {
+                tab_pic = pic;
+                if (tid < SVT_HIP_MAX_LISTS * SVT_HIP_MAX_REFS) {
+                    const int li = tid >> 2, ri = tid & 3;
+                    RefEnt &e = tab.ent[tid];
+#pragma unroll
+                    for (int k = 0; k < 3; k++) {
+                        CPlane &s = p.ref[li][ri].lvl[k];
+                        e.lvl[k].base = s.base; e.lvl[k].stride = s.stride;
+                        e.lvl[k].org_x = s.org_x; e.lvl[k].org_y = s.org_y; e.lvl[k].width = s.width; e.lvl[k].height = s.height;
+                    }
+                    const uint32_t dist = ref_distance(p, li, ri);
+                    e.dist = dist; e.sdist = scaled_distance(dist);
+                    const u64 a = d.picture_number, bb = d.ref_picture_number[li][ri];
+                    e.gm_dist = d.input_resolution <= 2 ? (uint16_t)iabs((int)(int16_t)((a > bb ? a : bb) - (a < bb ? a : bb))) : (uint16_t)iabs((int)(int16_t)(a - bb));
+                    e.live = (uint8_t)(li < nl && ri < (li ? d.num_of_ref_pic_to_search[1] : d.num_of_ref_pic_to_search[0]));
+                    e.srch = (uint8_t)searched(p, li);
+#pragma unroll
+                    for (int sri = 0; sri < 2; sri++) {
+                        int sa_w, sa_h;
+                        prehme_size(p, li, ri, sri, sa_w, sa_h);
+                        e.ph_w[sri] = (int16_t)sa_w; e.ph_h[sri] = (int16_t)sa_h;
+                    }
+                    e.pad = 0;
+                }
+                wave_sync();
+            }
+        }
+        auto ref_slot  = [](int li, int ri) { return (li * 4 + ri) & 7; };
+        auto ref_live  = [&](int li, int ri) -> bool { if constexpr (kTab) return tab.ent[ref_slot(li, ri)].live != 0; else return li < nl && ri < d.num_of_ref_pic_to_search[li]; };
+        auto ref_srch  = [&](int li, int ri) -> bool { if constexpr (kTab) return tab.ent[ref_slot(li, ri)].srch != 0; else return searched(p, li); };
+        auto ref_dist  = [&](int li, int ri) -> uint32_t { if constexpr (kTab) return tab.ent[ref_slot(li, ri)].dist; else return ref_distance(p, li, ri); };
+        auto ref_sdist = [&](int li, int ri) -> uint32_t { if constexpr (kTab) return tab.ent[ref_slot(li, ri)].sdist; else return scaled_distance(ref_distance(p, li, ri)); };
+        auto ref_plane = [&](int li, int ri, int k) -> decltype(auto) { if constexpr (kTab) return (tab.ent[ref_slot(li, ri)].lvl[k]); else return (p.ref[li][ri].lvl[k]); };
         if constexpr (me_is_search(MODE)) {
             constexpr int lvl = MODE == kMeS1 ? 1 : 2, parts = lvl == 1 ? 3 : 5;
             static_assert(offsetof(St, req) == kPersistBytes && offsetof(St, nreq) >= kPersistBytes - 16, "nreq sits in the last 16-byte word of the record's head, the requests behind it");
@@ -1511,8 +1633,8 @@
         };
         auto zz_post = [&]() {
             const int  li = (tid >> 2) & 1, ri = tid & 3;
-            const bool valid = tid < 8 && li < nl && ri < d.num_of_ref_pic_to_search[li];
-            const bool srch  = valid && searched(p, li);
+            const bool valid = tid < 8 && ref_live(li, ri);
+            const bool srch  = valid && ref_srch(li, ri);
             const u64  smask = __ballot(srch);
             uint32_t   z = 0xFFFFFFFFu;
             if (srch) {
@@ -1534,11 +1656,11 @@
         auto prehme_pre = [&](int bi) {
             const int  l_lo = c.prehme_l1_early_exit ? bi : 0, l_hi = c.prehme_l1_early_exit ? bi + 1 : nl;
             const int  li = (tid >> 3) & 1, ri = (tid >> 1) & 3, sri = tid & 1;
-            const bool mine = tid < 16 && li >= l_lo && li < l_hi && ri < d.num_of_ref_pic_to_search[li];
+            const bool mine = tid < 16 && li >= l_lo && li < l_hi && ref_live(li, ri);
             bool       push = false;
             if (mine) {
                 st.ph_req[li][ri][sri] = 0;
-                if (searched(p, li)) {
+                if (ref_srch(li, ri)) {
                     PreHme &ph = st.prehme[li][ri][sri];
                     bool    handled = false;
                     if (c.me_early_exit_th && st.zz_sad[li][ri] < c.me_early_exit_th) { ph.col = ph.row = 0; ph.sad = 0; ph.valid = 1; handled = true; }
@@ -1556,9 +1678,11 @@
             const int slot = __popcll(mask & ((1ull << tid) - 1ull));
             if (push) {
                 PreHme &ph = st.prehme[li][ri][sri];
-                CPlane &rp = p.ref[li][ri].lvl[0];
+                auto &rp = ref_plane(li, ri, 0);
                 const int ox16 = (int16_t)st.org_x >> 2, oy16 = (int16_t)st.org_y >> 2;
-                const SearchGeo sg = prehme_geometry(p, li, ri, sri, st.org_x, st.org_y);
+                SearchGeo sg;
+                if constexpr (kTab) sg = prehme_geometry_sized(rp, tab.ent[ref_slot(li, ri)].ph_w[sri], tab.ent[ref_slot(li, ri)].ph_h[sri], st.org_x, st.org_y);
+                else sg = prehme_geometry(p, li, ri, sri, st.org_x, st.org_y);
                 push_hme_req(st, p, 0, rp, ox16, oy16, (int)st.b64_w >> 2, (int)st.b64_h >> 2, sg.ox, sg.oy, sg.sa_w, sg.sa_h, c.prehme_skip_search_line, slot);
                 st.ph_req[li][ri][sri] = (uint8_t)(slot + 1);
                 dense_take(st, dense_lds, (((li ? r0n : 0) + ri) * kDenseKinds + sri), slot, sg, n_hit, n_miss);
@@ -1570,7 +1694,7 @@
         auto prehme_post = [&](int bi) {
             const int  l_lo = c.prehme_l1_early_exit ? bi : 0, l_hi = c.prehme_l1_early_exit ? bi + 1 : nl;
             const int  li = (tid >> 3) & 1, ri = (tid >> 1) & 3, sri = tid & 1;
-            const bool mine = tid < 16 && li >= l_lo && li < l_hi && ri < d.num_of_ref_pic_to_search[li];
+            const bool mine = tid < 16 && li >= l_lo && li < l_hi && ref_live(li, ri);
             const int  k = mine ? st.ph_req[li][ri][sri] : 0;
             if (k) {
                 PreHme &ph = st.prehme[li][ri][sri];
@@ -1585,10 +1709,10 @@
         auto prehme_final = [&]() {
             wave_sync();
             const int  li = (tid >> 2) & 1, ri = tid & 3;
-            const bool valid = tid < 8 && li < nl && ri < d.num_of_ref_pic_to_search[li];
+            const bool valid = tid < 8 && ref_live(li, ri);
             uint32_t   m = 0xFFFFFFFFu;
             if (valid) {
-                if (searched(p, li)) {
+                if (ref_srch(li, ri)) {
                     m = st.prehme[li][ri][0].sad < st.prehme[li][ri][1].sad ? st.prehme[li][ri][0].sad : st.prehme[li][ri][1].sad;
                 } else {
                     for (int sri = 0; sri < 2; sri++) {
@@ -1614,7 +1738,7 @@
                 region_of(tid, li, ri, h, w);
                 bool push = false;
                 int  sa_w = 0, sa_h = 0;
-                const bool mine = tid < 32 && li < nl && ri < d.num_of_ref_pic_to_search[li] && !(dep && ((li == 0 && ri == 0) != (bi == 0)));
+                const bool mine = tid < 32 && ref_live(li, ri) && !(dep && ((li == 0 && ri == 0) != (bi == 0)));
                 if (mine) {
                     if (h == 0 && w == 0) st.l0_req[li][ri] = 0;
                     bool handled = false;
@@ -1627,15 +1751,15 @@
                         }
                     }
                     if (!handled && !st.do_ref[li][ri]) { set_region(0, li, ri, w, h, 0, 0, 0xFFFFFFFFu); handled = true; }
-                    if (!handled && searched(p, li)) {
-                        hme_l0_search_area(st, p, li, ri, ref_distance(p, li, ri), sa_w, sa_h);
+                    if (!handled && ref_srch(li, ri)) {
+                        hme_l0_search_area(st, p, li, ri, ref_dist(li, ri), sa_w, sa_h);
                         push = true;
                     }
                 }
                 const u64 mask = __ballot(push);
                 const int slot = __popcll(mask & ((1ull << tid) - 1ull));
                 if (push) {
-                    const HmeGeom g = push_hme_level(st, p, 0, p.ref[li][ri].lvl[0], (int16_t)st.org_x >> 2, (int16_t)st.org_y >> 2, (int)st.b64_w >> 2,
+                    const HmeGeom g = push_hme_level(st, p, 0, ref_plane(li, ri, 0), (int16_t)st.org_x >> 2, (int16_t)st.org_y >> 2, (int)st.b64_w >> 2,
                                                      (int)st.b64_h >> 2, sa_w, sa_h, 0, 0, w, h, slot);
                     st.hx[0][li][ri][w][h] = g.ox; st.hy[0][li][ri][w][h] = g.oy;
                     if (h == 0 && w == 0) st.l0_req[li][ri] = (uint8_t)(slot + 1);
@@ -1650,7 +1774,7 @@
             if (tid < 64) {
                 int li, ri, h, w;
                 region_of(tid, li, ri, h, w);
-                const bool mine = tid < 32 && li < nl && ri < d.num_of_ref_pic_to_search[li] && !(dep && ((li == 0 && ri == 0) != (bi == 0)));
+                const bool mine = tid < 32 && ref_live(li, ri) && !(dep && ((li == 0 && ri == 0) != (bi == 0)));
                 const int  k0   = mine ? st.l0_req[li][ri] : 0;
                 if (k0) {
                     uint32_t sad; int x, y;
@@ -1681,7 +1805,7 @@
                 region_of(tid, li, ri, h, w);
                 bool push = false;
                 if (tid < 32) st.lvl_req[li][ri][w][h] = 0;
-                if (tid < 32 && li < nl && ri < d.num_of_ref_pic_to_search[li] && searched(p, li)) {
+                if (tid < 32 && ref_live(li, ri) && ref_srch(li, ri)) {
                     bool live = true;
                     if (lvl == 1) {
                         if (c.me_early_exit_th && st.zz_sad[li][ri] < (c.me_early_exit_th >> 2)) { set_region(1, li, ri, w, h, 0, 0, 0); live = false; }
@@ -1699,11 +1823,11 @@
                 if (push) {
                     HmeGeom g;
                     if (lvl == 1)
-                        g = push_hme_level(st, p, 1, p.ref[li][ri].lvl[1], (int16_t)st.org_x >> 1, (int16_t)st.org_y >> 1, (int)st.b64_w >> 1,
+                        g = push_hme_level(st, p, 1, ref_plane(li, ri, 1), (int16_t)st.org_x >> 1, (int16_t)st.org_y >> 1, (int)st.b64_w >> 1,
                                            (int)st.b64_h >> 1, (int16_t)c.hme_l1_sa.width, (int16_t)c.hme_l1_sa.height,
                                            st.hx[0][li][ri][w][h] >> 1, st.hy[0][li][ri][w][h] >> 1, 0, 0, slot);
                     else
-                        g = push_hme_level(st, p, 2, p.ref[li][ri].lvl[2], (int16_t)st.org_x, (int16_t)st.org_y, (int)st.b64_w, (int)st.b64_h,
+                        g = push_hme_level(st, p, 2, ref_plane(li, ri, 2), (int16_t)st.org_x, (int16_t)st.org_y, (int)st.b64_w, (int)st.b64_h,
                                            (int16_t)c.hme_l2_sa.width, (int16_t)c.hme_l2_sa.height, st.hx[1][li][ri][w][h],
                                            st.hy[1][li][ri][w][h], 0, 0, slot);
                     st.lvl_req[li][ri][w][h] = (uint8_t)(slot + 1);
@@ -1717,7 +1841,7 @@
                 int li, ri, h, w;
                 region_of(tid, li, ri, h, w);
                 const int scale = (lvl == 1) ? 2 : 1;
-                const int k = (li < nl && ri < d.num_of_ref_pic_to_search[li]) ? st.lvl_req[li][ri][w][h] : 0;
+                const int k = ref_live(li, ri) ? st.lvl_req[li][ri][w][h] : 0;
                 if (k) {
                     uint32_t sad; int x, y;
                     key_to_result(st.req_key[k - 1], full_hme, sad, x, y);
@@ -1730,8 +1854,8 @@
         auto centre = [&]() {
             {
                 const int  li = (tid >> 2) & 1, ri = tid & 3;
-                const bool valid = tid < 8 && li < nl && ri < d.num_of_ref_pic_to_search[li];
-                const bool srch  = valid && searched(p, li);
+                const bool valid = tid < 8 && ref_live(li, ri);
+                const bool srch  = valid && ref_srch(li, ri);
                 int16_t sx = 0, sy = 0;
                 u64     hme_sad = 0;
                 if (srch && c.enable_hme_flag) {
@@ -1783,7 +1907,7 @@
         auto c00_pre = [&](int gi) {
             const bool dep = me_dep;
             const int  li = (tid >> 2) & 1, ri = tid & 3;
-            const bool mine = tid < 8 && li < nl && ri < d.num_of_ref_pic_to_search[li] && !(dep && ((li == 0 && ri == 0) != (gi == 0)));
+            const bool mine = tid < 8 && ref_live(li, ri) && !(dep && ((li == 0 && ri == 0) != (gi == 0)));
             bool    push = false;
             int16_t cx = 0, cy = 0;
             if (mine) {
@@ -1795,7 +1919,7 @@
             const u64 mask = __ballot(push);
             const int slot = 2 * __popcll(mask & ((1ull << tid) - 1ull));
             if (push) {
-                CPlane &rp = p.ref[li][ri].lvl[2];
+                auto &rp = ref_plane(li, ri, 2);
                 const int ox = (int16_t)st.org_x, oy = (int16_t)st.org_y;
                 if (ox + cx < -63) cx = (int16_t)(-63 - ox);
                 if (ox + cx > rp.width - 1) cx = (int16_t)(cx - ((ox + cx) - (rp.width - 1)));
@@ -1811,12 +1935,12 @@
         auto probe_pre = [&](int gi) {
             const bool dep = me_dep;
             const int  li = (tid >> 2) & 1, ri = tid & 3;
-            const bool mine = tid < 8 && li < nl && ri < d.num_of_ref_pic_to_search[li] && !(dep && ((li == 0 && ri == 0) != (gi == 0))) && st.do_ref[li][ri];
+            const bool mine = tid < 8 && ref_live(li, ri) && !(dep && ((li == 0 && ri == 0) != (gi == 0))) && st.do_ref[li][ri];
             MeReq m = {};
             if (mine) {
-                CPlane &rp = p.ref[li][ri].lvl[2];
+                auto &rp = ref_plane(li, ri, 2);
                 int16_t  cx = st.me_cx[li][ri], cy = st.me_cy[li][ri];
-                const uint32_t dist = mctf ? (uint16_t)ref_distance(p, li, ri) : (uint16_t)scaled_distance(ref_distance(p, li, ri));
+                const uint32_t dist = mctf ? (uint16_t)ref_dist(li, ri) : (uint16_t)ref_sdist(li, ri);
                 int16_t sa_w = (int16_t)imin((int)(c.me_sa.sa_min.width * dist), c.me_sa.sa_max.width);
                 int16_t sa_h = (int16_t)imin((int)(c.me_sa.sa_min.height * dist), c.me_sa.sa_max.height);
                 if (c.mv_sa_adj_enabled && (!c.mv_sa_adj_nearest_ref_only || ri == 0)) {
@@ -1865,10 +1989,10 @@
                     const MeReq m = st.me[i];
                     int16_t sa_w = m.sa_w, sa_h = m.sa_h;
                     const int cx = m.ox, cy = m.oy;
-                    if (m.probe) {
+                    if (uni(m.probe)) {
                         const uint32_t mean = BEST_SAD(m.li, m.ri)[0] / 64;
                         const int32_t  dd   = (int32_t)BEST_SAD(m.li, m.ri)[21 + tid] - (int32_t)mean;
-                        const uint32_t var  = wave_sum((uint32_t)(dd * dd)) / 64;
+                        const uint32_t var  = ctrl_sum32((uint32_t)(dd * dd)) / 64;
                         if (var > c.me_sr_mult2_th) { sa_w = (int16_t)((imax(1, sa_w * 3 / 2) + 7) & ~7); sa_h = (int16_t)imax(1, sa_h * 3 / 2); }
                         if (var < c.me_sr_div4_th) { sa_w = (int16_t)((imax(1, sa_w >> 2) + 7) & ~7); sa_h = (int16_t)imax(3, imax(1, sa_h >> 2)); }
                         else if (var < c.me_sr_div2_th) { sa_w = (int16_t)((imin(sa_w, sa_w >> 1) + 7) & ~7); sa_h = (int16_t)imax(3, imin(sa_h, sa_h >> 1)); }
@@ -2021,7 +2145,7 @@
             for (int r = 0; r < 8; r++) {
                 const int li = r >> 2, ri = r & 3;
                 if (li >= nl || ri >= d.num_of_ref_pic_to_search[li]) continue;
-                const u64 t = st.do_ref[li][ri] ? (u64)wave_sum(BEST_SAD(li, ri)[21 + (tid & 63)]) : (u64)SVT_HIP_MAX_SAD_VALUE * 64;
+                const u64 t = uni(st.do_ref[li][ri]) ? (u64)ctrl_sum32(BEST_SAD(li, ri)[21 + (tid & 63)]) : (u64)SVT_HIP_MAX_SAD_VALUE * 64;
                 if ((tid & 63) == 0) st.hme_sad64[li][ri] = t;
             }
             wave_sync();
@@ -2059,33 +2183,34 @@
             wave_sync();
             for (int n = tid; n < d.max_number_of_pus_per_sb; n += kThreads) {
                 const int use = use_pu(n);
-                const int row = (n > 4) ? c_z_to_raster[n] : n;
+                const int row = (n > 4) ? z_to_raster(n) : n;
                 uint8_t first = 0;
                 auto put_cand = [&](int idx, uint8_t v) { l_cand[row * d.max_cand + idx] = v; if (idx == 0) first = v; };
                 uint32_t  nls = nl;
                 if (r0 == 1 && r1 == 0) {
-                    const int pu   = c_z_to_raster[n];
+                    const int pu   = z_to_raster(n);
                     st.me_dist[pu] = BEST_SAD(0, 0)[n];
                     if (use) l_total[pu] = 1;
                     if (st.do_ref[0][0] && use) { put_cand(0, pack(0, 0, 0, 0, 0)); l_mv[pu * d.max_refs] = BEST_MV(0, 0)[n]; }
                 } else if (r0 == 1 && r1 == 1) {
-                    const int     pu = c_z_to_raster[n];
+                    const int     pu = z_to_raster(n);
                     const uint8_t d0 = st.do_ref[0][0], d1 = (nls == 1) ? 0 : st.do_ref[1][0];
                     if (nls < 2 || !st.do_ref[1][0]) nls = 1;
                     const uint32_t prune_th = (d0 && d1) ? (uint32_t)c.prune_me_candidates_th : 0;
-                    uint8_t  blk[2] = {d0, d1};
+                    RefFlags<SVT_HIP_ME_LEAN_EPILOGUE != 0> blk;
+                    blk.set(0, 0, d0 != 0); blk.set(1, 0, d1 != 0);
                     uint8_t  off = 0;
                     const uint32_t s0 = BEST_SAD(0, 0)[n], s1 = BEST_SAD(1, 0)[n];
                     const uint32_t best = (d0 && d1) ? (s0 < s1 ? s0 : s1) : (d0 ? s0 : s1);
                     st.me_dist[pu] = best;
                     if (use) l_total[pu] = 1;
                     int min_list = -1;
-                    if (c.use_best_unipred_cand_only && blk[0] && blk[1]) min_list = s0 < s1 ? 0 : 1;
+                    if (c.use_best_unipred_cand_only && blk.get(0, 0) && blk.get(1, 0)) min_list = s0 < s1 ? 0 : 1;
                     for (uint32_t li = 0; li < nls && (use || off == 0); li++) {
-                        if (!blk[li]) continue;
+                        if (!blk.get((int)li, 0)) continue;
                         if (prune_th > 0) {
                             const uint32_t dev = (BEST_SAD(li, 0)[n] - best) * 100;
-                            if (dev > best * prune_th) { blk[li] = 0; continue; }
+                            if (dev > best * prune_th) { blk.set((int)li, 0, false); continue; }
                         }
                         if (min_list != -1 && min_list != (int)li) {
                             if (use) l_mv[pu * d.max_refs + (li ? d.max_l0 : 0)] = BEST_MV(li, 0)[n];
@@ -2097,25 +2222,25 @@
                         }
                         off++;
                     }
-                    if (blk[0] && blk[1] && use) { put_cand(off, pack(2, 0, 0, 0, 1)); l_total[pu] = (uint8_t)(off + 1); }
+                    if (blk.get(0, 0) && blk.get(1, 0) && use) { put_cand(off, pack(2, 0, 0, 0, 1)); l_total[pu] = (uint8_t)(off + 1); }
                 } else {
-                    const int pu = (n > 4) ? c_z_to_raster[n] : n;
+                    const int pu = (n > 4) ? z_to_raster(n) : n;
                     uint8_t   off = 0;
-                    uint8_t   blk[2][4] = {{0, 0, 0, 0}, {0, 0, 0, 0}};
+                    RefFlags<SVT_HIP_ME_LEAN_EPILOGUE != 0> blk;
                     const uint32_t prune_th = (uint32_t)c.prune_me_candidates_th;
                     uint32_t       best     = ~0u;
                     for (uint32_t li = 0; li < nls; li++)
-                        for (int ri = 0; ri < d.num_of_ref_pic_to_search[li]; ri++) {
-                            blk[li][ri] = st.do_ref[li][ri];
-                            if (blk[li][ri]) best = BEST_SAD(li, ri)[n] < best ? BEST_SAD(li, ri)[n] : best;
+                        for (int ri = 0; ri < (li ? r1 : r0); ri++) {
+                            blk.set((int)li, ri, st.do_ref[li][ri] != 0);
+                            if (blk.get((int)li, ri)) best = BEST_SAD(li, ri)[n] < best ? BEST_SAD(li, ri)[n] : best;
                         }
                     st.me_dist[pu] = best;
                     for (uint32_t li = 0; li < nls && (use || off == 0); li++)
-                        for (int ri = 0; ri < d.num_of_ref_pic_to_search[li] && (use || off == 0); ri++) {
-                            if (!blk[li][ri]) continue;
+                        for (int ri = 0; ri < (li ? r1 : r0) && (use || off == 0); ri++) {
+                            if (!blk.get((int)li, ri)) continue;
                             if (prune_th > 0) {
                                 const uint32_t dev = (BEST_SAD(li, ri)[n] - best) * 100;
-                                if (dev > best * prune_th) { blk[li][ri] = 0; continue; }
+                                if (dev > best * prune_th) { blk.set((int)li, ri, false); continue; }
                             }
                             if (use) {
                                 put_cand(off, pack(li, ri, ri, li == 0 ? li : 24, li == 1 ? li : 24));
@@ -2127,12 +2252,12 @@
                         for (int a = 0; a < r0; a++)
                             for (int bb = 0; bb < r1; bb++) {
                                 if (d.only_l_bwd && (a > 0 || bb > 0)) continue;
-                                if (blk[0][a] && blk[1][bb]) put_cand(off++, pack(2, a, bb, 0, 1));
+                                if (blk.get(0, a) && blk.get(1, bb)) put_cand(off++, pack(2, a, bb, 0, 1));
                             }
                         if (!d.only_l_bwd) {
                             for (int a = 1; a < r0; a++)
-                                if (blk[0][0] && blk[0][a]) put_cand(off++, pack(2, 0, a, 0, 0));
-                            if (r1 == 3 && blk[1][0] && blk[1][2]) put_cand(off++, pack(2, 0, 2, 1, 1));
+                                if (blk.get(0, 0) && blk.get(0, a)) put_cand(off++, pack(2, 0, a, 0, 0));
+                            if (r1 == 3 && blk.get(1, 0) && blk.get(1, 2)) put_cand(off++, pack(2, 0, 2, 1, 1));
                         }
                     }
                     if (use) l_total[pu] = off;
@@ -2140,19 +2265,27 @@
                 if (row < 88) st.cand0[row] = first;
             }
             wave_sync();
-            for (int i = tid; i < (int)(n_pu * d.max_refs); i += kThreads) o_mv[i] = l_mv[i];
-            for (int i = tid; i < (int)(n_pu * d.max_cand); i += kThreads) o_cand[i] = l_cand[i];
-            for (int i = tid; i < (int)n_pu; i += kThreads) o_total[i] = l_total[i];
+            auto copy_out = [&]() {
+                if constexpr (SVT_HIP_ME_LEAN_EPILOGUE != 0) {
+                    __builtin_assume(n_pu <= 85u);
+                    __builtin_assume(d.max_refs >= 0 && d.max_refs <= SVT_HIP_MAX_LISTS * SVT_HIP_MAX_REFS);
+                    __builtin_assume(d.max_cand >= 0 && d.max_cand <= 32);
+                }
+                for (int i = tid; i < (int)(n_pu * d.max_refs); i += kThreads) o_mv[i] = l_mv[i];
+                for (int i = tid; i < (int)(n_pu * d.max_cand); i += kThreads) o_cand[i] = l_cand[i];
+                for (int i = tid; i < (int)n_pu; i += kThreads) o_total[i] = l_total[i];
+            };
+            if constexpr (SVT_HIP_ME_LEAN_EPILOGUE == 0) copy_out();
 
             PROF(14);
             if (tid < 64) {
                 const uint32_t v8  = st.me_dist[21 + tid];
-                const uint32_t d8  = wave_sum(v8);
-                const uint32_t d16 = wave_sum(tid < 16 ? st.me_dist[5 + tid] : 0u);
-                const uint32_t d32 = wave_sum(tid < 4 ? st.me_dist[1 + tid] : 0u);
+                const uint32_t d8  = ctrl_sum32(v8);
+                const uint32_t d16 = ctrl_sum32(tid < 16 ? st.me_dist[5 + tid] : 0u);
+                const uint32_t d32 = ctrl_sum32(tid < 4 ? st.me_dist[1 + tid] : 0u);
                 const u64       mean = d8 / 64;
                 const long long dd   = (long long)v8 - (long long)mean;
-                const u64       ssq  = wave_sum((u64)(dd * dd));
+                const u64       ssq  = ctrl_sum64((u64)(dd * dd));
                 uint8_t stationary = 0, allow_gm = 0;
                 if (d.gm_enabled) {
                     const int low = d.input_resolution <= 2;
@@ -2162,17 +2295,20 @@
                     if (tid < nn) {
                         int idx = (low ? 21 : 5) + tid;
                         if (low && !d.enable_me_8x8) {
-                            if (idx >= 21) idx = c_8x8_to_16x16[idx - 21];
-                            if (!d.enable_me_16x16 && idx >= 5) idx = c_16x16_to_32x32[idx - 5];
-                        } else if (!low && !d.enable_me_16x16 && idx >= 5) idx = c_16x16_to_32x32[idx - 5];
+                            if (idx >= 21) idx = parent_16x16(idx - 21);
+                            if (!d.enable_me_16x16 && idx >= 5) idx = parent_32x32(idx - 5);
+                        } else if (!low && !d.enable_me_16x16 && idx >= 5) idx = parent_32x32(idx - 5);
                         const uint8_t  cb  = st.cand0[idx];
                         const unsigned dir = cb & 3;
                         const unsigned li  = (dir == 0 || dir == 2) ? ((cb >> 6) & 1) : ((cb >> 7) & 1);
                         const unsigned ri  = (dir == 0 || dir == 2) ? ((cb >> 2) & 3) : ((cb >> 4) & 3);
-                        const u64 a = d.picture_number, bb = d.ref_picture_number[li][ri];
-                        int th;
-                        if (low) { const int dist = (uint16_t)iabs((int)(int16_t)((a > bb ? a : bb) - (a < bb ? a : bb))); th = d.gm_use_distance_based_active_th ? imax(dist >> 1, 4) : 4; }
-                        else     { const int dist = (uint16_t)iabs((int)(int16_t)(a - bb)); th = d.gm_use_distance_based_active_th ? imax(dist * 16, 32) : 32; }
+                        int dist;
+                        if constexpr (kTab) dist = tab.ent[ref_slot((int)li, (int)ri)].gm_dist;
+                        else {
+                            const u64 a = d.picture_number, bb = d.ref_picture_number[li][ri];
+                            dist = low ? (uint16_t)iabs((int)(int16_t)((a > bb ? a : bb) - (a < bb ? a : bb))) : (uint16_t)iabs((int)(int16_t)(a - bb));
+                        }
+                        const int th = low ? (d.gm_use_distance_based_active_th ? imax(dist >> 1, 4) : 4) : (d.gm_use_distance_based_active_th ? imax(dist * 16, 32) : 32);
                         const uint32_t mv = BEST_MV(li, ri)[idx];
                         const int mx = (int)(int16_t)(mv & 0xFFFF) << 2, my = (int)(int16_t)(mv >> 16) << 2;
                         refk  = (int)(li * 4 + ri);
@@ -2191,14 +2327,17 @@
                             allow_gm = 1;
                     }
                 }
+              const uint32_t pix = uni(st.b64_w) * uni(st.b64_h), dist64 = st.me_dist[0];
+              const bool whole = SVT_HIP_ME_LEAN_EPILOGUE != 0 && pix == 4096u;
+              auto per_4096 = [&](uint32_t x) { return whole ? (x * 4096u) >> 12 : (x * 4096u) / pix; };
+              if constexpr (SVT_HIP_ME_LEAN_EPILOGUE != 0) copy_out();
               if (tid == 0) {
-                const uint32_t pix = st.b64_w * st.b64_h;
                 p.res.me_8x8_cost_variance[b] = (uint32_t)(ssq / 64);
                 p.res.rc_me_distortion[b]     = d.input_resolution <= 2 ? d8 : d16;
-                p.res.me_64x64_distortion[b]  = (st.me_dist[0] * 4096u) / pix;
-                p.res.me_32x32_distortion[b]  = (d32 * 4096u) / pix;
-                p.res.me_16x16_distortion[b]  = (d16 * 4096u) / pix;
-                p.res.me_8x8_distortion[b]    = (d8 * 4096u) / pix;
+                p.res.me_64x64_distortion[b]  = per_4096(dist64);
+                p.res.me_32x32_distortion[b]  = per_4096(d32);
+                p.res.me_16x16_distortion[b]  = per_4096(d16);
+                p.res.me_8x8_distortion[b]    = per_4096(d8);
                 p.res.stationary_block_present_sb[b] = stationary;
                 p.res.rc_me_allow_gm[b]              = allow_gm;
               }
@@ -2215,7 +2354,7 @@
                 }
             if (tid < 8) {
                 const int li = tid >> 2, ri = tid & 3;
-                const bool live = li < nl && ri < d.num_of_ref_pic_to_search[li];
+                const bool live = ref_live(li, ri);
                 if (p.res.do_ref) p.res.do_ref[(size_t)b * 8 + tid] = live ? st.do_ref[li][ri] : 0;
                 if (p.res.hme_sad) p.res.hme_sad[(size_t)b * 8 + tid] = live ? (uint32_t)st.hme_sad64[li][ri] : 0;
                 if (p.res.hme_sc) {
@@ -2260,7 +2399,14 @@
 
 #include "me_dense.inl"
 
-size_t svt_hip_me_kernel_lds_bytes(void) { return lds_layout(SVT_HIP_MAX_LISTS * SVT_HIP_MAX_REFS, 0, 1).total + SVT_HIP_ME_PROFILE_LDS; }
+size_t svt_hip_me_kernel_lds_bytes(void) {
+    uint32_t most = 0;
+    for (int mode : {kMeFull, kMeMid1, kMeS1, kMeMid2, kMeS2, kMeTail}) {
+        const uint32_t t = lds_layout(SVT_HIP_MAX_LISTS * SVT_HIP_MAX_REFS, 0, 1, mode).total;
+        most = t > most ? t : most;
+    }
+    return most + SVT_HIP_ME_PROFILE_LDS;
+}
 
 #include "svt_hip_internal.h"
 
@@ -2357,6 +2503,7 @@
         if (ctx->me_waves_per_cu && per_cu > ctx->me_waves_per_cu) per_cu = ctx->me_waves_per_cu;
         uint32_t grid = (uint32_t)ctx->num_cus * per_cu;
         if ((flags & 1u) && grid > (uint32_t)ctx->num_cus * kListWavesPerCu) grid = (uint32_t)ctx->num_cus * kListWavesPerCu;
+        if (ctx->me_max_waves && grid > ctx->me_max_waves) grid = ctx->me_max_waves;
         if (grid > total) grid = total;
         hipLaunchKernelGGL(kernel, dim3(grid), dim3(64), lds, lane->stream, d_hdr, d_par, flags);
     };
@@ -2440,3 +2587,9 @@
     ctx->me_waves_per_cu = waves;
     return SVT_HIP_OK;
 }
+
+extern "C" int svt_hip_context_set_me_max_waves(SvtHipContext *ctx, uint32_t waves) {
+    if (!ctx) return SVT_HIP_ERR_BAD_PARAM;
+    ctx->me_max_waves = waves;
+    return SVT_HIP_OK;
+}
diff --git a/svt-av1-psyex_amd/csrc/svt_hip_internal.h b/svt-av1-psyex_amd/csrc/svt_hip_internal.h
--- a/svt-av1-psyex_amd/csrc/svt_hip_internal.h
+++ b/svt-av1-psyex_amd/csrc/svt_hip_internal.h
@@ -52,6 +52,7 @@
     void       *tpl_group_host;
     hipEvent_t  tpl_group_done[4];
     int         tpl_group_next;
+    uint32_t    me_max_waves;
 };
 
 struct SvtHipPaPicture {
```

New measurement: 45880 Mpixels/s (median of 6 runs). 1.01x the previous value.
